# elcritch/figdraw

Measured on AMD Instinct MI355X. Metric: Mpixels/s composited @3840x2160, 300 SDF rects+shadows; % HBM roofline, higher is better.
Workload: dtype f32 (blur taps: u8 x f16 -> f32 MFMA); 1 GPU; S300@4K: renderlist_100 scene at 3840x2160, 300 shadowed SDF rects + full-frame and 360x240 2-pass Gaussian backdrop blur(18) (BASELINE.json configs[2]); draws=707, phases=3, blur_nodes=2, fragments=41088819, parallelism=single GPU, frames_in_flight_per_gpu=4, walk_pool_threads=7, walk_pool_threads_default=7

## Files before the change

figdraw_amd/csrc/fdh_context.cpp:

```cpp
#include "fdh_context.h"
#include "fdh_host.h"
#include "fdh_walkpool.h"

#include <chrono>

#include <algorithm>
#include <cmath>
#include <cstdio>
#include <cstring>

namespace fdh {

void hip_check(hipError_t e, const char* what) {
  if (e != hipSuccess) throw Error(FDH_ERR_HIP, std::string(what) + ": " + hipGetErrorString(e));
}

void poison_fresh(void* p, size_t bytes) {
#if defined(FDH_POISON)
  if (!p || !bytes) return;
  (void)hipMemset(p, FDH_POISON, bytes);
  (void)hipDeviceSynchronize();
#else
  (void)p; (void)bytes;
#endif
// ... 376 lines not shown
      B.sub_first[p] = at; B.sub_x0[p] = x0; B.sub_y0[p] = y0; B.sub_nx[p] = std::max(1, nx);
      at += nx * ny;
    }
    B.sub_first[np] = at;
    B.sub_n = np;
  }
  return B;
}

Context::Schedule Context::schedule(const LaunchJob& J, bool direct, bool partial) {
  const int nb = J.bins_x * J.bins_y;
  Schedule S;
  const int order_key = J.bins_x * 65536 + J.bins_y;
  if (order_valid_ && order_nb_ != order_key) order_valid_ = false;
  const bool sorting = J.clear && !J.phases.empty() && nb <= 8192 && J.phases[0].count > 0 && !direct && !partial;
  if (sorting) {
    S.order_now = order_valid_ ? d_order_[order_read_].ptr : nullptr;
    const int wr = order_valid_ ? 1 - order_read_ : order_read_;
    d_order_[wr].reserve(nb);
    S.order_next = d_order_[wr].ptr;
    order_read_ = wr;
    order_nb_ = order_key;
    order_valid_ = true;
  }
  static const int deep_env = [] { const char* e = std::getenv("FDH_DEEP_MIN"); return e ? std::atoi(e) : -1; }();
  S.deep_min = deep_env >= 0 ? deep_env : (vram_contexts_alive(device_) > 1 ? kDeepMinInFlight : kDeepMinDefault);
  if (sorting && S.deep_min > 0) {
    if (!deep_host_) {
      FDH_HIP(hipHostMalloc((void**)&deep_host_, 64, hipHostMallocDefault));
      for (int c = 0; c < 8; c++) deep_host_[c] = 0;
    }
    if (S.order_now) {
      uint32_t most = 0;
      for (int c = 0; c < 8; c++) most = std::max(most, (uint32_t)deep_host_[c]);
      S.deep_k8 = 8 * (int)std::min<uint32_t>(most, 1024u);
    }
  }
  return S;
}

uint32_t* Context::launch_blur(const LaunchJob& J, int p, uint32_t* cur, int row_lo, int row_hi, bool partial) {
  const Phase& ph = J.phases[p];
  if (ph.blur < 0) return cur;
  const BlurJob& j = J.blurs[ph.blur];
  const bool big = ph.blur == J.big_blur;
  const int vy0 = std::max(j.y0, row_lo), vy1 = std::min(j.y1, row_hi);
  if (vy1 <= vy0 || j.x1 <= j.x0) return cur;
  BlurParams bp;
  bp.W = J.W; bp.H = J.H; bp.pitch = J.W;
  bp.taps = j.taps;
  bp.node_pixels = (long long)(j.x1 - j.x0) * (j.y1 - j.y0);
  bp.fuse_draw = -1;
  bp.mx_w = (size_t)ph.blur < J.mx_w_h.size() ? J.mx_w_h[ph.blur] : nullptr;
  bp.x0 = j.x0; bp.x1 = j.x1; bp.y0 = vy0; bp.y1 = vy1;
  if ((size_t)ph.blur < J.blur_fused.size() && J.blur_fused[ph.blur]) {
    uint32_t* other = cur == fb_ ? alt_ : fb_;
    bp.src = cur; bp.dst = other;
    bp.fuse_draw = j.fuse_draw;
    span_begin(kSpanBlurFused);
    const bool done = launch_blur_fused(stream_, bp, J.mx_w_v[ph.blur], J.dv.recs, J.dv.exts);
    span_end();
    if (!done) throw Error(FDH_ERR_HIP, "fused blur: no kernel for this filter width (blur_fused_supported out of step with the launcher)");
    return other;
  }
  if (j.fuse_draw < 0 && J.latency_routes && blur_one_kernel_ok(j.x1 - j.x0, j.y1 - j.y0, j.taps.reach)) {
    bp.src = cur; bp.dst = backdrop_;
    span_begin(big ? kSpanBigBlurV : kSpanBlurV);
    launch_blur_small(stream_, bp);
    span_end();
    return cur;
  }
  bp.src = cur; bp.dst = blur_tmp_;
  bp.y0 = std::max(0, vy0 - j.taps.reach); bp.y1 = std::min(J.H, vy1 + j.taps.reach);
  const bool guard = partial && j.fuse_draw >= 0;
  if (guard) damage_.guard(stream_, J, ph.blur, false, cur, vy0, vy1);
  span_begin(big ? kSpanBigBlurH : kSpanBlurH);
  launch_blur_h(stream_, bp);
  span_end();
  bp.src = blur_tmp_; bp.dst = j.fuse_draw >= 0 ? cur : backdrop_;
  bp.mx_w = (size_t)ph.blur < J.mx_w_v.size() ? J.mx_w_v[ph.blur] : nullptr;
  bp.fuse_draw = j.fuse_draw;
  bp.y0 = vy0; bp.y1 = vy1;
  span_begin(big ? kSpanBigBlurV : kSpanBlurV);
  launch_blur_v(stream_, bp, J.dv.recs, J.dv.exts);
  span_end();
  if (guard) damage_.guard(stream_, J, ph.blur, true, cur, vy0, vy1);
  return cur;
}

CompositeParams Context::composite_params(const LaunchJob& J, int p, uint32_t* cur, int row_lo, int row_hi, bool direct, const Schedule& S) const {
  const Phase& ph = J.phases[p];
  const int nb = J.bins_x * J.bins_y;
  const bool full = p == 0 && J.clear;
  CompositeParams C;
  C.lists = J.lists + (size_t)p * nb * J.list_stride;
  C.counts = J.counts + (size_t)p * nb;
  C.backdrop = backdrop_;
  C.fb = cur;
  for (int l = 0; l < kMaxMips; l++) C.atlas.level[l] = atlas_levels_[l];
  C.atlas.size = atlas_size_; C.atlas.n_levels = n_levels_;
  C.W = J.W; C.H = J.H; C.pitch = J.W;
  C.bins_x = J.bins_x; C.stride = J.list_stride;
  C.bin_x0 = full ? 0 : ph.bin_x0; C.bin_y0 = full ? 0 : ph.bin_y0;
  C.bin_nx = full ? J.bins_x : ph.bin_x1 - ph.bin_x0; C.bin_ny = full ? J.bins_y : ph.bin_y1 - ph.bin_y0;
  C.row_lo = row_lo; C.row_hi = row_hi;
  C.load_fb = full ? 0 : 1;
  C.clear_rgba8 = J.clear_rgba8;
  C.direct = direct ? 1 : 0; C.direct_first = ph.first; C.direct_n = ph.count; C.binrec = J.dv.binrecs;
  C.order = full ? S.order_now : nullptr; C.order_next = full ? S.order_next : nullptr;
  C.deep_k8 = full ? S.deep_k8 : 0; C.deep_min = S.deep_min;
  static const int deep_strip_min = [] { const char* e = std::getenv("FDH_DEEP_STRIP_MIN"); return e ? std::atoi(e) : kDeepStripMinDefault; }();
  C.deep_strip_min = deep_strip_min;
  C.deep_out = (full && S.order_next && S.deep_min > 0) ? const_cast<uint32_t*>(deep_host_) : nullptr;
  C.has_slow = ph.has_slow; C.has_slow_atlas = ph.has_slow_atlas; C.has_rot = ph.has_rot; C.has_atlas = ph.has_atlas; C.has_masks = ph.has_masks;
  C.mask_spill = J.mask_spill; C.spill_stride = J.spill_stride;
  return C;
}

void Context::launch_frame(const LaunchJob& J, bool profile, uint32_t upload_seq) {
  profiling_ = profile;
  std::vector<int> lo, hi;
  phase_rows(J, lo, hi);
  const bool direct = direct_frame(J);
  const BinParams B = bin_params(J, upload_seq);
  span_begin(kSpanBin); if (!direct) launch_bin(stream_, B); span_end();
  const bool partial = damage_.launch(stream_, J, B, readback_, [this](bool begin) { if (begin) span_begin(kSpanBin); else span_end(); });
  const Schedule S = schedule(J, direct, partial);
  uint32_t* cur = fb_;
  for (int p = 0; p < (int)J.phases.size(); p++) {
    cur = launch_blur(J, p, cur, lo[p], hi[p], partial);
    CompositeParams C = composite_params(J, p, cur, lo[p], hi[p], direct, S);
    if (C.load_fb == 0) stats_.deep_bins = (float)composite_build(C).deep_k8;
    span_begin(p == 0 ? kSpanCompositeMain : kSpanCompositeLater);
    if (partial) damage_.composite(stream_, J, C);
    else launch_composite(stream_, J.dv.recs, J.dv.exts, C);
    span_end();
  }
  if (cur != fb_) std::swap(fb_, alt_);
  damage_.launched_whole(J);
  FDH_HIP(hipGetLastError());
}

void Context::replay(int times) {
  need_device("replay");
  drain();
  if (!have_frame_) throw Error(FDH_ERR_INVALID, "replay: no frame has been submitted");
  FDH_HIP(hipSetDevice(device_));
  if (times <= 0) return;
  FDH_HIP(hipEventRecord(ev_[0], stream_));
  for (int i = 0; i < times; i++) launch_frame(job_, false);
  FDH_HIP(hipEventRecord(ev_[1], stream_));
  FDH_HIP(hipEventSynchronize(ev_[1]));
  float ms = 0.0f;
  FDH_HIP(hipEventElapsedTime(&ms, ev_[0], ev_[1]));
  stats_.ms_total = ms / (float)times;
}

void Context::replay_async(int times) {
  need_device("replay_async");
  drain();
// ... 140 lines not shown
```

figdraw_amd/csrc/fdh_context.h:

```cpp
#pragma once
#include <hip/hip_runtime.h>

#include <algorithm>
#include <atomic>
#include <chrono>
#include <condition_variable>
#include <cstdint>
#include <cstdlib>
#include <cstring>
#include <exception>
#include <memory>
#include <mutex>
#include <stdexcept>
#include <string>
#include <thread>
#include <unordered_map>
#include <vector>

#include "../../include/figdraw_hip.h"
#include "../../include/figdraw_hip_pick.h"
#include "../../include/figdraw_hip_readback.h"
#include "../../include/figdraw_hip_stream.h"
#include "fdh_kernels.h"

// ... 279 lines not shown
  std::vector<DrawRec> recs;
  std::vector<BinRec> bins;
  std::vector<QuadExt> exts;
  std::vector<PickTag> tags;
  bool tagged = false;
  PhaseSum sum;
  int64_t fragments = 0;
  bool cacheable = false;
  bool dirty = true;
  uint64_t atlas_epoch = 0;
  int cull_y0 = 0, cull_y1 = 0;
};
struct RetainedLayer {
  int32_t zlevel = 0;
  std::vector<FdhFig> nodes;
  std::vector<int32_t> roots;
  std::vector<RetainedRoot> cache;
};
struct RetainedScene {
  bool valid = false;
  float fw = 0, fh = 0, rgba[4] = {1, 1, 1, 1};
  bool clear = true;
  float ui_scale = 1.0f, aa = 0.0f;
  bool subpixel = false, variants = false;
  uint32_t table_epoch = 0, table_epoch_seen = 0;
  std::vector<RetainedLayer> layers;
  std::vector<FdhGlyph> glyphs;
  std::vector<int64_t> variant_ids;
  std::vector<FdhDrawOp> ops;
  std::vector<float> controls;
  std::vector<FdhTextRect> text_rects;
  int64_t roots_walked = 0, roots_reused = 0;
};

struct FrameLayout {
  size_t recs = 0, exts = 0, binrecs = 0, boxes = 0, chunks = 0, phase_first = 0, tables = 0, total = 0;
  size_t n = 0, n_ext = 0, n_chunks = 1;
  std::vector<size_t> mx_h, mx_v;
  size_t misc() const { return chunks; }
  void lay_out(size_t n_recs, size_t n_exts, size_t n_phases, const std::vector<BlurJob>& blurs);
  bool operator==(const FrameLayout& o) const {
    return total == o.total && recs == o.recs && exts == o.exts && binrecs == o.binrecs && boxes == o.boxes && chunks == o.chunks &&
           phase_first == o.phase_first && n == o.n && n_ext == o.n_ext && mx_h == o.mx_h && mx_v == o.mx_v;
  }
};

struct LaunchJob {
  struct View { DrawRec* recs = nullptr; QuadExt* exts = nullptr; BinRec* binrecs = nullptr; int* phase_first = nullptr; uint32_t* binbox = nullptr; uint32_t* chunkbox = nullptr; };
  int W = 0, H = 0;
  int rec_y0 = 0, rec_y1 = 0;
  bool clear = true;
  bool latency_routes = true;
  uint32_t clear_rgba8 = 0xFFFFFFFFu;
  std::vector<Phase> phases;
  std::vector<BlurJob> blurs;
  std::vector<const uint4*> mx_w_h, mx_w_v;
  std::vector<char> blur_fused;
  int n_fused = 0;
  int n_recs = 0;
  FrameLayout layout;
  View dv;
  uint32_t* mask_spill = nullptr;
  size_t spill_stride = 0;
  uint2* lists = nullptr;
  uint32_t* counts = nullptr;
  int bins_x = 0, bins_y = 0, list_stride = 0, binbox_shift = 0;
  int big_blur = -1;
  std::vector<UploadRun> runs;
  UploadTable table;
  void* d_dst = nullptr;
  int staging_slot = -1;
  bool damage = false, damage_force = false;
  uint64_t damage_key = 0;
  int n_exts = 0;
  bool pick = false;
  std::vector<PickTag> pick_tags;
  int pick_depth = 0;
};

}
#include "fdh_damage_host.h"
namespace fdh {

class Context : public Recorder {
 public:
  Context(int atlas_size, float pixel_scale, int device, uint32_t flags);
  ~Context();

  void begin_frame(int w, int h, bool clear, const float rgba[4]);
  void end_frame();
  float pixel_scale() const { return pixel_scale_; }
  void set_subpixel_enabled(bool e) { subpixel_enabled_ = e; }
  void set_subpixel_variants(bool e) { subpixel_variants_ = e; }
  void set_text_lcd_filtering(bool e) { text_lcd_filtering_ = e; }
  bool text_lcd_filtering() const { return text_lcd_filtering_; }
  void comm_info(int* rank, int* world) const { *rank = comm_ ? comm_rank_ : 0; *world = comm_ ? comm_world_ : 1; }

  void put_image(int64_t key, int w, int h, const uint8_t* rgba, int out_rect[4]);
  void put_glyph_image(int64_t key, int w, int h, const uint8_t* rgba, uint32_t flags, int out_rect[4]);
  void put_glyph_outline(int64_t key, int w, int h, const float* segs, int n, uint32_t flags, int out_rect[4]);
  void update_image(int64_t key, int w, int h, const uint8_t* rgba);
  void put_mips(int64_t key, int n, const int* ws, const int* hs, const uint8_t* const* premul_rgba, int out_rect[4]);
  void put_flippy(int64_t key, const uint8_t* data, size_t n, int out_rect[4]);
  void remove_image(int64_t key) { entries_.erase(key); atlas_epoch_++; }
  bool has_image(int64_t key) const { return entries_.count(key) != 0; }
  void reset_atlas(int minimum_size);
// ... 37 lines not shown
  void set_damage_tracking(bool on);
  void damage_bins(uint8_t* mask, int cap, int* bins_x, int* bins_y, int* n_damaged, bool changed_only);
  void set_damage_readback(bool on);
  void read_damage(const FdhDamageTile** tiles, const uint8_t** pixels, int* n_tiles, int* frame_w, int* frame_h, int* full);
  void read_damage_into(uint8_t* image, int64_t pitch_bytes, int w, int h, int* n_tiles);
  void read_damage_coded(const FdhCodedTile** tiles, const uint8_t** payload, int* n_tiles, int64_t* payload_bytes, int* frame_w, int* frame_h, int* full);
  void set_damage_exact(bool on);
  void damage_exact_stats(int* n_pending, int* n_changed, int* fresh);
  void set_pick(bool on) { pick_on_ = on; }
  void set_pick_tag(int32_t z, int32_t id) { tag_ = PickTag{z, id}; }
  void pick_points(const float* xy, int n, int threshold, uint32_t flags, int max_hits, FdhPickHit* out, int* counts);
  void pick_region(int x, int y, int w, int h, int threshold, uint32_t flags, int32_t* out_draw);
  void pick_draw_tags(int32_t* zlevels, int32_t* ids, int cap, int* n);
  void set_cull(int mode) { cull_mode_ = mode < 0 ? 0 : (mode > 2 ? 2 : mode); }
  int64_t culled_draws() const { return culled_total_; }
  void set_walk_threads(int n) { walk_threads_ = n < 0 ? -1 : (n > 64 ? 64 : n); }
  int walk_threads() const;
  int64_t parallel_groups() const { return parallel_groups_; }
  void set_blur_route(int route) { blur_route_ = route < 0 ? -1 : (route ? 1 : 0); }
  void replay(int times);
  void replay_timed(int times, float* ms_out);
  void replay_async(int times);
  void profile(int times);
  void frame_stats(FdhFrameStats* out) { drain(); *out = stats_; out->ms_host_launch = launch_ms_.load(std::memory_order_relaxed); }
  void flush() { drain(); }

 private:
  friend class Recorder;
  friend struct ParallelWalk;
  void release_device_state();
  void rec_begin_frame(bool clear, const float rgba[4]);
  void rec_end_frame();
  void alloc_atlas(int size);
  void upload_atlas_rect(int level, int x, int y, int w, int h, const uint8_t* rgba);
  void put_levels(int x, int y, int w, int h, const uint8_t* rgba);
  void find_empty_rect(int w, int h, int* ox, int* oy);
  struct FoldGuard {
    BinRec* br = nullptr;
    BBox box{0, 0, 0, 0};
    FoldGuard() = default;
    FoldGuard(FoldGuard&& o) noexcept : br(o.br), box(o.box) { o.br = nullptr; }
    FoldGuard(const FoldGuard&) = delete;
    FoldGuard& operator=(const FoldGuard&) = delete;
    ~FoldGuard() { if (br) br->box = box; }
  };

  void prepare(LaunchJob& J);
  void describe_frame(LaunchJob& J);
  void size_bin_buffers(LaunchJob& J);
  void layout_frame_block(LaunchJob& J);
  void choose_fused_blurs(LaunchJob& J);
  void consolidate_pieces();
  FoldGuard fold_clear(LaunchJob& J);
  void damage_frame_key(LaunchJob& J) const;
  bool shadow_usable(const LaunchJob& J);
  bool tables_resident(const LaunchJob& J, bool shadow_ok);
  void build_misc(const LaunchJob& J, bool tables_resident);
  bool patch_runs(LaunchJob& J, bool shadow_ok);
  void gather_runs(LaunchJob& J, bool tables_resident);
  void account_frame(LaunchJob& J);
  void fence_staging();
  void issue(LaunchJob& J);
  void launch_frame(const LaunchJob& J, bool profile, uint32_t upload_seq = 0);
  struct Schedule { const int* order_now = nullptr; int* order_next = nullptr; int deep_min = 0, deep_k8 = 0; };
  void phase_rows(const LaunchJob& J, std::vector<int>& lo, std::vector<int>& hi) const;
  BinParams bin_params(const LaunchJob& J, uint32_t upload_seq) const;
  Schedule schedule(const LaunchJob& J, bool direct, bool partial);
  uint32_t* launch_blur(const LaunchJob& J, int p, uint32_t* cur, int row_lo, int row_hi, bool partial);
  CompositeParams composite_params(const LaunchJob& J, int p, uint32_t* cur, int row_lo, int row_hi, bool direct, const Schedule& S) const;
  template <typename Buf> void reserve_quiet(Buf& buf, size_t n);
  void drain();
  void worker_main();
  hipEvent_t next_event();
  void ensure_surfaces();
  void need_device(const char* what) const;
  void split_phase(int blur);
  void open_piece();
  void close_piece();
  void add_piece(const Piece& p, const PhaseSum& s, const BBox& outer_union, int64_t fragments, int64_t culled);
  void add_sum(const PhaseSum& s, int depth_base);
  void close_phase();
  uint32_t global_index(uint32_t lane0_index) const { return lane0_index + g0_delta_; }
  uint32_t global_count() const;
  Lane& lane(int i) { return i < 0 ? *merge_lane_[(size_t)staging_i_] : *lanes_[(size_t)staging_i_][(size_t)i]; }
  Lane& ensure_lane(int i);
  void splice_cached(const RetainedRoot& C);
  void pick_routes();
  void pool_slots(int slots);

  int device_ = 0;
  uint32_t flags_ = 0;
  int blur_route_ = -1;
  bool latency_routes_ = true;
  std::shared_ptr<void> comm_;
  int comm_rank_ = 0, comm_world_ = 1;
  hipStream_t own_stream_ = nullptr, stream_ = nullptr;
  volatile unsigned int* hdp_flush_reg_ = nullptr;
  hipEvent_t ev_[2] = {};
  std::vector<hipEvent_t> ev_pool_;
  size_t ev_used_ = 0;
  enum SpanKind { kSpanBin, kSpanCompositeMain, kSpanCompositeLater, kSpanBlurH, kSpanBlurV, kSpanBigBlurH, kSpanBigBlurV, kSpanBlurFused, kSpanKinds };
  struct Span { SpanKind kind; hipEvent_t a, b; };
  std::vector<Span> spans_;
  bool profiling_ = false;
  void span_begin(SpanKind kind); void span_end();

// ... 23 lines not shown
  std::exception_ptr worker_error_;
  alignas(128) LaunchJob job_;
  std::atomic<float> launch_ms_{0.0f};
  alignas(128) LaunchJob next_;
  const void* tables_dev_ = nullptr;
  FrameLayout tables_layout_;
  std::vector<float> tables_sig_, tables_sig_next_;

  alignas(128) bool rec_diff_upload_ = false;
  std::vector<Piece> pieces_;
  bool piece_open_ = false;
  uint32_t n_total_ = 0, n_ext_total_ = 0;
  uint32_t g0_delta_ = 0;
  std::vector<Phase> phases_;
  std::vector<BlurJob> blurs_;
  BBox phase_u_{0, 0, 0, 0};
  int stride_max_ = 1;
  int phase_extra_ = 0;
  int deepest_clip_ = 0;
  int64_t frag_mode_[4] = {0, 0, 0, 0}, frag_ellip_ = 0, frag_other_ = 0;
  bool have_frame_ = false;

  alignas(128) uint32_t* fb_ = nullptr;
  uint32_t *backdrop_ = nullptr, *blur_tmp_ = nullptr;
  uint32_t* alt_ = nullptr;
  uint32_t* dbg_snap_ = nullptr;
  void glyph_to_atlas(uint32_t* cur, uint32_t* nxt, int w, int h, int x, int y, uint32_t flags);
  void put_glyph_mtsdf(int64_t key, int w, int h, const float* segs, int n, float range, int out_rect[4]);
  DeviceBuf<float> glyph_lines_, glyph_acc_, glyph_edges_;
  DeviceBuf<uint32_t> glyph_a_, glyph_b_;
  RetainedScene retained_;
  uint64_t atlas_epoch_ = 1;
  void rebase_side(FdhFig* nodes, int n, const FdhScene* side);
  void compact_side();
  bool host_only_ = false;
  bool rec_on_ = false, rec_first_ = true, rec_mark_first_ = true;
  size_t rec_mark_ = 0;
  std::string rec_;
  int surf_w_ = 0, surf_h_ = 0;
  DeviceBuf<uint8_t> d_frame_;
  DeviceBuf<uint32_t> d_mask_spill_;
  DeviceBuf<uint2> d_lists_;
  DeviceBuf<uint32_t> d_counts_;
  DeviceBuf<int> d_order_[2];
  DamageTracker damage_;
  DamageReadback readback_;
  ReadFrame read_frame(const char* who);
  bool pick_on_ = false, pick_frame_ = false;
  void pick_check(const char* who, int threshold, uint32_t flags);
  DeviceBuf<uint8_t> d_pick_, d_pick_spill_;
  PinnedBuf<uint8_t> h_pick_;
  int order_read_ = 0, order_nb_ = 0;
  bool order_valid_ = false;
  struct MxTables { int reach; std::vector<float> dense; std::vector<uint8_t> h, v; };
  std::vector<MxTables> mx_cache_;
  static constexpr int kStaging = 4;
  std::vector<std::unique_ptr<Lane>> lanes_[kStaging];
  std::unique_ptr<Lane> merge_lane_[kStaging];
  std::vector<std::unique_ptr<Recorder>> pool_recs_;
  uint64_t frame_no_ = 0;
  HostVec<uint8_t> misc_[kStaging];
  std::vector<uint8_t> misc_host_;
  const uint8_t* misc_dev_[kStaging] = {};
  const uint8_t* misc_dev_host_[kStaging] = {};
  std::vector<uint8_t> shadow_;
  FrameLayout shadow_layout_;
  const void* shadow_dev_ = nullptr;
  int64_t uploaded_bytes_ = 0;
  hipEvent_t staging_ev_[kStaging] = {};
  char staging_busy_[kStaging] = {};
  uint32_t staging_seq_[kStaging] = {};
  volatile uint32_t* deep_host_ = nullptr;
  volatile uint32_t* seq_host_ = nullptr;
  uint32_t upload_seq_ = 0;
  void wait_staging(int slot);
  int staging_i_ = 0;

  int atlas_size_ = 0, initial_atlas_size_ = 0, atlas_margin_ = 4, n_levels_ = 0;
  uint32_t* atlas_levels_[kMaxMips] = {};
  std::vector<uint16_t> heights_;
  std::unordered_map<int64_t, AtlasEntry> entries_;

  FdhFrameStats stats_ = {};
 public:
  int64_t host_ns_[12] = {};
  struct HostTimer {
    int64_t& acc; std::chrono::steady_clock::time_point t0;
    explicit HostTimer(int64_t& a) : acc(a), t0(std::chrono::steady_clock::now()) {}
    ~HostTimer() { acc += std::chrono::duration_cast<std::chrono::nanoseconds>(std::chrono::steady_clock::now() - t0).count(); }
  };
 private:
  std::chrono::steady_clock::time_point t_begin_frame_, t_walk_begin_;
  float host_record_ms_ = 0.0f;
};

template <typename Buf> void Context::reserve_quiet(Buf& buf, size_t n) {
  if (n <= buf.cap) return;
  drain();
  FDH_HIP(hipStreamSynchronize(stream_));
  buf.reserve(n);
}

void record_host_form(DrawRec& r);
void stripe_rows(int height, int world, int rank, int* y0, int* y1);
void comm_unique_id(uint8_t out[FDH_COMM_ID_BYTES]);
void blur_weight_fragments(float blur_radius, bool vertical, float* dense, uint16_t* frag_bits, int* reach, int* k_steps);
void saturated_core_of(const float rect[4], const float rx[4], const float ry[4], int mode, float factor, float spread,
// ... 4 lines not shown
```

figdraw_amd/csrc/fdh_device.h:

```cpp
#pragma once
#include <hip/hip_runtime.h>
#include <hip/hip_ext.h>
#include <stdint.h>
#include <algorithm>
#include <type_traits>

#include "fdh_kernels.h"

#include <cstddef>
#include <cstdlib>

namespace fdh {

#ifndef FDH_STATS
#define FDH_STATS 0
#endif
#ifndef FDH_TIMING
#define FDH_TIMING 0
#endif
#ifndef FDH_SPLIT_UNIFORM
#define FDH_SPLIT_UNIFORM 0
#endif
#if FDH_TIMING
#define FDH_NOW() clock64()
// ... 375 lines not shown
    long long a0 = (long long)q.e[t][0].a * X + (long long)q.e[t][0].b * Y + q.e[t][0].c;
    long long a1 = (long long)q.e[t][1].a * X + (long long)q.e[t][1].b * Y + q.e[t][1].c;
    long long a2 = (long long)q.e[t][2].a * X + (long long)q.e[t][2].b * Y + q.e[t][2].c;
    bool in = a0 >= 0 && a1 >= 0 && a2 >= 0;
    uint32_t own = q.own >> (t * 3);
    if (a0 == 0 && !(own & 1u)) in = false;
    if (a1 == 0 && !(own & 2u)) in = false;
    if (a2 == 0 && !(own & 4u)) in = false;
    if (in) { hit = t; e0 = a0; e1 = a1; e2 = a2; }
  }
  f.covered = f.covered && hit >= 0;
  const int t = hit < 0 ? 0 : hit;
  const float is = q.inv_sum[t];
  const float l0 = (float)e0 * is, l1 = (float)e1 * is, l2 = (float)e2 * is;
  const float u0 = t == 0 ? uax : utx, v0 = t == 0 ? uay : uay;
  const float u1 = t == 0 ? uax : uax, v1 = t == 0 ? uty : uay;
  const float u2 = utx, v2 = uty;
  f.u = l0 * u0 + l1 * u1 + l2 * u2;
  f.v = l0 * v0 + l1 * v1 + l2 * v2;
  F4 c0 = unpack255(t == 0 ? r.col[3] : r.col[2]);
  F4 c1 = unpack255(t == 0 ? r.col[0] : r.col[3]);
  F4 c2 = unpack255(r.col[1]);
  const float k = 1.0f / 255.0f;
  f.col.x = (l0 * c0.x + l1 * c1.x + l2 * c2.x) * k;
  f.col.y = (l0 * c0.y + l1 * c1.y + l2 * c2.y) * k;
  f.col.z = (l0 * c0.z + l1 * c1.z + l2 * c2.z) * k;
  f.col.w = (l0 * c0.w + l1 * c1.w + l2 * c2.w) * k;
  f.fw_u = q.fw_u[t];
  f.fw_v = q.fw_v[t];
  f.lod = q.lod[t];
  return f;
}

typedef float f2 __attribute__((ext_vector_type(2)));
__device__ __forceinline__ void blend(F4& F, float r, float g, float b, float sa) {
  const float ia = 1.0f - sa, A = 255.0f * sa;
  F.x = __builtin_rintf(__builtin_fmaf(F.x, ia, r * A));
  F.y = __builtin_rintf(__builtin_fmaf(F.y, ia, g * A));
  F.z = __builtin_rintf(__builtin_fmaf(F.z, ia, b * A));
  F.w = __builtin_rintf(__builtin_fmaf(F.w, ia, A));
}
__device__ __forceinline__ void blend_pre(F4& F, f2 c_rg, f2 c_ba, float ia) {
  f2 xy = {F.x, F.y}, zw = {F.z, F.w};
  const f2 ia2 = {ia, ia};
  xy = __builtin_elementwise_fma(xy, ia2, c_rg);
  zw = __builtin_elementwise_fma(zw, ia2, c_ba);
  F.x = __builtin_rintf(xy.x); F.y = __builtin_rintf(xy.y); F.z = __builtin_rintf(zw.x); F.w = __builtin_rintf(zw.y);
}

__device__ __forceinline__ void blend_black(F4& F, float A, float ia) {
  F.x = __builtin_rintf(F.x * ia); F.y = __builtin_rintf(F.y * ia); F.z = __builtin_rintf(F.z * ia); F.w = __builtin_rintf(__builtin_fmaf(F.w, ia, A));
}

__device__ __forceinline__ float rect_mask_alpha(const DrawRec& r, float cx, float cy) {
  float lx = (r.ox * cx + r.oy * cy) + r.inv_w;
  float ly = (r.inv_h * cx + r.f0 * cy) + r.f1;
  float qx = lx - r.p0, qy = ly - r.p1;
  float dist = shape_dist((r.op_mode & F_ELLIP) != 0u, qx, -qy, r.p2, r.p3, r.r[0], r.r[1], r.r[2], r.r[3]);
  return 1.0f - clamp01(r.aa * dist + 0.5f);
}

__device__ __forceinline__ DrawRec load_rec(const DrawRec* __restrict__ p) {
  DrawRec r;
  const uint4* __restrict__ src = reinterpret_cast<const uint4*>(p);
  uint4* dst = reinterpret_cast<uint4*>(&r);
#pragma unroll
  for (int i = 0; i < 8; i++) dst[i] = src[i];
  return r;
}

typedef uint32_t u32x4 __attribute__((ext_vector_type(4)));
__device__ __forceinline__ DrawRec load_rec_whole(const DrawRec* __restrict__ p) {
  const u32x4* __restrict__ src = reinterpret_cast<const u32x4*>(p);
  u32x4 q[8];
#pragma unroll
  for (int i = 0; i < 8; i++) q[i] = src[i];
  asm volatile("" : "+s"(q[0]), "+s"(q[1]), "+s"(q[2]), "+s"(q[3]), "+s"(q[4]), "+s"(q[5]), "+s"(q[6]), "+s"(q[7]));
  DrawRec r;
  const auto f = [](uint32_t v) { return __uint_as_float(v); };
  r.op_mode = q[0].x; r.ext = q[0].y; r.ox = f(q[0].z); r.oy = f(q[0].w);
  r.inv_w = f(q[1].x); r.inv_h = f(q[1].y); r.p0 = f(q[1].z); r.p1 = f(q[1].w);
  r.p2 = f(q[2].x); r.p3 = f(q[2].y); r.f0 = f(q[2].z); r.f1 = f(q[2].w);
  r.r[0] = f(q[3].x); r.r[1] = f(q[3].y); r.r[2] = f(q[3].z); r.r[3] = f(q[3].w);
  r.col[0] = q[4].x; r.col[1] = q[4].y; r.col[2] = q[4].z; r.col[3] = q[4].w;
  r.mid = q[5].x; r.stop = q[5].y; r.aa = f(q[5].z); r.aux = f(q[5].w);
  r.aux2 = f(q[6].x);
  r.bx0 = (int16_t)(q[6].y & 0xffffu); r.by0 = (int16_t)(q[6].y >> 16); r.bx1 = (int16_t)(q[6].z & 0xffffu); r.by1 = (int16_t)(q[6].z >> 16);
  r.ix0 = (int16_t)(q[6].w & 0xffffu); r.iy0 = (int16_t)(q[6].w >> 16); r.ix1 = (int16_t)(q[7].x & 0xffffu); r.iy1 = (int16_t)(q[7].x >> 16);
  r.kx = f(q[7].y); r.ky = f(q[7].z); r._pad = q[7].w;
  return r;
}
static_assert(LE_PLAIN == 0x80000000u, "the compositor tests LE_PLAIN as the sign bit");
static_assert(offsetof(DrawRec, p2) == 32 && offsetof(DrawRec, col) == 64 && offsetof(DrawRec, aux2) == 96 && offsetof(DrawRec, bx0) == 100 && offsetof(DrawRec, ix0) == 108 && offsetof(DrawRec, aa) == 88 && offsetof(DrawRec, kx) == 116, "load_rec_whole follows DrawRec's layout");

__device__ __forceinline__ void local_x4(const DrawRec& r, float cx0, float (&lx)[4]) {
  lx[0] = __builtin_fmaf(cx0 - r.ox, r.inv_w, -0.5f) * (2.0f * r.p0);
  lx[1] = lx[0] + r.kx;
  lx[2] = __builtin_fmaf(2.0f, r.kx, lx[0]);
  lx[3] = __builtin_fmaf(3.0f, r.kx, lx[0]);
}
__device__ __forceinline__ float local_y_up(const DrawRec& r, float cy) {
  return __builtin_fmaf(r.oy - cy, r.inv_h, 0.5f) * (2.0f * r.p1);
}
__device__ __forceinline__ float cover_aa(float d, float aa) { return clamp01(__builtin_fmaf(-d, aa, 0.5f)); }

__device__ __forceinline__ void unpack2(uint32_t c, f2& rg, f2& ba) {
// ... 13 lines not shown
```

figdraw_amd/csrc/fdh_kernels.h:

```cpp
#pragma once
#include <hip/hip_runtime.h>

#include <cstdlib>

#include "fdh_types.h"

namespace fdh {

struct BinParams {
  const BinRec* binrec;
  const uint32_t* binbox;
  const uint32_t* chunkbox;
  int n_draws, binbox_shift;
  uint2* lists;
  uint32_t* counts;
  const int* phase_first;
  int n_phases, bins_x, bins_y, stride;
  const DrawRec* draws;
  const QuadExt* exts;
  int refine;
  uint32_t* seq_out = nullptr;
  uint32_t seq = 0;
  static constexpr int kBinSubs = 8;
  int sub_n = 0;
  int sub_first[kBinSubs + 1] = {};
  int sub_x0[kBinSubs] = {}, sub_y0[kBinSubs] = {}, sub_nx[kBinSubs] = {};
};

struct CompositeParams {
  const int* order;
  int* order_next;
  const uint32_t* counts;
  const uint2* lists;
  int bin_x0, bin_y0, bin_nx, bin_ny;
  int bins_x, stride;
  int row_lo, row_hi;
  int W, H, pitch;
  int load_fb;
  uint32_t clear_rgba8;
  int n_wg;
  uint32_t* fb;
  const uint32_t* backdrop;
  int has_masks;
  int has_slow;
  int has_slow_atlas = 0;
  int has_rot;
  int has_atlas;
  uint32_t* mask_spill;
  size_t spill_stride;
  AtlasView atlas;
  int direct = 0, direct_first = 0, direct_n = 0;
  const BinRec* binrec = nullptr;
  int deep_k8 = 0;
  int deep_strip_min = 0;
  int deep_min = 0;
  uint32_t* deep_out = nullptr;
};

struct BlurParams {
  const uint32_t* src;
  uint32_t* dst;
  int W, H, pitch;
  int x0, y0, x1, y1;
  int fuse_draw;
  const uint4* mx_w;
  BlurTaps taps;
  long long node_pixels = 0;
};

void set_launch_events(hipEvent_t start, hipEvent_t stop);
bool launch_events_used();
void launch_bin(hipStream_t s, const BinParams& P);
inline int forced_kernel_paths() { static const int v = [] { const char* e = std::getenv("FDH_FORCE_KERNEL_PATHS"); return e ? std::atoi(e) : 0; }(); return v; }
struct CompositeBuild { int paths = 4; size_t lds = 0; int deep_k8 = 0; bool deep = false; };
CompositeBuild composite_build(CompositeParams& P);
void launch_composite(hipStream_t s, const DrawRec* draws, const QuadExt* exts, CompositeParams P);
void launch_blur_h(hipStream_t s, const BlurParams& P);
void launch_blur_v(hipStream_t s, const BlurParams& P, const DrawRec* draws, const QuadExt* exts);
bool blur_one_kernel_ok(int w, int h, int reach);
void launch_blur_small(hipStream_t s, const BlurParams& P);
bool blur_fused_supported(int reach, int W, int pitch);
bool launch_blur_fused(hipStream_t s, const BlurParams& P, const uint4* w_v, const DrawRec* draws, const QuadExt* exts);
void launch_fill(hipStream_t s, uint32_t* p, uint32_t v, size_t n);
void launch_rasterize_lines(hipStream_t s, const float4* lines, int n, int w, int h, float* scratch, uint32_t* out);
void launch_lcd_filter(hipStream_t s, const uint32_t* src, uint32_t* dst, int w, int h);
void launch_minify2(hipStream_t s, const uint32_t* src, uint32_t* dst, int sw, int sh);
void launch_atlas_blit(hipStream_t s, uint32_t* level, int LS, int x, int y, const uint32_t* src, int w, int h);
void launch_msdf_generate(hipStream_t s, const float* edges, int n_edges, int w, int h, float orient, float range, uint32_t* out);
constexpr int kMaxUploadRuns = 96;
struct UploadRun { const void* src; uint32_t dst_off, bytes, ext_add, kind; };
struct UploadTable {
  uint32_t n_runs, copy_units, n_draws, binbox_shift;
  uint32_t bins_off, box_off, _pad0, _pad1;
  uint32_t unit_first[kMaxUploadRuns];
  UploadRun run[kMaxUploadRuns];
};
static_assert(sizeof(UploadTable) <= 4096, "the table must fit the kernel-argument segment");
void launch_upload_frame(hipStream_t s, void* dst, const UploadTable& T);

}
```

figdraw_amd/csrc/fdh_prepare.cpp:

```cpp
#include "fdh_context.h"
#include "fdh_damage.h"
#include "fdh_host.h"

#include <algorithm>
#include <chrono>
#include <cmath>
#include <cstring>

namespace fdh {

static uint16_t half_bits_rne(float f) {
  uint32_t u;
  std::memcpy(&u, &f, 4);
  const uint16_t sign = (uint16_t)((u >> 16) & 0x8000u);
  const float a = std::fabs(f);
  if (a == 0.0f) return sign;
  std::memcpy(&u, &a, 4);
  const int e = (int)(u >> 23) - 127;
  if (e < -14) return sign | (uint16_t)std::nearbyint(a * 16777216.0f);
  const uint32_t mant = u & 0x7fffffu, m = mant >> 13, rem = mant & 0x1fffu;
  uint32_t h = ((uint32_t)(e + 15) << 10) | m;
  if (rem > 0x1000u || (rem == 0x1000u && (m & 1u))) h++;
  return sign | (uint16_t)h;
}
static float half_value(uint16_t h) {
  const int e = (h >> 10) & 31, m = h & 1023;
  const float v = e == 0 ? std::ldexp((float)m, -24) : std::ldexp((float)(m + 1024), e - 25);
  return (h & 0x8000u) ? -v : v;
}
static void quantise_taps_f16(const BlurTaps& t, float* q) {
  const int r = t.reach;
  const double centre = (double)t.dense[kBlurPad + r] * 1024.0;
  q[r] = half_value(half_bits_rne((float)centre));
  double carry = 0.5 * (centre - (double)q[r]);
  for (int k = r - 1; k >= 0; k--) {
    if (t.dense[kBlurPad + k] == 0.0f) { q[k] = q[2 * r - k] = 0.0f; continue; }
    const double want = std::max((double)t.dense[kBlurPad + k] * 1024.0 + carry, 0.0);
    const float v = half_value(half_bits_rne((float)want));
    carry = want - (double)v;
    q[k] = q[2 * r - k] = v;
  }
}
static void build_mx_weights(const BlurTaps& t, bool vertical, uint8_t* out) {
  const int nk = mx_nk(t.reach, vertical), delta = mx_delta(t.reach, vertical);
  uint16_t* o = reinterpret_cast<uint16_t*>(out);
  float q[2 * kMaxBlurReach + 1];
  quantise_taps_f16(t, q);
  for (int m = 0; m < nk; m++)
    for (int lane = 0; lane < 64; lane++) {
      const int j = lane & 31, g = lane >> 5;
      for (int e = 0; e < 8; e++) {
        const int k = 16 * m + mx_krow(g, e, vertical) - delta - j;
#if FDH_MX_LO
        const float w = (k >= 0 && k <= 2 * t.reach) ? t.dense[kBlurPad + k] * 1024.0f : 0.0f;
        const uint16_t hi = half_bits_rne(w), lo = half_bits_rne(w - half_value(hi));
#else
        const float w = (k >= 0 && k <= 2 * t.reach) ? q[k] : 0.0f;
        const uint16_t hi = half_bits_rne(w), lo = 0;
#endif
        o[(((size_t)(2 * m) * 64 + lane) * 8) + e] = hi;
        o[(((size_t)(2 * m + 1) * 64 + lane) * 8) + e] = lo;
      }
    }
}

void blur_weight_fragments(float blur_radius, bool vertical, float* dense, uint16_t* frag_bits, int* reach, int* k_steps) {
  const BlurTaps t = make_taps(blur_radius);
  for (int k = 0; k <= 2 * t.reach; k++) dense[k] = t.dense[kBlurPad + k];
  *reach = t.reach;
  *k_steps = mx_nk(t.reach, vertical);
  if (*k_steps > kMxMaxNK) throw Error(FDH_ERR_INVALID, "blur_weight_fragments: filter too wide");
  build_mx_weights(t, vertical, reinterpret_cast<uint8_t*>(frag_bits));
}

void FrameLayout::lay_out(size_t n_recs, size_t n_exts, size_t n_phases, const std::vector<BlurJob>& blurs) {
  n = n_recs; n_ext = n_exts;
  n_chunks = std::max<size_t>((n + 255) / 256, 1);
  recs = 0;
  exts = align256(recs + n * sizeof(DrawRec));
  binrecs = align256(exts + n_ext * sizeof(QuadExt));
  boxes = align256(binrecs + n * sizeof(BinRec));
  chunks = align256(boxes + ((n + 3) & ~(size_t)3) * sizeof(uint32_t));
  phase_first = align256(chunks + n_chunks * sizeof(uint32_t));
  tables = align256(phase_first + (n_phases + 1) * sizeof(int));
  total = tables;
  mx_h.assign(blurs.size(), 0); mx_v.assign(blurs.size(), 0);
  for (size_t i = 0; i < blurs.size(); i++) {
    const int nkh = mx_nk(blurs[i].taps.reach, false), nkv = mx_nk(blurs[i].taps.reach, true);
    if (nkh > kMxMaxNK || nkv > kMxMaxNK) continue;
    mx_h[i] = total; total = align256(total + mx_table_bytes(nkh));
    mx_v[i] = total; total = align256(total + mx_table_bytes(nkv));
  }
}

void Context::prepare(LaunchJob& J) {
  const auto t_s0 = std::chrono::steady_clock::now();
  FDH_HIP(hipSetDevice(device_));
  describe_frame(J);
  size_bin_buffers(J);
  layout_frame_block(J);
  choose_fused_blurs(J);
  if (pieces_.size() * 3 + 2 > (size_t)kMaxUploadRuns) consolidate_pieces();
  const FoldGuard fold = fold_clear(J);
  damage_frame_key(J);
  const bool shadow_ok = shadow_usable(J), resident = tables_resident(J, shadow_ok);
  build_misc(J, resident);
  if (!patch_runs(J, shadow_ok)) gather_runs(J, resident);
  tables_dev_ = d_frame_.ptr; tables_layout_ = J.layout; tables_sig_.swap(tables_sig_next_);
  account_frame(J);
  fence_staging();
  stats_.ms_host_record = host_record_ms_;
  stats_.ms_host_upload = std::chrono::duration<float, std::milli>(std::chrono::steady_clock::now() - t_s0).count();
}

void Context::describe_frame(LaunchJob& J) {
  J.W = W_; J.H = H_; J.clear = clear_; J.clear_rgba8 = clear_rgba8_;
  J.rec_y0 = culling() ? cull_y0_ : 0; J.rec_y1 = culling() ? cull_y1_ : H_;
  J.latency_routes = latency_routes_;
  J.phases = phases_;
  J.blurs = blurs_;
  J.n_recs = (int)n_total_;
  J.n_exts = (int)n_ext_total_;
  J.bins_x = (W_ + kBin - 1) / kBin;
  J.bins_y = (H_ + kBin - 1) / kBin;
  J.binbox_shift = binbox_shift_;
  J.staging_slot = staging_i_;
}

void Context::size_bin_buffers(LaunchJob& J) {
  const int nb = J.bins_x * J.bins_y;
  J.list_stride = (stride_max_ + 7) & ~7;
  reserve_quiet(d_lists_, (size_t)J.phases.size() * nb * J.list_stride);
  reserve_quiet(d_counts_, (size_t)J.phases.size() * nb);
  J.lists = d_lists_.ptr; J.counts = d_counts_.ptr;
  J.mask_spill = nullptr;
  J.spill_stride = (size_t)nb * 16 * 64;
  if (deepest_clip_ > kMaskDepth) {
    const size_t levels = (size_t)(deepest_clip_ - kMaskDepth);
    if (levels * J.spill_stride * sizeof(uint32_t) > ((size_t)2 << 30))
      throw Error(FDH_ERR_UNSUPPORTED, "clip masks nested too deep for this frame size (the spill plane would exceed 2 GiB)");
    reserve_quiet(d_mask_spill_, levels * J.spill_stride);
    J.mask_spill = d_mask_spill_.ptr;
  }
}

void Context::layout_frame_block(LaunchJob& J) {
  FrameLayout& F = J.layout;
  F.lay_out(n_total_, n_ext_total_, J.phases.size(), J.blurs);
  if (F.total >= ((size_t)1 << 32)) throw Error(FDH_ERR_UNSUPPORTED, "frame block beyond 4 GiB");
  reserve_quiet(d_frame_, F.total);
  uint8_t* const d = d_frame_.ptr;
  J.d_dst = d;
  LaunchJob::View& dv = J.dv;
  dv.recs = reinterpret_cast<DrawRec*>(d + F.recs);
  dv.exts = reinterpret_cast<QuadExt*>(d + F.exts);
  dv.binrecs = reinterpret_cast<BinRec*>(d + F.binrecs);
// ... 13 lines not shown
  const bool fx_on = latency_routes_;
  J.blur_fused.assign(J.blurs.size(), 0);
  J.n_fused = 0;
  for (size_t i = 0; i < J.blurs.size(); i++) {
    const BlurJob& j = J.blurs[i];
    static const bool any_size = [] { const char* e = std::getenv("FDH_FORCE_BLUR_PATH"); return e && std::atoi(e) == 3; }();
    if (fx_on && clear_ && j.fuse_draw >= 0 && J.mx_w_h[i] && j.x0 == 0 && j.y0 == 0 && j.x1 == W_ && j.y1 == H_ && blur_fused_supported(j.taps.reach, W_, W_) &&
        (any_size || (long long)W_ * H_ >= 384 * 1024)) {
      J.blur_fused[i] = 1;
      J.n_fused++;
    }
  }
  if (J.n_fused > 0 && !alt_) {
    FDH_HIP(hipMalloc((void**)&alt_, (size_t)W_ * H_ * 4));
    poison_fresh(alt_, (size_t)W_ * H_ * 4);
    FDH_HIP(hipMemsetAsync(alt_, 0, (size_t)W_ * H_ * 4, stream_));
  }
}

Context::FoldGuard Context::fold_clear(LaunchJob& J) {
  FoldGuard g;
  static const bool fold_on = [] { const char* e = std::getenv("FDH_FOLD_CLEAR"); return !e || std::atoi(e) != 0; }();
  if (fold_on && clear_ && !pieces_.empty() && J.phases[0].count > 0) {
    const Piece& p0 = pieces_[0];
    Lane& L = lane(p0.lane);
    BinRec& br = L.bins[p0.first];
    const DrawRec& r = L.recs[p0.first];
    const uint32_t om = r.op_mode;
    if (((om >> 12) & 15u) == OP_DRAW && (br.flags & LE_PLAIN) && !(br.flags & BR_CORE_REMOVED) && (br.flags & BR_HAS_CORE) && br.ix0 <= 0 && br.iy0 <= 0 &&
        br.ix1 >= W_ && br.iy1 >= H_ && br.box.x0 <= 0 && br.box.y0 <= 0 && br.box.x1 >= W_ && br.box.y1 >= H_) {
      const float inv255 = 1.0f / 255.0f;
      const uint32_t c = r.col[0];
      float cf[3];
      std::memcpy(cf, &r.col[1], sizeof cf);
      const float sa = (float)(c >> 24) * inv255, A = 255.0f * sa, ia = 1.0f - sa;
      const float src[4] = {cf[0] * A, cf[1] * A, cf[2] * A, A};
      uint32_t out = 0;
      for (int k = 0; k < 4; k++) {
        const float F = (float)((J.clear_rgba8 >> (8 * k)) & 255u);
        const float v = std::nearbyintf(std::fmaf(F, ia, src[k]));
        out |= (uint32_t)std::min(std::max((int)v, 0), 255) << (8 * k);
      }
      J.clear_rgba8 = out;
      g.br = &br;
      g.box = br.box;
      br.box = BBox{0, 0, 0, 0};
      if (p0.lane > 0) L.publish_bytes(1, (size_t)p0.first * sizeof(BinRec), sizeof(BinRec));
    }
  }
  stats_.clear_folded = g.br ? 1.0f : 0.0f;
  return g;
}

void Context::damage_frame_key(LaunchJob& J) const {
  J.damage = damage_.on;
  J.damage_force = !clear_ || J.n_fused > 0 || J.blurs.size() > (size_t)kDamageMaxNodes;
  uint64_t k = 1469598103934665603ull;
  auto mix = [&k](uint64_t v) { for (int b = 0; b < 8; b++) { k ^= (v >> (8 * b)) & 255u; k *= 1099511628211ull; } };
  uint32_t aa_bits = 0, ps_bits = 0;
  std::memcpy(&aa_bits, &ctx_aa_, 4); std::memcpy(&ps_bits, &pixel_scale_, 4);
  mix((uint64_t)(uint32_t)W_ << 32 | (uint32_t)H_); mix((uint64_t)(uint32_t)J.bins_x << 32 | (uint32_t)J.bins_y);
  mix((uint64_t)J.clear_rgba8 << 1 | (clear_ ? 1u : 0u)); mix((uint64_t)aa_bits << 32 | ps_bits);
  mix(atlas_epoch_); mix((uint64_t)(uint32_t)atlas_size_);
  mix((uint64_t)(latency_routes_ ? 1u : 0u) << 8 | (uint64_t)(uint32_t)cull_mode_);
  J.damage_key = k;
}

bool Context::shadow_usable(const LaunchJob& J) {
  if (!rec_diff_upload_) shadow_dev_ = nullptr;
  return rec_diff_upload_ && shadow_dev_ == d_frame_.ptr && shadow_layout_ == J.layout && shadow_.size() == J.layout.total;
}

bool Context::tables_resident(const LaunchJob& J, bool shadow_ok) {
  std::vector<float>& sig = tables_sig_next_;
  sig.clear();
  for (size_t i = 0; i < J.blurs.size(); i++)
    if (J.layout.mx_h[i]) { const BlurTaps& t = J.blurs[i].taps; sig.push_back((float)t.reach); sig.insert(sig.end(), t.dense + kBlurPad, t.dense + kBlurPad + 2 * t.reach + 1); }
  return tables_dev_ == d_frame_.ptr && tables_layout_ == J.layout && tables_sig_ == sig && (!rec_diff_upload_ || shadow_ok);
}

void Context::build_misc(const LaunchJob& J, bool tables_resident) {
  const FrameLayout& F = J.layout;
  std::vector<uint8_t>& misc = misc_host_;
  const size_t o_misc = F.misc();
  misc.assign((tables_resident ? F.tables : F.total) - o_misc, 0);
  int* pf = reinterpret_cast<int*>(misc.data() + (F.phase_first - o_misc));
  for (size_t i = 0; i < J.phases.size(); i++) pf[i] = J.phases[i].first;
  pf[J.phases.size()] = (int)F.n;
  {
    uint32_t* cb = reinterpret_cast<uint32_t*>(misc.data());
    for (size_t c = 0; c < F.n_chunks; c++) cb[c] = 0x7f7f7f7fu;
    size_t g = 0;
    for (const Piece& p : pieces_) {
      const uint32_t* bx = lane(p.lane).boxes.p + p.first;
      for (uint32_t i = 0; i < p.n; i++, g++) {
        const uint32_t m = cb[g >> 8], v = bx[i];
        uint32_t o = 0;
        for (int sh = 0; sh < 32; sh += 8) o |= std::min((m >> sh) & 255u, (v >> sh) & 255u) << sh;
        cb[g >> 8] = o;
      }
    }
  }
  for (size_t i = 0; i < J.blurs.size() && !tables_resident; i++)
    if (F.mx_h[i]) {
      const BlurTaps& t = J.blurs[i].taps;
      const size_t bh = mx_table_bytes(mx_nk(t.reach, false)), bv = mx_table_bytes(mx_nk(t.reach, true));
      const MxTables* hit = nullptr;
      for (const MxTables& c : mx_cache_)
        if (c.reach == t.reach && std::memcmp(c.dense.data(), t.dense + kBlurPad, sizeof(float) * (2 * t.reach + 1)) == 0) { hit = &c; break; }
      if (!hit) {
        if (mx_cache_.size() >= 8) mx_cache_.erase(mx_cache_.begin());
        MxTables c;
        c.reach = t.reach;
        c.dense.assign(t.dense + kBlurPad, t.dense + kBlurPad + 2 * t.reach + 1);
        c.h.resize(bh); c.v.resize(bv);
        build_mx_weights(t, false, c.h.data());
        build_mx_weights(t, true, c.v.data());
        mx_cache_.push_back(std::move(c));
        hit = &mx_cache_.back();
      }
      std::memcpy(misc.data() + (F.mx_h[i] - o_misc), hit->h.data(), bh);
      std::memcpy(misc.data() + (F.mx_v[i] - o_misc), hit->v.data(), bv);
    }
  const int slot = J.staging_slot;
  HostVec<uint8_t>& up_misc = misc_[slot];
  up_misc.pinned = true;
  up_misc.vram = vram_staging(device_);
  up_misc.dev = device_;
  up_misc.n = 0;
  up_misc.reserve(misc.size());
  if (up_misc.p != misc_dev_host_[slot]) { misc_dev_[slot] = up_misc.device_view(); misc_dev_host_[slot] = up_misc.p; }
}

bool Context::patch_runs(LaunchJob& J, bool shadow_ok) {
  if (!shadow_ok || pieces_.size() > 1 || (!pieces_.empty() && pieces_[0].lane != 0)) return false;
  const Piece p0 = pieces_.empty() ? Piece{} : pieces_[0];
  if (p0.ext_first != 0) return false;
  const FrameLayout& F = J.layout;
  const std::vector<uint8_t>& misc = misc_host_;
  HostVec<uint8_t>& up_misc = misc_[J.staging_slot];
  const size_t o_misc = F.misc(), b_recs = F.n * sizeof(DrawRec), b_ext = F.n_ext * sizeof(QuadExt), b_bb = F.n * sizeof(BinRec);
  Lane& L = lane(0);
  L.publish(0, 0, 0, 0);
  std::vector<UploadRun>& runs = J.runs;
  runs.clear();
  std::vector<const uint8_t*> from;
  size_t dirty = 0;
  bool fits = true;
  auto diff = [&](const uint8_t* host, const uint8_t* dev_src, size_t off, size_t bytes, uint32_t kind) {
    for (size_t at = 0; at < bytes && fits; at += 256) {
      const size_t len = std::min<size_t>(256, bytes - at);
      if (std::memcmp(shadow_.data() + off + at, host + at, len) == 0) continue;
      dirty += len;
      if (!runs.empty() && runs.back().kind == kind && (size_t)runs.back().dst_off + runs.back().bytes == off + at) runs.back().bytes += (uint32_t)len;
      else if (runs.size() + 4 < (size_t)kMaxUploadRuns) { runs.push_back(UploadRun{dev_src + at, (uint32_t)(off + at), (uint32_t)len, 0u, kind}); from.push_back(host + at); }
      else fits = false;
    }
  };
  diff(reinterpret_cast<const uint8_t*>(L.recs.p + p0.first), L.d_recs + (size_t)p0.first * sizeof(DrawRec), F.recs, b_recs, 0u);
  diff(reinterpret_cast<const uint8_t*>(L.exts.p), L.d_exts, F.exts, b_ext, 0u);
  diff(reinterpret_cast<const uint8_t*>(L.bins.p + p0.first), L.d_bins + (size_t)p0.first * sizeof(BinRec), F.binrecs, b_bb, 1u);
  diff(misc.data(), misc_dev_[J.staging_slot], o_misc, F.tables - o_misc, 0u);
  if (!fits || dirty * 2 >= F.total) return false;
  for (size_t k = 0; k < runs.size(); k++) {
    std::memcpy(shadow_.data() + runs[k].dst_off, from[k], runs[k].bytes);
    const size_t off = runs[k].dst_off;
    if (off >= o_misc) std::memcpy(up_misc.p + (off - o_misc), misc.data() + (off - o_misc), runs[k].bytes);
    else if (off >= F.binrecs) L.publish_bytes(1, (size_t)p0.first * sizeof(BinRec) + (off - F.binrecs), runs[k].bytes);
    else if (off >= F.exts && b_ext) L.publish_bytes(2, off - F.exts, runs[k].bytes);
    else L.publish_bytes(0, (size_t)p0.first * sizeof(DrawRec) + (off - F.recs), runs[k].bytes);
  }
  uploaded_bytes_ = (int64_t)dirty;
  return true;
// ... 116 lines not shown
```

figdraw_amd/csrc/fdh_types.h:

```cpp
#pragma once
#include <stdint.h>

#ifndef FDH_MX_LO
#define FDH_MX_LO 0
#endif

namespace fdh {

constexpr int kTile = 8;
constexpr int kTileW = 4 * kTile;
constexpr int kTileH = kTile;
constexpr int kWavesPerWg = 4;
constexpr int kWgW = kTileW;
constexpr int kWgH = kTileH * kWavesPerWg;
constexpr int kBin = 64;
constexpr int kWgsPerBin = (kBin / kWgW) * (kBin / kWgH);
constexpr int kMaskDepth = 16;
constexpr int kDeepMinDefault = 24;
constexpr int kDeepMinInFlight = 40;
constexpr int kDeepStripMinDefault = 16;
constexpr int kMaxMips = 14;
constexpr int kMaxBlurTaps = 36;

enum : uint32_t { OP_DRAW = 0, OP_MASK_PUSH = 1, OP_MASK_POP = 2, OP_RMASK_BEGIN = 3, OP_RMASK_END = 4 };
// ... 22 lines not shown
  float aux2;
  int16_t bx0, by0, bx1, by1;
  int16_t ix0, iy0, ix1, iy1;
  float kx, ky;
  uint32_t _pad;
};
static_assert(sizeof(DrawRec) == 128, "DrawRec must be 128 bytes");

struct alignas(16) QuadExt {
  struct Edge { int32_t a, b; int64_t c; };
  Edge e[2][3];
  float inv_sum[2];
  uint32_t own;
  float fw_u[2], fw_v[2];
  float lod[2];
  float _pad[3];
  float core[4];
  float lm[2][6];
};
static_assert(sizeof(QuadExt) == 208 && offsetof(QuadExt, core) == 144 && offsetof(QuadExt, lm) == 160, "QuadExt: 208 bytes, core at 144, lm at 160");

struct alignas(8) BBox { int16_t x0, y0, x1, y1; };

struct alignas(8) BinRec { BBox box; int16_t ix0, iy0, ix1, iy1; uint32_t flags; uint32_t pad; };
static_assert(sizeof(BinRec) == 24, "BinRec must be 24 bytes");
constexpr uint32_t BR_HAS_CORE = 1u, BR_CORE_REMOVED = 2u;
constexpr uint32_t BR_GENERAL = 4u;
constexpr uint32_t BR_CURVE = 8u;
constexpr uint32_t BR_BOX_EXACT = 16u;
constexpr uint32_t LE_PLAIN = 1u << 31;
constexpr uint32_t LE_OPAQUE = 1u << 30;
constexpr int LE_PATH_SHIFT = 26;
constexpr uint32_t LE_SHARE = 1u << 25;
constexpr uint32_t LE_INDEX = LE_SHARE - 1u;

constexpr int kMaxBlurReach = 66;
constexpr int kBlurPad = 15;
struct BlurTaps {
  int n;
  int reach;
  int off[kMaxBlurTaps];
  float coef[kMaxBlurTaps];
  float dense[2 * kMaxBlurReach + 1 + 2 * kBlurPad + 16];
};

constexpr int kMxMaxNK = 11;
inline int mx_nk(int reach, bool vertical) { return (32 + 2 * reach + (vertical ? 0 : 3) + 15) / 16; }
inline int mx_delta(int reach, bool vertical) { return vertical ? 0 : ((-reach) % 4 + 4) % 4; }
#if defined(__HIPCC__)
__host__ __device__
#endif
inline int mx_krow(int g, int e, bool vertical) { return vertical ? (e & 3) + 8 * (e >> 2) + 4 * g : 8 * g + e; }
constexpr size_t mx_table_bytes(int nk) { return (size_t)nk * 2 * 64 * 16; }

struct AtlasView {
  const uint32_t* level[kMaxMips];
  int size;
  int n_levels;
};

}
```

figdraw_amd/csrc/k_blur_mx.hip:

```cpp
#include "fdh_device.h"

namespace fdh {
using h8 = __attribute__((ext_vector_type(8))) _Float16;
using f32x16 = __attribute__((ext_vector_type(16))) float;
union H8Bits { h8 v; uint32_t u[4]; };

template <int c> __device__ __forceinline__ h8 mx_frag(const uint32_t (&R)[8]) {
  constexpr uint32_t sel = 0x0c000c00u | (uint32_t)c | ((uint32_t)(4 + c) << 16);
  H8Bits o;
#pragma unroll
  for (int q = 0; q < 4; q++) o.u[q] = __builtin_amdgcn_perm(R[2 * q + 1], R[2 * q], sel);
  return o.v;
}
constexpr int kMxWaves = 2;
constexpr int mx_ring_slots(int nk, bool ) { return nk + 2; }
constexpr int mx_wg(int , bool ) { return 1; }
constexpr float kMxScale = 16384.0f;
constexpr int kMxSlot = 512;
__device__ __forceinline__ void lds_dma16(const void* src, uint32_t lds) {
  uint32_t m0_saved;
  asm volatile("s_mov_b32 %0, m0\n\ts_mov_b32 m0, %2\n\ts_nop 0\n\tglobal_load_lds_dwordx4 %1, off\n\ts_mov_b32 m0, %0"
               : "=&s"(m0_saved) : "v"(src), "s"(lds) : "memory");
}
__device__ __forceinline__ void lds_dma4(const void* src, uint32_t lds) {
  uint32_t m0_saved;
  asm volatile("s_mov_b32 %0, m0\n\ts_mov_b32 m0, %2\n\ts_nop 0\n\tglobal_load_lds_dword %1, off\n\ts_mov_b32 m0, %0"
               : "=&s"(m0_saved) : "v"(src), "s"(lds) : "memory");
}
template <int N> __device__ __forceinline__ void wait_vm() { asm volatile("s_waitcnt vmcnt(%0)" ::"n"(N) : "memory"); }

template <int NK, bool kV>
__global__ __launch_bounds__(64 * mx_wg(NK, kV), kMxWaves) void k_blur_mx(BlurParams P, const DrawRec* __restrict__ draws, const QuadExt* __restrict__ exts, int T) {
  constexpr int R = mx_ring_slots(NK, kV);
  extern __shared__ __attribute__((aligned(16))) uint32_t ring_wg[];
  constexpr int kWG = mx_wg(NK, kV);
  const int wave_in_wg = kWG > 1 ? __builtin_amdgcn_readfirstlane((int)(threadIdx.x >> 6)) : 0;
  uint32_t* const ring = ring_wg + wave_in_wg * (R * kMxSlot);
  const int a_lo = kV ? P.y0 : P.x0, a_hi = kV ? P.y1 : P.x1, a0 = a_lo & ~31;
  const int l0 = kV ? (P.x0 & ~31) : P.y0, l_hi = kV ? P.x1 : P.y1;
  const int n_along = (a_hi - a0 + 32 * T - 1) / (32 * T), n_lines = (l_hi - l0 + 31) >> 5;
  const int total = n_along * n_lines, per = (total + 7) >> 3, q = (int)(blockIdx.x >> 3) * kWG + wave_in_wg, item = (blockIdx.x & 7) * per + q;
  if (q >= per || item >= total) return;
  int sl, sa;
  if (kV) {
    constexpr int kBand = 16;
    const int per_band = kBand * n_along, band = item / per_band, rem = item - band * per_band;
    const int bw = min(kBand, n_lines - band * kBand);
    if (kWG > 1) {
      const int st = rem / n_along;
      sa = rem - st * n_along;
      sl = band * kBand + st;
    } else {
      sa = rem / bw;
      sl = band * kBand + rem - sa * bw;
    }
  } else {
    sl = item / n_along;
    sa = item - sl * n_along;
  }
  const int lane = threadIdx.x & 63, g = lane >> 5, j = lane & 31;
  const int reach = P.taps.reach;
  const int as = a0 + 32 * T * sa, lb = l0 + 32 * sl;
  const int n_blocks = min(T, (a_hi - as + 31) >> 5);
  const int w0 = as - reach, w0a = kV ? w0 : (w0 & ~3);
#if FDH_TIMING
  const unsigned long long T0 = FDH_NOW();
  unsigned long long T_wait = 0, T_st = 0, T_mma = 0, T_epi = 0, T_iss = 0;
#endif
  const uint32_t ring_lds = (uint32_t)reinterpret_cast<uintptr_t>(ring);

  const uint32_t* hsrc[2];
  if (!kV) {
    const int r = lane >> 2, c = lane & 3;
#pragma unroll
    for (int h = 0; h < 2; h++) {
      const int row = 16 * h + r, y = min(lb + row, P.y1 - 1);
      hsrc[h] = P.src + (size_t)y * P.pitch + 4 * (c ^ ((row >> 2) & 3));
    }
  }
  const int vxch = kV ? min(lb + 4 * (lane & 7), P.W - 4) : 0;
  int issue_slot = 0;
  auto issue = [&](int s) -> int {
    const uint32_t slot = ring_lds + (uint32_t)issue_slot * (kMxSlot * 4u);
    issue_slot = issue_slot + 1 == R ? 0 : issue_slot + 1;
    if (kV) {
      const int r = lane >> 3;
// ... 34 lines not shown
  h8 wlo[NK];
#endif
#pragma unroll
  for (int m = 0; m < NK; m++) {
    H8Bits a;
    const uint4 va = P.mx_w[(2 * m) * 64 + lane];
    a.u[0] = va.x; a.u[1] = va.y; a.u[2] = va.z; a.u[3] = va.w;
    whi[m] = a.v;
#if FDH_MX_LO
    H8Bits b;
    const uint4 vb = P.mx_w[(2 * m + 1) * 64 + lane];
    b.u[0] = vb.x; b.u[1] = vb.y; b.u[2] = vb.z; b.u[3] = vb.w;
    wlo[m] = b.v;
#endif
  }
  __builtin_amdgcn_s_waitcnt(0x0F70);
  last_batch = 0;
  int core_x0 = 0, core_y0 = 0, core_x1 = 0, core_y1 = 0;
  if (kV && P.fuse_draw >= 0) { const DrawRec* q = draws + P.fuse_draw; core_x0 = q->ix0; core_y0 = q->iy0; core_x1 = q->ix1; core_y1 = q->iy1; }
#if FDH_TIMING
  const unsigned long long T_pro = FDH_NOW() - T0 + (__builtin_amdgcn_readfirstlane(whi[0][0] != whi[0][1]) & 0u);
#endif
  uint32_t pend[16];
  uint32_t pmask = 0;
  int pbx = 0, pby = 0;
  auto store_pending = [&]() {
    const uint32_t lane_off = ((uint32_t)(4 * g) * (uint32_t)P.pitch + (uint32_t)j) * 4u;
    char* base = reinterpret_cast<char*>(P.dst + (size_t)pby * P.pitch + pbx);
    if (__all(pmask == 0xffffu)) {
#pragma unroll
      for (int rr = 0; rr < 16; rr++)
        *reinterpret_cast<uint32_t*>(base + (size_t)((rr & 3) + 8 * (rr >> 2)) * P.pitch * 4u + lane_off) = pend[rr];
    } else if (__any(pmask != 0u)) {
#pragma unroll
      for (int rr = 0; rr < 16; rr++)
        if ((pmask >> rr) & 1u) *reinterpret_cast<uint32_t*>(base + (size_t)((rr & 3) + 8 * (rr >> 2)) * P.pitch * 4u + lane_off) = pend[rr];
    }
    pmask = 0;
  };
  int slot0 = 0;
#pragma unroll 1
  for (int b = 0; b < n_blocks; b++) {
#if FDH_TIMING
    const unsigned long long Ta = FDH_NOW();
#endif
    wait_for_all_but(last_batch);
#if FDH_TIMING
    const unsigned long long Tb = FDH_NOW();
#endif
    store_pending();
#if FDH_TIMING
    const unsigned long long Tc = FDH_NOW();
#endif
    f32x16 acc[4];
#pragma unroll
    for (int c = 0; c < 4; c++)
#pragma unroll
      for (int e = 0; e < 16; e++) acc[c][e] = 0.0f;
#pragma unroll
    for (int m = 0; m < NK; m++) {
      const uint32_t* slot = ring + (slot0 + m >= R ? slot0 + m - R : slot0 + m) * kMxSlot;
      uint32_t t8[8];
      if (kV) {
#pragma unroll
        for (int t = 0; t < 8; t++) t8[t] = slot[((t & 3) + 8 * (t >> 2) + 4 * g) * 32 + j];
      } else {
        const uint4* row4 = reinterpret_cast<const uint4*>(slot + j * 16);
        const int sw = (j >> 2) & 3;
        const uint4 lo4 = row4[(2 * g) ^ sw], hi4 = row4[(2 * g + 1) ^ sw];
        t8[0] = lo4.x; t8[1] = lo4.y; t8[2] = lo4.z; t8[3] = lo4.w; t8[4] = hi4.x; t8[5] = hi4.y; t8[6] = hi4.z; t8[7] = hi4.w;
      }
      const h8 f0 = mx_frag<0>(t8), f1 = mx_frag<1>(t8), f2_ = mx_frag<2>(t8), f3 = mx_frag<3>(t8);
      if (kV) {
        acc[0] = __builtin_amdgcn_mfma_f32_32x32x16_f16(whi[m], f0, acc[0], 0, 0, 0);
        acc[1] = __builtin_amdgcn_mfma_f32_32x32x16_f16(whi[m], f1, acc[1], 0, 0, 0);
        acc[2] = __builtin_amdgcn_mfma_f32_32x32x16_f16(whi[m], f2_, acc[2], 0, 0, 0);
        acc[3] = __builtin_amdgcn_mfma_f32_32x32x16_f16(whi[m], f3, acc[3], 0, 0, 0);
#if FDH_MX_LO
        acc[0] = __builtin_amdgcn_mfma_f32_32x32x16_f16(wlo[m], f0, acc[0], 0, 0, 0);
        acc[1] = __builtin_amdgcn_mfma_f32_32x32x16_f16(wlo[m], f1, acc[1], 0, 0, 0);
        acc[2] = __builtin_amdgcn_mfma_f32_32x32x16_f16(wlo[m], f2_, acc[2], 0, 0, 0);
        acc[3] = __builtin_amdgcn_mfma_f32_32x32x16_f16(wlo[m], f3, acc[3], 0, 0, 0);
#endif
      } else {
        acc[0] = __builtin_amdgcn_mfma_f32_32x32x16_f16(f0, whi[m], acc[0], 0, 0, 0);
        acc[1] = __builtin_amdgcn_mfma_f32_32x32x16_f16(f1, whi[m], acc[1], 0, 0, 0);
        acc[2] = __builtin_amdgcn_mfma_f32_32x32x16_f16(f2_, whi[m], acc[2], 0, 0, 0);
        acc[3] = __builtin_amdgcn_mfma_f32_32x32x16_f16(f3, whi[m], acc[3], 0, 0, 0);
#if FDH_MX_LO
        acc[0] = __builtin_amdgcn_mfma_f32_32x32x16_f16(f0, wlo[m], acc[0], 0, 0, 0);
        acc[1] = __builtin_amdgcn_mfma_f32_32x32x16_f16(f1, wlo[m], acc[1], 0, 0, 0);
        acc[2] = __builtin_amdgcn_mfma_f32_32x32x16_f16(f2_, wlo[m], acc[2], 0, 0, 0);
        acc[3] = __builtin_amdgcn_mfma_f32_32x32x16_f16(f3, wlo[m], acc[3], 0, 0, 0);
#endif
      }
    }
#if FDH_TIMING
    const unsigned long long Td = FDH_NOW() + (__builtin_amdgcn_readfirstlane(__float_as_uint(acc[0][0] + acc[1][0] + acc[2][0] + acc[3][0])) & 0u);
#endif
    const int bx = kV ? lb : as + 32 * b, by = kV ? as + 32 * b : lb;
    const int x = bx + j;
    pbx = bx; pby = by;
    const bool x_ok = x >= P.x0 && x < P.x1;
#pragma unroll
    for (int rr = 0; rr < 16; rr++)
      pend[rr] = pack2(f2{acc[0][rr] * kMxScale, acc[1][rr] * kMxScale}, f2{acc[2][rr] * kMxScale, acc[3][rr] * kMxScale});
    if (bx >= P.x0 && bx + 32 <= P.x1 && by >= P.y0 && by + 32 <= P.y1) {
      pmask = 0xffffu;
    } else {
#pragma unroll
      for (int rr = 0; rr < 16; rr++) {
        const int y = by + (rr & 3) + 8 * (rr >> 2) + 4 * g;
        if (x_ok && y >= P.y0 && y < P.y1) pmask |= 1u << rr;
      }
    }
    if (kV && P.fuse_draw >= 0) {
      const bool core = bx >= core_x0 && bx + 32 <= core_x1 && by >= core_y0 && by + 32 <= core_y1;
      bool replace_all = false;
      if (core) {
        uint32_t conj = pend[0];
#pragma unroll
        for (int rr = 1; rr < 16; rr++) conj &= pend[rr];
        replace_all = __all((conj >> 24) == 255u);
      }
      if (!replace_all) {
      uint32_t blend_mask = 0;
      uint32_t* sc0 = ring + slot0 * kMxSlot;
      uint32_t* sc1 = ring + (slot0 + 1 >= R ? slot0 + 1 - R : slot0 + 1) * kMxSlot;
      if (core) {
#pragma unroll
        for (int rr = 0; rr < 16; rr++) if (((pmask >> rr) & 1u) && (pend[rr] >> 24) != 255u) blend_mask |= 1u << rr;
      } else {
        const uint32_t valid = pmask;
        pmask = 0;
#pragma unroll
        for (int rr = 0; rr < 16; rr++) (rr < 8 ? sc0 : sc1)[(rr & 7) * 64 + lane] = __float_as_uint(((valid >> rr) & 1u) ? 1.0f : -1.0f);
        __builtin_amdgcn_wave_barrier();
        const DrawRec r = load_rec(draws + P.fuse_draw);
        const int ry0 = min(max(P.y0 - by, 0), 32), ry1 = max(ry0, min(P.y1 - by, 32)), rx0 = min(max(P.x0 - bx, 0), 32), rx1 = max(rx0, min(P.x1 - bx, 32));
        const int ra = min(max(core_y0 - by, ry0), ry1), rb = max(ra, min(max(core_y1 - by, ry0), ry1));
        const int ca = min(max(core_x0 - bx, rx0), rx1), cb = max(ca, min(max(core_x1 - bx, rx0), rx1));
        const int nra = ra - ry0, nca = ca - rx0, nr = nra + ry1 - rb, nc = nca + rx1 - cb;
#pragma unroll 1
        for (int u0 = 0; u0 < nr + nc; u0 += 2) {
          const int u = u0 + g;
          int dx, dy;
          if (u < nr) { dy = u < nra ? ry0 + u : rb + (u - nra); dx = j; }
          else { const int v = u - nr; dx = v < nca ? rx0 + v : cb + (v - nca); dy = j; }
          if (u >= nr + nc) continue;
          const int ex = bx + dx, ey = by + dy;
          float alpha = -1.0f;
          if (ex >= P.x0 && ex < P.x1 && ey >= P.y0 && ey < P.y1) {
            const Frag f = make_frag(r, exts, ex, ey);
            if (f.covered) {
              const float lx = (f.u - 0.5f) * 2.0f * r.p0, ly = (f.v - 0.5f) * 2.0f * r.p1;
              const float dist = shape_dist((r.op_mode & F_ELLIP) != 0u, lx, -ly, r.p2, r.p3, r.r[0], r.r[1], r.r[2], r.r[3]);
              alpha = 1.0f - clamp01(r.aa * dist + 0.5f);
            }
          }
          const int er = (dy & 3) + 4 * (dy >> 3), el = dx + 32 * ((dy >> 2) & 1);
          (er < 8 ? sc0 : sc1)[(er & 7) * 64 + el] = __float_as_uint(alpha);
        }
        __builtin_amdgcn_wave_barrier();
#pragma unroll
        for (int rr = 0; rr < 16; rr++) {
          const float al = __uint_as_float((rr < 8 ? sc0 : sc1)[(rr & 7) * 64 + lane]);
          if (al >= 0.0f) {
            pmask |= 1u << rr;
            if (al != 1.0f || (pend[rr] >> 24) != 255u) blend_mask |= 1u << rr;
          }
        }
      }
      if (__any(blend_mask != 0u)) {
        uint32_t dstv[16];
#pragma unroll
        for (int rr = 0; rr < 16; rr++)
          dstv[rr] = ((blend_mask >> rr) & 1u) ? P.dst[(size_t)(by + (rr & 3) + 8 * (rr >> 2) + 4 * g) * P.pitch + x] : 0u;
        const float k = 1.0f / 255.0f;
#pragma unroll
        for (int rr = 0; rr < 16; rr++) {
          if (!((blend_mask >> rr) & 1u)) continue;
          const float alpha = core ? 1.0f : __uint_as_float((rr < 8 ? sc0 : sc1)[(rr & 7) * 64 + lane]);
          const F4 bl = unpack255(pend[rr]);
          F4 Fd = unpack255(dstv[rr]);
          const float sa = bl.w * k * alpha, A = 255.0f * sa;
          const float ia = 1.0f - sa;
          Fd.x = __builtin_rintf(__builtin_fmaf(Fd.x, ia, bl.x * k * A));
          Fd.y = __builtin_rintf(__builtin_fmaf(Fd.y, ia, bl.y * k * A));
          Fd.z = __builtin_rintf(__builtin_fmaf(Fd.z, ia, bl.z * k * A));
          Fd.w = __builtin_rintf(__builtin_fmaf(Fd.w, ia, A));
          pend[rr] = pack255(Fd);
        }
        __builtin_amdgcn_s_waitcnt(0x0F70);
      }
      __builtin_amdgcn_wave_barrier();
      }
    }
#if FDH_TIMING
    const unsigned long long Te = FDH_NOW() + (__builtin_amdgcn_readfirstlane(pend[0] + pend[15]) & 0u);
#endif
    __builtin_amdgcn_sched_barrier(0);
    last_batch = 0;
    if (b + 2 < n_blocks) { last_batch = issue(2 * b + NK + 2); last_batch += issue(2 * b + NK + 3); }
    slot0 = slot0 + 2 >= R ? slot0 + 2 - R : slot0 + 2;
#if FDH_TIMING
    const unsigned long long Tf = FDH_NOW();
    T_wait += Tb - Ta; T_st += Tc - Tb; T_mma += Td - Tc; T_epi += Te - Td; T_iss += Tf - Te;
#endif
  }
  store_pending();
#if FDH_TIMING
  if (lane == 0 && blockIdx.x < 32768) {
    unsigned long long* row = g_wave_times + 16 * ((size_t)blockIdx.x + (kV ? 32768 : 0));
    row[0] = FDH_NOW() - T0; row[1] = T_pro; row[2] = T_wait; row[3] = T_st; row[4] = T_mma; row[5] = T_epi; row[6] = kV ? 3 : 2; row[7] = T_iss; row[8] = n_blocks; row[9] = T0;
  }
#endif
}

constexpr int fx_vblocks(int nkv) { return ((nkv - 1) >> 1) + 1; }
constexpr int kFxWaves = 4;
constexpr int fx_wg_ksteps(int nkh) { return nkh + 2 * (kFxWaves - 1); }
constexpr int fx_slots(int nkh, int nkv) { return nkh + nkv + 2 * fx_wg_ksteps(nkh); }
constexpr float kMxMagic = 12582912.0f;
template <int NKH, int NKV>
__global__ __launch_bounds__(64 * kFxWaves, 2) void k_blur_fx(BlurParams P, const uint4* __restrict__ w_v, const DrawRec* __restrict__ draws, const QuadExt* __restrict__ exts, int T) {
  constexpr int HB = fx_vblocks(NKV);
  constexpr int NKW = fx_wg_ksteps(NKH);
  extern __shared__ __attribute__((aligned(16))) uint32_t ring[];
  const int wave = __builtin_amdgcn_readfirstlane((int)(threadIdx.x >> 6));
  const uint4* const hw = reinterpret_cast<const uint4*>(ring);
  const uint4* const vw = reinterpret_cast<const uint4*>(ring + NKH * kMxSlot);
  uint32_t* const src_base = ring + (NKH + NKV) * kMxSlot;
  const int n_strips = (P.x1 - (P.x0 & ~31) + 31) >> 5, n_sg = (n_strips + kFxWaves - 1) / kFxWaves;
  const int y_first = P.y0 & ~31;
  const int n_seg = (P.y1 - y_first + 32 * T - 1) / (32 * T);
  const int total = n_sg * n_seg, per = (total + 7) >> 3, q = (int)(blockIdx.x >> 3), item = (blockIdx.x & 7) * per + q;
  if (q >= per || item >= total) return;
  const int seg = item / n_sg, sg = item - seg * n_sg;
  const int strip = kFxWaves * sg + wave;
  const bool active = strip < n_strips;
  const int lane = threadIdx.x & 63, g = lane >> 5, j = lane & 31;
  const int reach = P.taps.reach;
  const int xb = (P.x0 & ~31) + 32 * strip;
  const int ys = y_first + 32 * T * seg;
  const int n_blocks = min(T, (P.y1 - ys + 31) >> 5);
  const int ws = ys - reach;
  const int w0a = ((P.x0 & ~31) + 32 * kFxWaves * sg - reach) & ~3;
  const uint32_t ring_lds = (uint32_t)reinterpret_cast<uintptr_t>(ring);
  const uint32_t src_lds = ring_lds + (uint32_t)((NKH + NKV) * kMxSlot * 4);

  auto issue_block = [&](int i) __attribute__((always_inline)) {
    const int r = lane >> 2, c = lane & 3;
    const uint32_t* dma_row[2];
#pragma unroll
    for (int h = 0; h < 2; h++) {
      const int row = 16 * h + r;
      int y = ws + 32 * i + row;
      y = y < 0 ? 0 : (y > P.H - 1 ? P.H - 1 : y);
      dma_row[h] = P.src + (size_t)y * P.pitch + 4 * (c ^ ((row >> 2) & 3));
    }
    const uint32_t copy = src_lds + (uint32_t)((i & 1) * NKW) * (kMxSlot * 4u);
#pragma unroll
    for (int s0 = 0; s0 < NKW; s0 += kFxWaves) {
      const int s = s0 + wave;
      if (s >= NKW) break;
      const uint32_t slot = copy + (uint32_t)s * (kMxSlot * 4u);
      const int xk = w0a + 16 * s;
      if (xk >= 0 && xk + 16 <= P.W) {
        lds_dma16(dma_row[0] + xk, slot);
        lds_dma16(dma_row[1] + xk, slot + 1024u);
      } else {
        const int rr = lane >> 4, pp = lane & 15;
#pragma unroll 1
        for (int e = 0; e < 8; e++) {
          const int row = 4 * e + rr;
          int y = ws + 32 * i + row;
          y = y < 0 ? 0 : (y > P.H - 1 ? P.H - 1 : y);
          int gx = xk + 4 * ((pp >> 2) ^ ((row >> 2) & 3)) + (pp & 3);
          gx = gx < 0 ? 0 : (gx > P.W - 1 ? P.W - 1 : gx);
          lds_dma4(P.src + (size_t)y * P.pitch + gx, slot + e * 256u);
        }
      }
    }
  };
  auto wait_for_all_but = [&](int n) __attribute__((always_inline)) {
    if (n >= 16) wait_vm<16>(); else if (n >= 3) wait_vm<3>(); else if (n == 2) wait_vm<2>(); else if (n == 1) wait_vm<1>(); else wait_vm<0>();
    __builtin_amdgcn_sched_barrier(0);
  };

#if FDH_TIMING
  const unsigned long long T0 = FDH_NOW();
  unsigned long long T_wait = 0, T_h = 0, T_v = 0, T_epi = 0, T_st = 0, T_cv = 0, T_cv_mark = 0, T_dma = 0;
#endif
  issue_block(0);
  int v_pieces = 0;
  {
    constexpr int NF = 2 * (NKH + NKV);
#pragma unroll
    for (int f0 = 0; f0 < NF; f0 += kFxWaves) {
      const int f = f0 + wave;
      if (f < NF) {
        lds_dma16((f < 2 * NKH ? P.mx_w + f * 64 : w_v + (f - 2 * NKH) * 64) + lane, ring_lds + (uint32_t)f * 1024u);
        if (f >= 2 * NKH) v_pieces++;
      }
    }
  }
#if FDH_TIMING
  const unsigned long long T_pro = FDH_NOW() - T0;
#endif
  int core_x0 = 0, core_y0 = 0, core_x1 = 0, core_y1 = 0;
  if (P.fuse_draw >= 0) { const DrawRec* qd = draws + P.fuse_draw; core_x0 = qd->ix0; core_y0 = qd->iy0; core_x1 = qd->ix1; core_y1 = qd->iy1; }

  uint32_t stash[2 * HB][4][4];
  auto operand = [](const uint32_t (&u)[4]) { H8Bits o; o.u[0] = u[0]; o.u[1] = u[1]; o.u[2] = u[2]; o.u[3] = u[3]; return o.v; };
  f32x16 acc[4];
  auto phase = [&](auto ph_tag, bool vertical) __attribute__((always_inline)) {
    constexpr int PH = decltype(ph_tag)::value;
    asm volatile("; k_blur_fx: phase %0" ::"n"(PH));
#pragma unroll
    for (int c = 0; c < 4; c++)
#pragma unroll
      for (int s2 = 0; s2 < 2; s2++)
#pragma unroll
        for (int qq = 0; qq < 4; qq++) {
          const float x0 = __builtin_fmaf(acc[c][8 * s2 + 2 * qq], kMxScale, kMxMagic), x1 = __builtin_fmaf(acc[c][8 * s2 + 2 * qq + 1], kMxScale, kMxMagic);
          const uint32_t pr = __builtin_amdgcn_perm(__float_as_uint(x1), __float_as_uint(x0), 0x0c040c00u);
          stash[2 * PH + s2][c][qq] = pr;
        }
#pragma unroll
    for (int c = 0; c < 4; c++)
#pragma unroll
      for (int s2 = 0; s2 < 2; s2++)
#pragma unroll
        for (int qq = 0; qq < 4; qq++) asm volatile("" : "+v"(stash[2 * PH + s2][c][qq]));
#if FDH_TIMING
    T_cv_mark = FDH_NOW() + (__builtin_amdgcn_readfirstlane(stash[2 * PH][0][0] ^ stash[2 * PH + 1][3][3]) & 0u);
#endif
    if (!vertical) return;
#pragma unroll
    for (int c = 0; c < 4; c++)
#pragma unroll
      for (int e = 0; e < 16; e++) acc[c][e] = 0.0f;
    constexpr int first = (PH + 1) % HB;
    uint4 va = vw[lane], vb = vw[64 + lane];
#pragma unroll
    for (int m = 0; m < NKV; m++) {
      const int slot = 2 * ((first + (m >> 1)) % HB) + (m & 1);
      H8Bits whi, wlo;
      whi.u[0] = va.x; whi.u[1] = va.y; whi.u[2] = va.z; whi.u[3] = va.w; wlo.u[0] = vb.x; wlo.u[1] = vb.y; wlo.u[2] = vb.z; wlo.u[3] = vb.w;
      if (m + 1 < NKV) { va = vw[(2 * m + 2) * 64 + lane]; vb = vw[(2 * m + 3) * 64 + lane]; }
      acc[0] = __builtin_amdgcn_mfma_f32_32x32x16_f16(whi.v, operand(stash[slot][0]), acc[0], 0, 0, 0);
      acc[1] = __builtin_amdgcn_mfma_f32_32x32x16_f16(whi.v, operand(stash[slot][1]), acc[1], 0, 0, 0);
      acc[2] = __builtin_amdgcn_mfma_f32_32x32x16_f16(whi.v, operand(stash[slot][2]), acc[2], 0, 0, 0);
      acc[3] = __builtin_amdgcn_mfma_f32_32x32x16_f16(whi.v, operand(stash[slot][3]), acc[3], 0, 0, 0);
#if FDH_MX_LO
      acc[0] = __builtin_amdgcn_mfma_f32_32x32x16_f16(wlo.v, operand(stash[slot][0]), acc[0], 0, 0, 0);
      acc[1] = __builtin_amdgcn_mfma_f32_32x32x16_f16(wlo.v, operand(stash[slot][1]), acc[1], 0, 0, 0);
      acc[2] = __builtin_amdgcn_mfma_f32_32x32x16_f16(wlo.v, operand(stash[slot][2]), acc[2], 0, 0, 0);
      acc[3] = __builtin_amdgcn_mfma_f32_32x32x16_f16(wlo.v, operand(stash[slot][3]), acc[3], 0, 0, 0);
#endif
      __builtin_amdgcn_sched_barrier(0);
    }
  };

  const int n_hblocks = n_blocks + HB - 1;
  int stores_behind = v_pieces;
  auto iteration = [&](auto ph_tag, int i) __attribute__((always_inline)) {
#if FDH_TIMING
    const unsigned long long Ta = FDH_NOW();
#endif
    wait_for_all_but(stores_behind);
    stores_behind = 0;
    __builtin_amdgcn_s_barrier();
    __builtin_amdgcn_sched_barrier(0);
    if (i + 1 < n_hblocks) issue_block(i + 1);
    __builtin_amdgcn_sched_barrier(0);
    if (!active) return;
    const uint32_t* const src_ring = src_base + ((i & 1) * NKW + 2 * wave) * kMxSlot;
#if FDH_TIMING
    const unsigned long long Tb = FDH_NOW();
#endif
#pragma unroll
    for (int c = 0; c < 4; c++)
#pragma unroll
      for (int e = 0; e < 16; e++) acc[c][e] = 0.0f;
    {
      const int sw = (j >> 2) & 3;
      auto texels = [&](int m, uint4& lo4, uint4& hi4) __attribute__((always_inline)) {
        const uint4* rowq = reinterpret_cast<const uint4*>(src_ring + m * kMxSlot + j * 16);
        lo4 = rowq[(2 * g) ^ sw]; hi4 = rowq[(2 * g + 1) ^ sw];
      };
      uint4 tl[3], th[3], wa[2], wb[2];
      h8 fr[2][4];
      texels(0, tl[0], th[0]);
      wa[0] = hw[lane]; wb[0] = hw[64 + lane];
      if (NKH > 1) { texels(1, tl[1], th[1]); wa[1] = hw[2 * 64 + lane]; wb[1] = hw[3 * 64 + lane]; }
      {
        const uint32_t t8[8] = {tl[0].x, tl[0].y, tl[0].z, tl[0].w, th[0].x, th[0].y, th[0].z, th[0].w};
        fr[0][0] = mx_frag<0>(t8); fr[0][1] = mx_frag<1>(t8); fr[0][2] = mx_frag<2>(t8); fr[0][3] = mx_frag<3>(t8);
      }
      __builtin_amdgcn_sched_barrier(0);
#pragma unroll
      for (int m = 0; m < NKH; m++) {
        const int cur = m & 1, nxt = cur ^ 1;
        H8Bits whi, wlo;
        whi.u[0] = wa[cur].x; whi.u[1] = wa[cur].y; whi.u[2] = wa[cur].z; whi.u[3] = wa[cur].w;
        wlo.u[0] = wb[cur].x; wlo.u[1] = wb[cur].y; wlo.u[2] = wb[cur].z; wlo.u[3] = wb[cur].w;
        if (m + 2 < NKH) texels(m + 2, tl[(m + 2) % 3], th[(m + 2) % 3]);
        acc[0] = __builtin_amdgcn_mfma_f32_32x32x16_f16(fr[cur][0], whi.v, acc[0], 0, 0, 0);
        acc[1] = __builtin_amdgcn_mfma_f32_32x32x16_f16(fr[cur][1], whi.v, acc[1], 0, 0, 0);
        acc[2] = __builtin_amdgcn_mfma_f32_32x32x16_f16(fr[cur][2], whi.v, acc[2], 0, 0, 0);
        acc[3] = __builtin_amdgcn_mfma_f32_32x32x16_f16(fr[cur][3], whi.v, acc[3], 0, 0, 0);
        if (m + 1 < NKH) {
          const uint4 &a4 = tl[(m + 1) % 3], &b4 = th[(m + 1) % 3];
          const uint32_t t8[8] = {a4.x, a4.y, a4.z, a4.w, b4.x, b4.y, b4.z, b4.w};
          fr[nxt][0] = mx_frag<0>(t8); fr[nxt][1] = mx_frag<1>(t8); fr[nxt][2] = mx_frag<2>(t8); fr[nxt][3] = mx_frag<3>(t8);
        }
#if FDH_MX_LO
        acc[0] = __builtin_amdgcn_mfma_f32_32x32x16_f16(fr[cur][0], wlo.v, acc[0], 0, 0, 0);
        acc[1] = __builtin_amdgcn_mfma_f32_32x32x16_f16(fr[cur][1], wlo.v, acc[1], 0, 0, 0);
        acc[2] = __builtin_amdgcn_mfma_f32_32x32x16_f16(fr[cur][2], wlo.v, acc[2], 0, 0, 0);
        acc[3] = __builtin_amdgcn_mfma_f32_32x32x16_f16(fr[cur][3], wlo.v, acc[3], 0, 0, 0);
#endif
        if (m + 2 < NKH) { wa[cur] = hw[(2 * m + 4) * 64 + lane]; wb[cur] = hw[(2 * m + 5) * 64 + lane]; }
        __builtin_amdgcn_sched_group_barrier(0x100, 2, 0);
        __builtin_amdgcn_sched_group_barrier(0x008, 4, 0);
        __builtin_amdgcn_sched_group_barrier(0x002, 16, 0);
#if FDH_MX_LO
        __builtin_amdgcn_sched_group_barrier(0x008, 4, 0);
        __builtin_amdgcn_sched_group_barrier(0x100, 2, 0);
#else
        __builtin_amdgcn_sched_group_barrier(0x100, 1, 0);
#endif
        __builtin_amdgcn_sched_barrier(0);
      }
    }
#if FDH_TIMING
    const unsigned long long Tc = FDH_NOW() + (__builtin_amdgcn_readfirstlane(__float_as_uint(acc[0][0] + acc[1][0] + acc[2][0] + acc[3][0])) & 0u);
    T_wait += Tb - Ta; T_h += Tc - Tb;
#endif
    const int b = i - (HB - 1);
    const int bx = xb, by = ys + 32 * b;
    const bool core = bx >= core_x0 && bx + 32 <= core_x1 && by >= core_y0 && by + 32 <= core_y1;
    __builtin_amdgcn_sched_barrier(0);
#if FDH_TIMING
    const unsigned long long Tc2 = FDH_NOW();
#endif
    phase(ph_tag, b >= 0);
#if FDH_TIMING
    const unsigned long long Td = FDH_NOW() + (__builtin_amdgcn_readfirstlane(__float_as_uint(acc[0][0] + acc[1][0] + acc[2][0] + acc[3][0])) & 0u);
    T_v += Td - Tc; T_cv += T_cv_mark - Tc2; T_dma += Tc2 - Tc;
#endif
    if (b < 0) return;
    const int x = bx + j;
    const bool x_ok = x >= P.x0 && x < P.x1;
    uint32_t pend[16];
    uint32_t pmask = 0;
#pragma unroll
    for (int rr = 0; rr < 16; rr++)
      pend[rr] = pack2(f2{acc[0][rr] * kMxScale, acc[1][rr] * kMxScale}, f2{acc[2][rr] * kMxScale, acc[3][rr] * kMxScale});
    if (bx >= P.x0 && bx + 32 <= P.x1 && by >= P.y0 && by + 32 <= P.y1) {
      pmask = 0xffffu;
    } else {
#pragma unroll
      for (int rr = 0; rr < 16; rr++) {
        const int y = by + (rr & 3) + 8 * (rr >> 2) + 4 * g;
        if (x_ok && y >= P.y0 && y < P.y1) pmask |= 1u << rr;
      }
    }
    if (P.fuse_draw >= 0) {
      bool replace_all = false;
      if (core) {
        uint32_t conj = pend[0];
#pragma unroll
        for (int rr = 1; rr < 16; rr++) conj &= pend[rr];
        replace_all = __all((conj >> 24) == 255u);
      }
      if (!replace_all) {
        const uint32_t valid = pmask;
        float al16[16];
#pragma unroll
        for (int rr = 0; rr < 16; rr++) al16[rr] = 1.0f;
        if (!core) {
          const DrawRec r = load_rec(draws + P.fuse_draw);
          const int ry0 = min(max(P.y0 - by, 0), 32), ry1 = max(ry0, min(P.y1 - by, 32)), rx0 = min(max(P.x0 - bx, 0), 32), rx1 = max(rx0, min(P.x1 - bx, 32));
          const int ra = min(max(core_y0 - by, ry0), ry1), rb = max(ra, min(max(core_y1 - by, ry0), ry1));
          const int ca = min(max(core_x0 - bx, rx0), rx1), cb = max(ca, min(max(core_x1 - bx, rx0), rx1));
          const int nra = ra - ry0, nca = ca - rx0, nr = nra + ry1 - rb, nc = nca + rx1 - cb;
#pragma unroll 1
          for (int u0 = 0; u0 < nr + nc; u0 += 2) {
            const int u = min(u0 + g, nr + nc - 1);
            int dx, dy;
            if (u < nr) { dy = u < nra ? ry0 + u : rb + (u - nra); dx = j; }
            else { const int v = u - nr; dx = v < nca ? rx0 + v : cb + (v - nca); dy = j; }
            const int ex = bx + dx, ey = by + dy;
            float alpha = 0.0f;
            if (ex >= P.x0 && ex < P.x1 && ey >= P.y0 && ey < P.y1) {
              const Frag f = make_frag(r, exts, ex, ey);
              if (f.covered) {
                const float lx = (f.u - 0.5f) * 2.0f * r.p0, ly = (f.v - 0.5f) * 2.0f * r.p1;
                const float dist = shape_dist((r.op_mode & F_ELLIP) != 0u, lx, -ly, r.p2, r.p3, r.r[0], r.r[1], r.r[2], r.r[3]);
                alpha = 1.0f - clamp01(r.aa * dist + 0.5f);
              }
            }
            const int abits = (int)__float_as_uint(alpha);
#pragma unroll
            for (int rr = 0; rr < 16; rr++) {
              const int y = (rr & 3) + 8 * (rr >> 2) + 4 * g;
              int su = -2, sl = 0;
              if (y >= ry0 && y < ry1 && j >= rx0 && j < rx1) {
                if (y < ra || y >= rb) { su = y < ra ? y - ry0 : nra + (y - rb); sl = j; }
                else if (j < ca || j >= cb) { su = nr + (j < ca ? j - rx0 : nca + (j - cb)); sl = y; }
              }
              const int v = __builtin_amdgcn_ds_bpermute(4 * (sl + 32 * (su & 1)), abits);
              if ((su & ~1) == u0) al16[rr] = __uint_as_float((uint32_t)v);
            }
          }
        }
        uint32_t blend_mask = 0;
#pragma unroll
        for (int rr = 0; rr < 16; rr++) {
          if (!((valid >> rr) & 1u)) continue;
          if (al16[rr] != 1.0f || (pend[rr] >> 24) != 255u) blend_mask |= 1u << rr;
        }
        if (__any(blend_mask != 0u)) {
          uint32_t dstv[16];
#pragma unroll
          for (int rr = 0; rr < 16; rr++)
            dstv[rr] = ((blend_mask >> rr) & 1u) ? P.src[(size_t)(by + (rr & 3) + 8 * (rr >> 2) + 4 * g) * P.pitch + x] : 0u;
          const float k = 1.0f / 255.0f;
#pragma unroll
          for (int rr = 0; rr < 16; rr++) {
            if (!((blend_mask >> rr) & 1u)) continue;
            const float alpha = al16[rr];
            const F4 bl = unpack255(pend[rr]);
            F4 Fd = unpack255(dstv[rr]);
            const float sa = bl.w * k * alpha, A = 255.0f * sa, ia = 1.0f - sa;
            Fd.x = __builtin_rintf(__builtin_fmaf(Fd.x, ia, bl.x * k * A));
            Fd.y = __builtin_rintf(__builtin_fmaf(Fd.y, ia, bl.y * k * A));
            Fd.z = __builtin_rintf(__builtin_fmaf(Fd.z, ia, bl.z * k * A));
            Fd.w = __builtin_rintf(__builtin_fmaf(Fd.w, ia, A));
            pend[rr] = pack255(Fd);
          }
          __builtin_amdgcn_s_waitcnt(0x0F70);
        }
      }
    }
#if FDH_TIMING
    const unsigned long long Te = FDH_NOW() + (__builtin_amdgcn_readfirstlane(pend[0] + pend[15]) & 0u);
    T_epi += Te - Td;
#endif
    __builtin_amdgcn_sched_barrier(0);
    {
      const uint32_t lane_off = ((uint32_t)(4 * g) * (uint32_t)P.pitch + (uint32_t)j) * 4u;
      char* base = reinterpret_cast<char*>(P.dst + (size_t)by * P.pitch + bx);
      if (__all(pmask == 0xffffu)) {
#pragma unroll
        for (int rr = 0; rr < 16; rr++)
          *reinterpret_cast<uint32_t*>(base + (size_t)((rr & 3) + 8 * (rr >> 2)) * P.pitch * 4u + lane_off) = pend[rr];
        stores_behind = 16;
      } else if (__any(pmask != 0u)) {
#pragma unroll
        for (int rr = 0; rr < 16; rr++)
          if ((pmask >> rr) & 1u) *reinterpret_cast<uint32_t*>(base + (size_t)((rr & 3) + 8 * (rr >> 2)) * P.pitch * 4u + lane_off) = pend[rr];
      }
    }
    __builtin_amdgcn_sched_barrier(0);
#if FDH_TIMING
    T_st += FDH_NOW() - Te;
#endif
  };
#pragma unroll 1
  for (int i = 0; i < n_hblocks; i += HB) {
    iteration(std::integral_constant<int, 0>{}, i);
    if (HB >= 2) { if (i + 1 >= n_hblocks) break; iteration(std::integral_constant<int, HB >= 2 ? 1 : 0>{}, i + 1); }
    if (HB >= 3) { if (i + 2 >= n_hblocks) break; iteration(std::integral_constant<int, HB >= 3 ? 2 : 0>{}, i + 2); }
  }
#if FDH_TIMING
  if (lane == 0) {
    const size_t w_id = (size_t)blockIdx.x * kFxWaves + wave;
    if (w_id < 32768) {
      unsigned long long* row = g_wave_times + 16 * w_id;
      row[0] = FDH_NOW() - T0; row[1] = T_pro; row[2] = T_wait; row[3] = T_h; row[4] = T_v; row[5] = T_epi; row[6] = 7; row[7] = T_st; row[8] = n_hblocks; row[9] = T0; row[10] = n_blocks; row[11] = T_cv; row[12] = T_dma;
    }
  }
#endif
}

static int mx_pick_t(long long per_cu, long long outputs_along, long long lines) {
  const long long slots = 256 * std::min<long long>(per_cu, 4 * kMxWaves);
  const long long along_blocks = (outputs_along + 31) / 32, line_groups = (lines + 31) / 32;
  for (int t = 1; t < 64; t++) if (line_groups * ((along_blocks + t - 1) / t) <= slots) return t;
  return 64;
}
template <int NK, bool kV> static void launch_blur_mx(hipStream_t s, const BlurParams& P, const DrawRec* draws, const QuadExt* exts) {
  constexpr size_t lds = (size_t)mx_ring_slots(NK, kV) * kMxSlot * sizeof(uint32_t);
  constexpr int kWG = mx_wg(NK, kV);
  static const int per_cu = [] {
    int n = 0;
    if (hipOccupancyMaxActiveBlocksPerMultiprocessor(&n, k_blur_mx<NK, kV>, 64 * kWG, lds * kWG) != hipSuccess || n <= 0) n = std::min<int>(4 * kMxWaves, 160 / (mx_ring_slots(NK, kV) * 2)) / kWG;
    return n * kWG;
  }();
  const int t = kV ? mx_pick_t(per_cu, P.y1 - P.y0, P.x1 - P.x0) : mx_pick_t(per_cu, P.x1 - P.x0, P.y1 - P.y0);
  const int a_lo = kV ? P.y0 : P.x0, a_hi = kV ? P.y1 : P.x1, l_lo = kV ? (P.x0 & ~31) : P.y0, l_hi = kV ? P.x1 : P.y1;
  const int total = ((a_hi - (a_lo & ~31) + 32 * t - 1) / (32 * t)) * ((l_hi - l_lo + 31) / 32);
  FDH_LAUNCH((k_blur_mx<NK, kV>), dim3(8 * ((total + 8 * kWG - 1) / (8 * kWG))), dim3(64 * kWG), lds * kWG, s, P, draws, exts, t);
}
template <bool kV> static bool launch_blur_mx_nk(hipStream_t s, const BlurParams& P, const DrawRec* draws, const QuadExt* exts) {
  if (!P.mx_w || (P.pitch & 3) || (reinterpret_cast<uintptr_t>(P.src) & 15) || P.W < 4) return false;
  const int nk = mx_nk(P.taps.reach, kV);
  switch (nk) {
    case 3: launch_blur_mx<3, kV>(s, P, draws, exts); return true;
    case 4: launch_blur_mx<4, kV>(s, P, draws, exts); return true;
    case 5: launch_blur_mx<5, kV>(s, P, draws, exts); return true;
    case 6: launch_blur_mx<6, kV>(s, P, draws, exts); return true;
    case 7: launch_blur_mx<7, kV>(s, P, draws, exts); return true;
    case 8: launch_blur_mx<8, kV>(s, P, draws, exts); return true;
    case 9: launch_blur_mx<9, kV>(s, P, draws, exts); return true;
    case 10: launch_blur_mx<10, kV>(s, P, draws, exts); return true;
    case 11: launch_blur_mx<11, kV>(s, P, draws, exts); return true;
    default: return false;
  }
}
template <int NKH, int NKV> static void launch_blur_fx(hipStream_t s, const BlurParams& P, const uint4* w_v, const DrawRec* draws, const QuadExt* exts) {
  constexpr size_t lds = (size_t)fx_slots(NKH, NKV) * kMxSlot * sizeof(uint32_t);
  static const int wg_per_cu = [] {
    int n = 0;
    if (hipOccupancyMaxActiveBlocksPerMultiprocessor(&n, k_blur_fx<NKH, NKV>, 64 * kFxWaves, lds) != hipSuccess || n <= 0) n = std::min<int>(8 / kFxWaves, (int)(160 * 1024 / lds));
    return n;
  }();
  const int n_strips = (P.x1 - (P.x0 & ~31) + 31) >> 5, n_sg = (n_strips + kFxWaves - 1) / kFxWaves, blocks = (P.y1 - (P.y0 & ~31) + 31) >> 5;
  const long long slots = 256LL * std::min(wg_per_cu, 8 / kFxWaves);
  int t = 2;
  while (t < 64 && (long long)n_sg * ((blocks + t - 1) / t) > slots) t++;
  const int total = n_sg * ((blocks + t - 1) / t), per = (total + 7) / 8;
  FDH_LAUNCH((k_blur_fx<NKH, NKV>), dim3(8 * per), dim3(64 * kFxWaves), lds, s, P, w_v, draws, exts, t);
}
bool blur_fused_supported(int reach, int W, int pitch) {
  const int nkh = mx_nk(reach, false), nkv = mx_nk(reach, true);
  return (pitch & 3) == 0 && W >= 4 && nkh >= 3 && nkh <= 6 && (nkh == nkv || nkh == nkv + 1);
}
bool launch_blur_fused(hipStream_t s, const BlurParams& P, const uint4* w_v, const DrawRec* draws, const QuadExt* exts) {
  if (P.x1 <= P.x0 || P.y1 <= P.y0) return true;
  if (!P.mx_w || !w_v || !blur_fused_supported(P.taps.reach, P.W, P.pitch) || (reinterpret_cast<uintptr_t>(P.src) & 15)) return false;
  const int nkh = mx_nk(P.taps.reach, false), nkv = mx_nk(P.taps.reach, true);
#define FDH_FX(a, b) if (nkh == a && nkv == b) { launch_blur_fx<a, b>(s, P, w_v, draws, exts); return true; }
  FDH_FX(3, 3) FDH_FX(4, 3) FDH_FX(4, 4) FDH_FX(5, 4) FDH_FX(5, 5) FDH_FX(6, 5) FDH_FX(6, 6)
#undef FDH_FX
  return false;
}
bool launch_blur_mx_pass(bool vertical, hipStream_t s, const BlurParams& P, const DrawRec* draws, const QuadExt* exts) {
  return vertical ? launch_blur_mx_nk<true>(s, P, draws, exts) : launch_blur_mx_nk<false>(s, P, draws, exts);
}
}
```

figdraw_amd/csrc/k_composite.hip:

```cpp
#include "fdh_device.h"
#include "fdh_shade.h"
#include "fdh_damage.h"

#ifndef FDH_TU
#define FDH_TU 0
#endif

namespace fdh {

__device__ __forceinline__ void order_bins_wave(const uint32_t* __restrict__ counts, int* __restrict__ order, int nx, int nb, uint32_t* offs, int lane, int cls,
                                                int deep_min = 0, uint32_t* __restrict__ deep_out = nullptr) {
#pragma unroll
  for (int k = 0; k < 4; k++) offs[lane + 64 * k] = 0;
  __builtin_amdgcn_wave_barrier();
  constexpr int kU = 8;
  const int nc = (nb - cls + 7) >> 3;
  for (int i0 = lane; i0 < nc; i0 += 64 * kU) {
    uint32_t c[kU];
#pragma unroll
    for (int k = 0; k < kU; k++) c[k] = i0 + 64 * k < nc ? counts[cls + 8 * (i0 + 64 * k)] : 0xffffffffu;
#pragma unroll
    for (int k = 0; k < kU; k++) if (c[k] != 0xffffffffu) atomicAdd(&offs[255u - min(c[k], 255u)], 1u);
  }
  __builtin_amdgcn_wave_barrier();
// ... 106 lines not shown
constexpr int kFastWaves = 5;
constexpr int kAtlasWaves = 5;
constexpr int kSlowWaves = 4;
constexpr int kSlowAtlasWaves = 3;
constexpr int kRotWaves = 4;
constexpr int kUniformWaves = 6;
constexpr int kWinCols = 64, kWinRows = 12, kWinStride = 68;
constexpr int kDeepSlots = 6;
constexpr int kDeepSlotFloats = 16 * 64;
constexpr int kDeepHdr = 8;
[[maybe_unused]] constexpr int kDeepLdsDwords = kDeepSlots * (kDeepSlotFloats + kDeepHdr) + kDeepSlots + 2;
constexpr uint32_t DT_NOP = 0, DT_PACKED = 1, DT_PACKED_BLACK = 2, DT_GENERIC = 3, DT_SELF17 = 4, DT_UNIFORM_PRE = 5;
struct DeepRing {
  float* data;
  uint32_t* hdr;
  uint32_t* ready;
  uint32_t* consumed;
  __device__ __forceinline__ explicit DeepRing(uint32_t* lds)
      : data(reinterpret_cast<float*>(lds)), hdr(lds + kDeepSlots * kDeepSlotFloats), ready(lds + kDeepSlots * (kDeepSlotFloats + kDeepHdr)),
        consumed(lds + kDeepSlots * (kDeepSlotFloats + kDeepHdr) + kDeepSlots) {}
};
__device__ __forceinline__ void deep_wait_ge(const uint32_t* p, const uint32_t want) {
  for (int spins = 0; spins < (1 << 20); spins++) {
    const uint32_t v = __builtin_amdgcn_readfirstlane(__hip_atomic_load(p, __ATOMIC_ACQUIRE, __HIP_MEMORY_SCOPE_WORKGROUP));
    if ((int32_t)(v - want) >= 0) return;
    __builtin_amdgcn_s_sleep(1);
  }
}

__device__ __forceinline__ uint32_t strip_shade_count(const CompositeParams& P, const int bin, const int sbit, const int lane) {
  const uint32_t cnt = P.counts[bin];
  const uint2* __restrict__ list = P.lists + (size_t)bin * P.stride;
  uint32_t n = 0;
  for (uint32_t base = 0; base < cnt; base += 64) {
    const uint32_t i = base + lane;
    const uint2 e = list[min(i, cnt - 1u)];
    const uint32_t ey = i < cnt ? e.y : 0u;
    const uint32_t st = (ey >> sbit) & 0x10001u;
    unsigned long long m = __ballot(st != 0u);
    const unsigned long long m_opaque = __ballot(st == 0x10001u && (e.x & LE_OPAQUE) != 0u);
    if (m_opaque != 0) m &= ~((1ull << (63 - __builtin_clzll(m_opaque))) - 1ull);
    m &= ~__ballot(st == 0x10001u && (int32_t)e.x < 0);
    n += (uint32_t)__builtin_popcountll(m);
  }
  return n;
}

template <int kPaths, bool kFull, int kRole, bool kDirect = false>
__device__ __forceinline__ void composite_strip(const CompositeParams& P, const DrawRec* __restrict__ draws, const QuadExt* __restrict__ exts,
                                                uint32_t* composite_lds, const int bin, const int sidx, const int sbit, const int tx0, const int ty0,
                                                const int lane, const int shader_id);

template <int kPaths, bool kFull, bool kDirect = false>
__global__ __launch_bounds__(64, (kPaths & 16) ? kSlowAtlasWaves : (kPaths & 1) ? kSlowWaves : kPaths == 4 ? kUniformWaves : (kPaths & 2) ? kAtlasWaves : (kPaths & 8) ? kRotWaves : kFastWaves) void k_composite_tiles(
    const int* __restrict__ a_order, int* __restrict__ a_order_next, const uint32_t* __restrict__ a_counts, const uint2* __restrict__ a_lists,
    int a_bin_x0, int a_bin_y0, int a_bin_nx, int a_bin_ny, int a_bins_x, int a_stride, int a_row_lo, int a_row_hi,
    const DrawRec* __restrict__ draws, const QuadExt* __restrict__ exts, const CompositeParams P_in) {
  CompositeParams P = P_in;
  [[maybe_unused]] const AtlasView& atlas_view = P_in.atlas;
  P.order = kFull ? a_order : nullptr; P.order_next = kFull ? a_order_next : nullptr; P.counts = a_counts; P.lists = a_lists;
  if (kFull) P.load_fb = 0;
  P.bin_x0 = a_bin_x0; P.bin_y0 = a_bin_y0; P.bin_nx = a_bin_nx; P.bin_ny = a_bin_ny;
  P.bins_x = a_bins_x; P.stride = a_stride; P.row_lo = a_row_lo; P.row_hi = a_row_hi;
  extern __shared__ uint32_t composite_lds[];
  uint32_t (*mask_stack)[kMaskDepth][64] = reinterpret_cast<uint32_t (*)[kMaskDepth][64]>(composite_lds);
  constexpr int kStripsPerBin = kWgsPerBin * kWavesPerWg;
  const int blk = P.order_next ? (int)blockIdx.x - 8 : (int)blockIdx.x;
  const int q = blk >> 3, xcd = blk & 7;
  if (blk < 0) {
    order_bins_wave(P.counts, P.order_next, P.bin_nx, P.bin_nx * P.bin_ny, &mask_stack[0][0][0], threadIdx.x, (int)blockIdx.x, kPaths == 4 ? P.deep_min : 0, kPaths == 4 ? P.deep_out : nullptr);
    return;
  }
  int bin_local = xcd + 8 * (q / kStripsPerBin);
  const int sidx = q % kStripsPerBin;
  if (bin_local >= P.bin_nx * P.bin_ny) return;
  const int j = sidx >> 2, wave = sidx & 3, lane = threadIdx.x & 63;
  const int sbit = j * 4 + wave;
  int bly, blx;
  if (P.order) {
    const int rc = P.order[bin_local];
    bly = rc >> 16; blx = rc & 0xffff;
  } else {
    bly = bin_local / P.bin_nx; blx = bin_local - bly * P.bin_nx;
  }
  const int bin_x = P.bin_x0 + blx, bin_y = P.bin_y0 + bly;
  const int bin = bin_y * P.bins_x + bin_x;
  const int tx0 = bin_x * kBin + (j & 1) * kWgW;
  const int ty0 = bin_y * kBin + (j >> 1) * kWgH + wave * kTileH;
  if (tx0 >= P.W) return;
  asm volatile("");
  if (ty0 >= P.H) return;
  asm volatile("");
  if (ty0 + kTileH <= P.row_lo) return;
  asm volatile("");
  if (ty0 >= P.row_hi) return;
#if FDH_TU == 1
  composite_strip<kPaths, kFull, 0, kDirect>(P, draws, exts, composite_lds, bin, sidx, sbit, tx0, ty0, lane, 0);
#else
  constexpr int kRole = 0;
  constexpr int shader_id = 0;
  {
#include "k_composite_strip.inc"
  }
#endif
}

template <int kUnit>
__global__ __launch_bounds__(256, kUniformWaves) void k_composite_deep(const DrawRec* __restrict__ draws, const QuadExt* __restrict__ exts, CompositeParams P) {
  extern __shared__ uint32_t composite_lds[];
  constexpr int kStripsPerBin = kWgsPerBin * kWavesPerWg;
  const int lane = threadIdx.x & 63, wg_wave = __builtin_amdgcn_readfirstlane((int)threadIdx.x >> 6);
  int blk = (int)blockIdx.x - 8;
  if (blk < 0) {
    if (wg_wave == 0) order_bins_wave(P.counts, P.order_next, P.bin_nx, P.bin_nx * P.bin_ny, composite_lds, lane, (int)blockIdx.x, P.deep_min, P.deep_out);
    return;
  }
  const int n_deep = P.deep_k8 * kStripsPerBin;
  const bool deep = blk < n_deep;
  int bin_local, sidx;
  if (deep) {
    const int q = blk >> 3;
    bin_local = (blk & 7) + 8 * (q / kStripsPerBin);
    sidx = q % kStripsPerBin;
// ... 41 lines not shown
  const int i = (int)blockIdx.x;
  if (i >= (int)dmg_count[0] * kStripsPerBin) return;
  CompositeParams P = P_in;
  P.order = nullptr; P.order_next = nullptr; P.deep_k8 = 0; P.deep_out = nullptr; P.direct = 0;
  if (kFull) P.load_fb = 0;
  extern __shared__ uint32_t composite_lds[];
  const int lane = threadIdx.x & 63;
  const int bin = dmg_list[i / kStripsPerBin];
  const int sidx = i % kStripsPerBin;
  const int bin_y = bin / P.bins_x, bin_x = bin - bin_y * P.bins_x;
  if (bin_x < P.bin_x0 || bin_x >= P.bin_x0 + P.bin_nx || bin_y < P.bin_y0 || bin_y >= P.bin_y0 + P.bin_ny) return;
  const int j = sidx >> 2, wave = sidx & 3;
  const int sbit = j * 4 + wave;
  const int tx0 = bin_x * kBin + (j & 1) * kWgW;
  const int ty0 = bin_y * kBin + (j >> 1) * kWgH + wave * kTileH;
  if (tx0 >= P.W) return;
  asm volatile("");
  if (ty0 >= P.H) return;
  asm volatile("");
  if (ty0 + kTileH <= P.row_lo) return;
  asm volatile("");
  if (ty0 >= P.row_hi) return;
  composite_strip<kPaths, kFull, 0>(P, draws, exts, composite_lds, bin, sidx, sbit, tx0, ty0, lane, 0);
}
template <int kPaths, bool kFull, bool kDirect>
static void launch_tiles(hipStream_t s, const CompositeBuild& b, int grid, const DrawRec* draws, const QuadExt* exts, const CompositeParams& P) {
  FDH_LAUNCH((k_composite_tiles<kPaths, kFull, kDirect>), dim3(grid), dim3(64), b.lds, s, P.order, P.order_next, P.counts, P.lists, P.bin_x0, P.bin_y0,
             P.bin_nx, P.bin_ny, P.bins_x, P.stride, P.row_lo, P.row_hi, draws, exts, P);
}
template <int kPaths>
static void launch_damage(hipStream_t s, const CompositeBuild& b, int grid, const DrawRec* draws, const QuadExt* exts, const CompositeParams& P,
                          const int* list, const uint32_t* count) {
  if (P.load_fb == 0) FDH_LAUNCH((k_composite_damage<kPaths, true>), dim3(grid), dim3(64), b.lds, s, list, count, draws, exts, P);
  else FDH_LAUNCH((k_composite_damage<kPaths, false>), dim3(grid), dim3(64), b.lds, s, list, count, draws, exts, P);
}
template <int kPaths>
static void launch_tiles_build(hipStream_t s, const CompositeBuild& b, int grid, const DrawRec* draws, const QuadExt* exts, const CompositeParams& P) {
  constexpr bool kHasDirect = kPaths == 0 || kPaths == 2 || kPaths == 4;
  const bool direct = kHasDirect && P.direct;
  if (P.load_fb == 0) direct ? launch_tiles<kPaths, true, kHasDirect>(s, b, grid, draws, exts, P) : launch_tiles<kPaths, true, false>(s, b, grid, draws, exts, P);
  else direct ? launch_tiles<kPaths, false, kHasDirect>(s, b, grid, draws, exts, P) : launch_tiles<kPaths, false, false>(s, b, grid, draws, exts, P);
}

void launch_composite_uniform(hipStream_t s, const CompositeBuild& b, int grid, const DrawRec* draws, const QuadExt* exts, const CompositeParams& P);
void launch_composite_damage_uniform(hipStream_t s, const CompositeBuild& b, int grid, const DrawRec* draws, const QuadExt* exts, const CompositeParams& P,
                                     const int* list, const uint32_t* count);
#if FDH_TU == 1 || !FDH_SPLIT_UNIFORM
void launch_composite_uniform(hipStream_t s, const CompositeBuild& b, int grid, const DrawRec* draws, const QuadExt* exts, const CompositeParams& P) {
  if (b.deep) {
    const int bins8 = (P.bin_nx * P.bin_ny + 7) / 8;
    FDH_LAUNCH((k_composite_deep<FDH_TU>), dim3(8 + P.deep_k8 * 16 + 8 * bins8 * kWgsPerBin), dim3(256), b.lds, s, draws, exts, P);
  } else if (b.paths == 2) launch_tiles_build<2>(s, b, grid, draws, exts, P);
  else if (b.paths == 0) launch_tiles_build<0>(s, b, grid, draws, exts, P);
  else launch_tiles_build<4>(s, b, grid, draws, exts, P);
}
void launch_composite_damage_uniform(hipStream_t s, const CompositeBuild& b, int grid, const DrawRec* draws, const QuadExt* exts, const CompositeParams& P,
                                     const int* list, const uint32_t* count) {
  if (b.paths == 2) launch_damage<2>(s, b, grid, draws, exts, P, list, count);
  else if (b.paths == 0) launch_damage<0>(s, b, grid, draws, exts, P, list, count);
  else launch_damage<4>(s, b, grid, draws, exts, P, list, count);
}
#endif

#if FDH_TU == 0
CompositeBuild composite_build(CompositeParams& P) {
  switch (forced_kernel_paths()) {
    case 3: P.has_slow = 1; P.has_slow_atlas = 0; break;
    case 19: P.has_slow = 1; P.has_slow_atlas = 1; break;
    case 8: P.has_rot = 1; break;
    case 2: P.has_atlas = 1; break;
    case 1: P.has_masks = 1; break;
  }
  CompositeBuild b;
  if (P.has_slow || (P.has_rot && P.has_atlas)) b.paths = P.has_slow_atlas ? 19 : 3;
  else if (P.has_rot) b.paths = 8;
  else b.paths = P.has_atlas ? 2 : P.has_masks ? 0 : 4;
  const int bins8 = (P.bin_nx * P.bin_ny + 7) / 8;
  if (b.paths == 4 && P.load_fb == 0 && P.order && P.order_next) b.deep_k8 = std::min(P.deep_k8 & ~7, 8 * bins8);
  b.deep = b.deep_k8 > 0;
  b.lds = b.deep ? sizeof(uint32_t) * kDeepLdsDwords
                 : (P.has_masks ? sizeof(uint32_t) * kMaskDepth * 64 : sizeof(uint32_t) * 256) +
                       (P.has_atlas || P.has_slow ? sizeof(uint32_t) * kWinRows * kWinStride : 0);
  return b;
}
void launch_composite_damage(hipStream_t s, const DrawRec* draws, const QuadExt* exts, CompositeParams P, const int* list, const uint32_t* count,
                             int grid) {
  if (grid <= 0 || P.bin_nx <= 0 || P.bin_ny <= 0) return;
  const CompositeBuild b = composite_build(P);
  P.n_wg = grid;
  if (b.paths == 19) launch_damage<19>(s, b, grid, draws, exts, P, list, count);
  else if (b.paths == 3) launch_damage<3>(s, b, grid, draws, exts, P, list, count);
  else if (b.paths == 8) launch_damage<8>(s, b, grid, draws, exts, P, list, count);
  else launch_composite_damage_uniform(s, b, grid, draws, exts, P, list, count);
}
void launch_composite(hipStream_t s, const DrawRec* draws, const QuadExt* exts, CompositeParams P) {
  const int n = P.bin_nx * P.bin_ny * kWgsPerBin;
  if (n <= 0) return;
  const CompositeBuild b = composite_build(P);
  P.n_wg = n;
  P.deep_k8 = b.deep_k8;
  const int bins8 = (P.bin_nx * P.bin_ny + 7) / 8;
  const int grid = 8 * bins8 * kWgsPerBin * kWavesPerWg + (P.order_next ? 8 : 0);
  if (b.paths == 19) launch_tiles_build<19>(s, b, grid, draws, exts, P);
  else if (b.paths == 3) launch_tiles_build<3>(s, b, grid, draws, exts, P);
  else if (b.paths == 8) launch_tiles_build<8>(s, b, grid, draws, exts, P);
  else launch_composite_uniform(s, b, grid, draws, exts, P);
}
#endif
}
```

figdraw_amd/csrc/k_composite_strip.inc:

```
  static_assert(kRole == 0 || (kPaths == 4 && kFull), "deep strips: the no-clip build's full-frame launch only");
  constexpr int kStripsPerBin = kWgsPerBin * kWavesPerWg;
  constexpr int mslot = 0;
  constexpr bool kBlender = kRole == 1, kShader = kRole == 2;
  uint32_t (*mask_stack)[kMaskDepth][64] = reinterpret_cast<uint32_t (*)[kMaskDepth][64]>(composite_lds);
  const DeepRing ring(composite_lds);
  uint32_t rank = 0, unit = 0;
  const int tx1 = tx0 + kTileW, ty1 = ty0 + kTileH;
  const int px0 = tx0 + (lane & 7) * 4, py = ty0 + (lane >> 3);
  const size_t spill_at = ((size_t)bin * kStripsPerBin + (size_t)sidx) * 64 + (size_t)lane;
  auto stack_put = [&](const int depth, const uint32_t v) __attribute__((always_inline)) {
    if (depth < kMaskDepth) mask_stack[mslot][depth][lane] = v;
    else __hip_atomic_store(P.mask_spill + (size_t)(depth - kMaskDepth) * P.spill_stride + spill_at, v, __ATOMIC_RELAXED, __HIP_MEMORY_SCOPE_AGENT);
  };
  auto stack_get = [&](const int depth) __attribute__((always_inline)) -> uint32_t {
    if (depth < kMaskDepth) return mask_stack[mslot][depth][lane];
    return __hip_atomic_load(P.mask_spill + (size_t)(depth - kMaskDepth) * P.spill_stride + spill_at, __ATOMIC_RELAXED, __HIP_MEMORY_SCOPE_AGENT);
  };
  constexpr bool kMasks = (kPaths & 4) == 0;
#if FDH_TIMING
  const unsigned long long T0 = FDH_NOW(), W0 = wall_clock64();
  unsigned long long T_cull = 0, T_rec = 0, T_shade = 0, T_cnt = 0, n_draws_t = 0, T_cull_core = 0, n_core_t = 0, n_all_t = 0;
  unsigned long long T_mode[4] = {0, 0, 0, 0}, N_mode[4] = {0, 0, 0, 0};
#endif
  constexpr bool direct = kDirect;
  const uint32_t cnt = direct ? (uint32_t)P.direct_n : P.counts[bin];
#if FDH_TIMING
  T_cnt = FDH_NOW() - T0 + (cnt & 0u);
#endif
  if (!kFull && cnt == 0 && P.load_fb) return;

  const bool row_ok = py < P.H;
  const bool vec_ok = row_ok && px0 + 3 < P.W && (P.pitch & 3) == 0;
  const size_t pix = (size_t)py * P.pitch + px0;
  F4 F0, F1, F2, F3;
  F0 = F1 = F2 = F3 = unpack255(P.clear_rgba8);
  if (!kFull && P.load_fb) {
    if (vec_ok) {
      const uint4 q = *reinterpret_cast<const uint4*>(P.fb + pix);
      F0 = unpack255(q.x); F1 = unpack255(q.y); F2 = unpack255(q.z); F3 = unpack255(q.w);
    } else if (row_ok) {
      if (px0 + 0 < P.W) F0 = unpack255(P.fb[pix + 0]);
      if (px0 + 1 < P.W) F1 = unpack255(P.fb[pix + 1]);
      if (px0 + 2 < P.W) F2 = unpack255(P.fb[pix + 2]);
      if (px0 + 3 < P.W) F3 = unpack255(P.fb[pix + 3]);
    }
  }
  float mk0 = 1.0f, mk1 = 1.0f, mk2 = 1.0f, mk3 = 1.0f;
  float rm0 = 1.0f, rm1 = 1.0f, rm2 = 1.0f, rm3 = 1.0f;
  int mask_depth = 0;
  bool rmask_on = false;
  bool touched = false;
  const uint2* __restrict__ list = P.lists + (size_t)bin * P.stride;
  const float cy = (float)py + 0.5f;
  const float cx0 = (float)px0 + 0.5f;
  const float inv255 = 1.0f / 255.0f;

  auto deep_slot = [&](const uint32_t rk) __attribute__((always_inline)) -> uint32_t {
    if (rk >= (uint32_t)kDeepSlots) deep_wait_ge(ring.consumed, rk - (uint32_t)kDeepSlots + 1u);
    return rk % (uint32_t)kDeepSlots;
  };
  auto deep_publish = [&](const uint32_t slot, const uint32_t rk, const uint32_t tag, const uint32_t h1, const uint32_t h2, const uint32_t h3, const uint32_t h4, const uint32_t h5) __attribute__((always_inline)) {
    uint32_t* h = ring.hdr + slot * kDeepHdr;
    h[0] = tag; h[1] = h1; h[2] = h2; h[3] = h3; h[4] = h4; h[5] = h5;
    __hip_atomic_store(ring.ready + slot, rk + 1u, __ATOMIC_RELEASE, __HIP_MEMORY_SCOPE_WORKGROUP);
  };
  auto deep_nop = [&](const uint32_t rk) __attribute__((always_inline)) { deep_publish(deep_slot(rk), rk, DT_NOP, 0u, 0u, 0u, 0u, 0u); };
  auto deep_consume = [&](const uint32_t rk) __attribute__((always_inline)) {
    const uint32_t slot = rk % (uint32_t)kDeepSlots;
    const uint32_t* h = ring.hdr + slot * kDeepHdr;
    const float* v = ring.data + slot * kDeepSlotFloats + lane;
    uint32_t tag, h1, h2, h3, h4, h5;
    float v0, v1, v2, v3;
#if FDH_TIMING
    const unsigned long long Tw0 = FDH_NOW();
#endif
    for (int spins = 0; spins < (1 << 20); spins++) {
      const uint32_t seq = __hip_atomic_load(ring.ready + slot, __ATOMIC_ACQUIRE, __HIP_MEMORY_SCOPE_WORKGROUP);
      tag = h[0]; h1 = h[1]; h2 = h[2]; h3 = h[3]; h4 = h[4]; h5 = h[5];
      v0 = v[0]; v1 = v[64]; v2 = v[128]; v3 = v[192];
      asm volatile("" : "+v"(tag), "+v"(h1), "+v"(h2), "+v"(h3), "+v"(h4), "+v"(h5), "+v"(v0), "+v"(v1), "+v"(v2), "+v"(v3));
      if ((int32_t)((uint32_t)__builtin_amdgcn_readfirstlane(seq) - (rk + 1u)) >= 0) break;
#if FDH_TIMING
      N_mode[3]++;
#endif
      __builtin_amdgcn_s_sleep(1);
    }
#if FDH_TIMING
    T_mode[3] += FDH_NOW() - Tw0 + (tag & 0u);
#endif
    tag = __builtin_amdgcn_readfirstlane(tag);
    if (tag == DT_PACKED || tag == DT_PACKED_BLACK) {
      const f2 saa = {v0, v1}, sab = {v2, v3};
      const f2 Aa = saa * 255.0f, Ab = sab * 255.0f, iaa = 1.0f - saa, iab = 1.0f - sab;
      if (tag == DT_PACKED_BLACK) {
        blend_black(F0, Aa.x, iaa.x); blend_black(F1, Aa.y, iaa.y); blend_black(F2, Ab.x, iab.x); blend_black(F3, Ab.y, iab.y);
      } else {
        const f2 crg = {__uint_as_float(__builtin_amdgcn_readfirstlane(h1)), __uint_as_float(__builtin_amdgcn_readfirstlane(h2))};
// ... 34 lines not shown
      e = list[min(i, cnt - 1u)];
    }
    const uint32_t idx = e.x;
    const uint32_t ey = i < cnt ? e.y : 0u;
    const uint32_t st = (ey >> sbit) & 0x10001u;
    unsigned long long m = __ballot(st != 0u);
    const unsigned long long m_core = __ballot(st == 0x10001u);
    const unsigned long long m_inq = __ballot(st == 0x10000u);
    if (!kMasks || !P.has_masks) {
      const unsigned long long m_opaque = __ballot(st == 0x10001u && (idx & LE_OPAQUE) != 0u);
      if (m_opaque != 0) m &= ~((1ull << (63 - __builtin_clzll(m_opaque))) - 1ull);
    }
#if FDH_TIMING
    T_cull += FDH_NOW() - Tc0 + (m & 0ull);
#endif
    if (m == 0) continue;
    const unsigned long long m_plainc = m_core & __ballot((int32_t)idx < 0);
    u32x4 plain_col = {0u, 0u, 0u, 0u};
    if (kBlender) plain_col = *reinterpret_cast<const u32x4*>(draws[idx & LE_INDEX].col);
    const uint32_t code_l = idx & (15u << LE_PATH_SHIFT);
    const unsigned long long m_simple = m & ~m_core & __ballot((kPaths & 3) == 0 ? code_l != 0u : (code_l - 1u) < (4u << LE_PATH_SHIFT));
    auto dist4 = [&](const DrawRec& r, const f2 pxa, const f2 pxb, const float py_, const float bx, const float by, f2& da, f2& db) __attribute__((always_inline)) {
      const bool top = py_ > 0.0f;
      const float rR = top ? r.r[0] : r.r[1], rL = top ? r.r[2] : r.r[3];
      const float ay = __builtin_fabsf(py_) - by;
      const f2 rra = {pxa.x > 0.0f ? rR : rL, pxa.y > 0.0f ? rR : rL}, rrb = {pxb.x > 0.0f ? rR : rL, pxb.y > 0.0f ? rR : rL};
      const f2 axa = {__builtin_fabsf(pxa.x), __builtin_fabsf(pxa.y)}, axb = {__builtin_fabsf(pxb.x), __builtin_fabsf(pxb.y)};
      const f2 qxa = axa - bx + rra, qxb = axb - bx + rrb;
      const f2 qya = ay + rra, qyb = ay + rrb;
      f2 ma = {__builtin_fmaxf(qxa.x, qya.x), __builtin_fmaxf(qxa.y, qya.y)}, mb = {__builtin_fmaxf(qxb.x, qyb.x), __builtin_fmaxf(qxb.y, qyb.y)};
      const f2 lowa = {__builtin_fminf(qxa.x, qya.x), __builtin_fminf(qxa.y, qya.y)}, lowb = {__builtin_fminf(qxb.x, qyb.x), __builtin_fminf(qxb.y, qyb.y)};
      if (__any(lowa.x > 0.0f || lowa.y > 0.0f || lowb.x > 0.0f || lowb.y > 0.0f)) {
        const f2 sa2 = qxa * qxa + qya * qya, sb2 = qxb * qxb + qyb * qyb;
        ma.x = lowa.x > 0.0f ? fsqrt(sa2.x) : ma.x; ma.y = lowa.y > 0.0f ? fsqrt(sa2.y) : ma.y;
        mb.x = lowb.x > 0.0f ? fsqrt(sb2.x) : mb.x; mb.y = lowb.y > 0.0f ? fsqrt(sb2.y) : mb.y;
      }
      da = ma - rra; db = mb - rrb;
    };
    auto dist4e = [&](const DrawRec& r, const f2 pxa, const f2 pxb, const float py_, const float bx, const float by, f2& oa, f2& ob) __attribute__((always_inline)) {
      const float px4[4] = {pxa.x, pxa.y, pxb.x, pxb.y};
      float d4[4];
      shape_distN<4>(true, px4, py_, bx, by, r.r[0], r.r[1], r.r[2], r.r[3], d4);
      oa = {d4[0], d4[1]}; ob = {d4[2], d4[3]};
    };
    auto edge_geom = [&](const DrawRec& r, const bool inset, const bool ellip, f2& lxa, f2& lxb, float& pyy, f2& da, f2& db) __attribute__((always_inline)) {
      const float shx = inset ? r.p0 : r.p2, shy = inset ? r.p1 : r.p3;
      pyy = local_y_up(r, cy);
      float lx4[4];
      local_x4(r, cx0, lx4);
      lxa = {lx4[0], lx4[1]}; lxb = {lx4[2], lx4[3]};
      if ((kPaths & 3) == 0 && ellip) dist4e(r, lxa, lxb, pyy, shx, shy, da, db); else dist4(r, lxa, lxb, pyy, shx, shy, da, db);
    };
    auto edge_blend = [&](const DrawRec& r, const uint32_t mode, const bool ellip, const bool inq, const float m_p2, const float m_p3, const float m_f0, const float m_f1,
                          const u32x4 m_col, const f2 lxa, const f2 lxb, const float pyy, const f2 da, const f2 db, F4& A0, F4& A1, F4& A2, F4& A3, const uint32_t rk) __attribute__((always_inline)) {
      f2 ala, alb;
      if (mode == 3u) {
        ala = {cover_aa(da.x, r.aa), cover_aa(da.y, r.aa)}; alb = {cover_aa(db.x, r.aa), cover_aa(db.y, r.aa)};
      } else if (mode == 12u) {
        const float h = m_f0 * 0.5f;
        const f2 ea = da + h, eb = db + h;
        const f2 ga = {__builtin_fabsf(ea.x), __builtin_fabsf(ea.y)}, gb = {__builtin_fabsf(eb.x), __builtin_fabsf(eb.y)};
        ala = {cover_aa(ga.x - h, r.aa), cover_aa(ga.y - h, r.aa)}; alb = {cover_aa(gb.x - h, r.aa), cover_aa(gb.y - h, r.aa)};
        if (__all(ala.x == 0.0f && ala.y == 0.0f && alb.x == 0.0f && alb.y == 0.0f)) {
          if (kShader) deep_nop(rk);
          return;
        }
      } else if (mode == 9u) {
        f2 sha, shb;
        if ((kPaths & 3) == 0 && ellip) dist4e(r, lxa - m_p2, lxb - m_p2, pyy + m_p3, r.p0, r.p1, sha, shb); else dist4(r, lxa - m_p2, lxb - m_p2, pyy + m_p3, r.p0, r.p1, sha, shb);
        const float spread = m_f1;
        const f2 sda = sha + spread, sdb = shb + spread;
        const float rs = frcp(__builtin_fmaxf(0.5f * m_f0, 0.5f));
        const f2 za = f2{__builtin_fminf(sda.x, 0.0f), __builtin_fminf(sda.y, 0.0f)} * rs, zb = f2{__builtin_fminf(sdb.x, 0.0f), __builtin_fminf(sdb.y, 0.0f)} * rs;
        const f2 ea = -0.72134752044f * za * za, eb = -0.72134752044f * zb * zb;
        ala = {cover_aa(da.x, r.aa) * fexp2(ea.x), cover_aa(da.y, r.aa) * fexp2(ea.y)};
        alb = {cover_aa(db.x, r.aa) * fexp2(eb.x), cover_aa(db.y, r.aa) * fexp2(eb.y)};
      } else {
        const float spread = m_f1;
        const f2 sda = da - spread, sdb = db - spread;
        if (__all(sda.x <= 0.0f && sda.y <= 0.0f && sdb.x <= 0.0f && sdb.y <= 0.0f)) {
          ala = 1.0f; alb = 1.0f;
        } else {
          const float rs = frcp(__builtin_fmaxf(0.5f * m_f0, 0.5f));
          const f2 za = f2{__builtin_fmaxf(sda.x, 0.0f), __builtin_fmaxf(sda.y, 0.0f)} * rs, zb = f2{__builtin_fmaxf(sdb.x, 0.0f), __builtin_fmaxf(sdb.y, 0.0f)} * rs;
          const f2 ea = -0.72134752044f * za * za, eb = -0.72134752044f * zb * zb;
          ala = {fexp2(ea.x), fexp2(ea.y)};
          alb = {fexp2(eb.x), fexp2(eb.y)};
        }
      }
      const float cw = (float)(m_col.x >> 24) * inv255;
      f2 saa = ala * cw, sab = alb * cw;
      FDH_COUNT(inq ? 64 : 65);
      if ((m_col.y | m_col.z | m_col.w) == 0u) FDH_COUNT(71);
      if (!inq) {
        const uint32_t xrel = (uint32_t)(px0 - (int)r.bx0);
        const uint32_t wcov = (py >= r.by0 && py < r.by1) ? (uint32_t)((int)r.bx1 - (int)r.bx0) : 0u;
        saa.x = xrel < wcov ? saa.x : 0.0f; saa.y = xrel + 1u < wcov ? saa.y : 0.0f;
        sab.x = xrel + 2u < wcov ? sab.x : 0.0f; sab.y = xrel + 3u < wcov ? sab.y : 0.0f;
      }
      if (kShader) {
        const uint32_t slot = deep_slot(rk);
        float* v = ring.data + slot * kDeepSlotFloats + lane;
        v[0] = saa.x; v[64] = saa.y; v[128] = sab.x; v[192] = sab.y;
        deep_publish(slot, rk, (m_col.y | m_col.z | m_col.w) == 0u ? DT_PACKED_BLACK : DT_PACKED, m_col.y, m_col.z, m_col.w, 0u, 0u);
        return;
      }
      const f2 Aa = saa * 255.0f, Ab = sab * 255.0f, iaa = 1.0f - saa, iab = 1.0f - sab;
// ... 16 lines not shown
        mask_depth--;
        if (mask_depth > 0) {
          const uint32_t w = stack_get(mask_depth - 1);
          mk0 = (float)(w & 255u) * inv255; mk1 = (float)((w >> 8) & 255u) * inv255;
          mk2 = (float)((w >> 16) & 255u) * inv255; mk3 = (float)(w >> 24) * inv255;
        } else {
          mk0 = mk1 = mk2 = mk3 = 1.0f;
        }
        return;
      }
      if (kMasks && op == OP_RMASK_END) { rm0 = rm1 = rm2 = rm3 = 1.0f; rmask_on = false; return; }
      if (kMasks && op == OP_RMASK_BEGIN && r.inv_h == 0.0f) {
        float qx[4], dm[4];
#pragma unroll
        for (int k = 0; k < 4; k++) qx[k] = ((r.ox * (cx0 + (float)k) + r.oy * cy) + r.inv_w) - r.p0;
        const float qy = ((r.inv_h * cx0 + r.f0 * cy) + r.f1) - r.p1;
        shape_distN<4>((om & F_ELLIP) != 0u, qx, -qy, r.p2, r.p3, r.r[0], r.r[1], r.r[2], r.r[3], dm);
        rm0 = 1.0f - clamp01(r.aa * dm[0] + 0.5f); rm1 = 1.0f - clamp01(r.aa * dm[1] + 0.5f);
        rm2 = 1.0f - clamp01(r.aa * dm[2] + 0.5f); rm3 = 1.0f - clamp01(r.aa * dm[3] + 0.5f);
        rmask_on = true;
        return;
      }
      const bool atlas_mode = (mode == 0u) || (mode >= 13u && mode <= 16u);
      const bool fast = (kPaths & 11) == 0 || (!(om & F_GENERAL) && !atlas_mode && mode < 18u && (op == OP_DRAW || (kMasks && op == OP_MASK_PUSH)));
      constexpr bool kSlow = (kPaths & 1) != 0, kAtlas = (kPaths & 2) != 0, kRot = (kPaths & 9) != 0;
      if (kAtlas && atlas_mode && !(om & F_GENERAL) && op == OP_DRAW && !(mode == 0u && r.aux2 > 0.0f && atlas_view.n_levels >= 2)) {
        const uint32_t fill_mode = (om >> 9) & 7u;
        const int S = atlas_view.size, msk = S - 1;
        const float fS = (float)S;
        const uint32_t* __restrict__ tex = atlas_view.level[0];
        if (mode == 0u && (om & F_TEXEL_1TO1) != 0u) {
          const uint32_t xrel = (uint32_t)(px0 - (int)r.bx0);
          const bool rowc = py >= r.by0 && py < r.by1;
          const uint32_t wcov = rowc ? (uint32_t)((int)r.bx1 - (int)r.bx0) : 0u;
          const bool any_px = rowc & (px0 + 3 >= (int)r.bx0) & (px0 < (int)r.bx1);
          const int tx = px0 + (int)r.ext, ty = py + (int)r._pad;
          const uint32_t off_in = ((((uint32_t)ty) << (uint32_t)__builtin_ctz((uint32_t)S)) + (uint32_t)tx) << 2;
          const uint32_t off = any_px ? off_in : 0u;
          struct __attribute__((packed, aligned(4))) Run4 { uint32_t v[4]; };
          const Run4 run = *reinterpret_cast<const Run4*>(reinterpret_cast<const char*>(tex) + off);
          const F4 c0u = unpack255(r.col[0]);
          const bool solid = (om & F_SOLID) != 0u, masked = mask_depth > 0 || rmask_on;
          const bool lane_col = solid || (r.col[0] == r.col[1] && r.col[2] == r.col[3]);
          const float t = (cy - r.oy) * r.inv_h;
          F4 colL = {c0u.x * inv255, c0u.y * inv255, c0u.z * inv255, c0u.w * inv255};
          if (!solid && lane_col) {
            const F4 br = unpack255(r.col[1]), tr = unpack255(r.col[2]), tl = unpack255(r.col[3]);
            const float s0 = (cx0 - r.ox) * r.inv_w;
            colL.x = tri_lerp(tl.x, c0u.x, br.x, tr.x, s0, t) * inv255;
            colL.y = tri_lerp(tl.y, c0u.y, br.y, tr.y, s0, t) * inv255;
            colL.z = tri_lerp(tl.z, c0u.z, br.z, tr.z, s0, t) * inv255;
            colL.w = tri_lerp(tl.w, c0u.w, br.w, tr.w, s0, t) * inv255;
          }
          auto texel_px = [&](const int k, F4& F, const float mk, const float rm) __attribute__((always_inline)) {
            const F4 a = unpack255(run.v[k]);
            F4 col = colL;
            if (!lane_col) {
              const F4 br = unpack255(r.col[1]), tr = unpack255(r.col[2]), tl = unpack255(r.col[3]);
              const float sk = (cx0 + (float)k - r.ox) * r.inv_w;
              col.x = tri_lerp(tl.x, c0u.x, br.x, tr.x, sk, t) * inv255;
              col.y = tri_lerp(tl.y, c0u.y, br.y, tr.y, sk, t) * inv255;
              col.z = tri_lerp(tl.z, c0u.z, br.z, tr.z, sk, t) * inv255;
              col.w = tri_lerp(tl.w, c0u.w, br.w, tr.w, sk, t) * inv255;
            }
            float sa = a.w * inv255 * col.w;
            if (masked) sa = sa * mk * rm;
            blend(F, a.x * inv255 * col.x, a.y * inv255 * col.y, a.z * inv255 * col.z, (xrel + (uint32_t)k) < wcov ? sa : 0.0f);
          };
          texel_px(0, F0, mk0, rm0); texel_px(1, F1, mk1, rm1); texel_px(2, F2, mk2, rm2); texel_px(3, F3, mk3, rm3);
          return;
        }
        const float uax = r.r[0], uay = r.r[1], utx = r.r[2], uty = r.r[3];
        const float t = (cy - r.oy) * r.inv_h;
        const float v = uay + (uty - uay) * t;
        const float ty_ = v * fS - 0.5f, fy = __builtin_floorf(ty_), ayf = ty_ - fy;
        const int y0 = (int)fy & msk, y1 = (y0 + 1) & msk;
        const uint32_t xrel = (uint32_t)(px0 - (int)r.bx0);
        const uint32_t wcov = (py >= r.by0 && py < r.by1) ? (uint32_t)((int)r.bx1 - (int)r.bx0) : 0u;
        float ushift = 0.0f;
        if (mode == 0u && (om & F_SUBPIXEL)) ushift = r.aux * frcp(__builtin_fmaxf(fS, 1.0f));
        float sK[4], uK[4], axK[4];
        uint32_t q00[4], q01[4], q10[4], q11[4];
        int fxi[4];
#pragma unroll
        for (int k = 0; k < 4; k++) {
          sK[k] = (cx0 + (float)k - r.ox) * r.inv_w;
          uK[k] = uax + (utx - uax) * sK[k];
          const float tx_ = (uK[k] - ushift) * fS - 0.5f, fx = __builtin_floorf(tx_);
          axK[k] = tx_ - fx;
          fxi[k] = (int)fx;
        }
        const int fyi = (int)fy;
        const int wxa = __builtin_amdgcn_readlane(fxi[0], 0), wxb = __builtin_amdgcn_readlane(fxi[3], 7);
        const int wya = __builtin_amdgcn_readlane(fyi, 0), wyb = __builtin_amdgcn_readlane(fyi, 56);
        const int wx0 = min(wxa, wxb), wx1 = max(wxa, wxb) + 1, wy0 = min(wya, wyb), wy1 = max(wya, wyb) + 1;
        const bool windowed = wx1 - wx0 < kWinCols && wy1 - wy0 < kWinRows && wx0 >= 0 && wy0 >= 0 && wx1 + 3 < S && wy1 < S;
        if (windowed) {
          uint32_t* const win = composite_lds + (P.has_masks ? kMaskDepth * 64 : 256);
          {
            const int lr = lane >> 4, lc = (lane & 15) * 4;
            const int cc = min(lc, (wx1 - wx0) & ~3);
            struct __attribute__((packed, aligned(4))) Run4 { uint32_t v[4]; };
#pragma unroll
            for (int pass = 0; pass < kWinRows / 4; pass++) {
              const int row = min(pass * 4 + lr, wy1 - wy0);
              const Run4 run = *reinterpret_cast<const Run4*>(tex + (((uint32_t)(wy0 + row)) << (uint32_t)__builtin_ctz((uint32_t)S)) + (uint32_t)(wx0 + cc));
              uint4 q4 = {run.v[0], run.v[1], run.v[2], run.v[3]};
              *reinterpret_cast<uint4*>(win + (pass * 4 + lr) * kWinStride + lc) = q4;
            }
          }
          __builtin_amdgcn_wave_barrier();
          const int ly = min(max(fyi - wy0, 0), kWinRows - 2);
#pragma unroll
          for (int k = 0; k < 4; k++) {
            const int lx = min(max(fxi[k] - wx0, 0), kWinCols - 2);
            const uint32_t* w0 = win + ly * kWinStride + lx;
            q00[k] = w0[0]; q01[k] = w0[1]; q10[k] = w0[kWinStride]; q11[k] = w0[kWinStride + 1];
          }
          __builtin_amdgcn_wave_barrier();
        } else {
          const char* __restrict__ texb = reinterpret_cast<const char*>(tex);
          const uint32_t row0 = ((uint32_t)y0 * (uint32_t)S) << 2, row1 = ((uint32_t)y1 * (uint32_t)S) << 2;
          auto texel = [&](uint32_t off) __attribute__((always_inline)) { return *reinterpret_cast<const uint32_t*>(texb + off); };
#pragma unroll
          for (int k = 0; k < 4; k++) {
            const uint32_t x0 = (uint32_t)(fxi[k] & msk), x1 = (x0 + 1u) & (uint32_t)msk;
            q00[k] = texel(row0 + (x0 << 2)); q01[k] = texel(row0 + (x1 << 2));
            q10[k] = texel(row1 + (x0 << 2)); q11[k] = texel(row1 + (x1 << 2));
          }
        }
        const bool solid = (om & F_SOLID) != 0u;
        const bool masked = mask_depth > 0 || rmask_on;
        const bool msdf = mode != 0u;
        const bool is_mtsdf = (mode == 14u || mode == 16u), is_stroke = (mode == 15u || mode == 16u);
        float spr = 1.0f;
        if (msdf) {
          const float unit = r.f0 * frcp(r.p0);
          const float fw_u = __builtin_fabsf((utx - uax) * r.inv_w), fw_v = __builtin_fabsf((uty - uay) * r.inv_h);
          spr = __builtin_fmaxf(0.5f * (unit * frcp(fw_u) + unit * frcp(fw_v)), 1.0f);
        }
        const F4 c0u = unpack255(r.col[0]);
        const bool lane_col = solid || (r.col[0] == r.col[1] && r.col[2] == r.col[3]);
        F4 colL = {c0u.x * inv255, c0u.y * inv255, c0u.z * inv255, c0u.w * inv255};
        if (!solid && lane_col) {
          const F4 br = unpack255(r.col[1]), tr = unpack255(r.col[2]), tl = unpack255(r.col[3]);
          colL.x = tri_lerp(tl.x, c0u.x, br.x, tr.x, sK[0], t) * inv255;
          colL.y = tri_lerp(tl.y, c0u.y, br.y, tr.y, sK[0], t) * inv255;
          colL.z = tri_lerp(tl.z, c0u.z, br.z, tr.z, sK[0], t) * inv255;
          colL.w = tri_lerp(tl.w, c0u.w, br.w, tr.w, sK[0], t) * inv255;
        }
        const bool msdf3 = msdf && !is_mtsdf;
        auto pixel = [&](const int k, F4& F, const float mk, const float rm) __attribute__((always_inline)) {
          const F4 a = unpack255(q00[k]), b = unpack255(q01[k]), c = unpack255(q10[k]), d = unpack255(q11[k]);
          const float ax = axK[k];
          F4 col = colL;
          if (!lane_col) {
            const F4 br = unpack255(r.col[1]), tr = unpack255(r.col[2]), tl = unpack255(r.col[3]);
            col.x = tri_lerp(tl.x, c0u.x, br.x, tr.x, sK[k], t) * inv255;
            col.y = tri_lerp(tl.y, c0u.y, br.y, tr.y, sK[k], t) * inv255;
            col.z = tri_lerp(tl.z, c0u.z, br.z, tr.z, sK[k], t) * inv255;
            col.w = tri_lerp(tl.w, c0u.w, br.w, tr.w, sK[k], t) * inv255;
          }
          float sr, sg, sb, sa;
          if (msdf3) {
            const float bx_ = mixf(a.x, b.x, ax) * (1.0f - ayf) + mixf(c.x, d.x, ax) * ayf;
            const float by_ = mixf(a.y, b.y, ax) * (1.0f - ayf) + mixf(c.y, d.y, ax) * ayf;
            const float bz_ = mixf(a.z, b.z, ax) * (1.0f - ayf) + mixf(c.z, d.z, ax) * ayf;
            const F4 fc = eval_fill_rec(r, col, fill_mode, uK[k], v);
            const float sd = median3(bx_, by_, bz_) * inv255;
            const float spd = spr * (sd - r.f1);
            const float alpha = is_stroke ? clamp01(__builtin_fmaxf(r.p1, 0.0f) * 0.5f - __builtin_fabsf(spd) + 0.5f) : clamp01(spd + 0.5f);
            sr = fc.x; sg = fc.y; sb = fc.z; sa = fc.w * alpha;
          } else {
            F4 tx;
            tx.x = (mixf(a.x, b.x, ax) * (1.0f - ayf) + mixf(c.x, d.x, ax) * ayf) * inv255;
            tx.y = (mixf(a.y, b.y, ax) * (1.0f - ayf) + mixf(c.y, d.y, ax) * ayf) * inv255;
            tx.z = (mixf(a.z, b.z, ax) * (1.0f - ayf) + mixf(c.z, d.z, ax) * ayf) * inv255;
            tx.w = (mixf(a.w, b.w, ax) * (1.0f - ayf) + mixf(c.w, d.w, ax) * ayf) * inv255;
            if (!msdf) {
              sr = tx.x * col.x; sg = tx.y * col.y; sb = tx.z * col.z; sa = tx.w * col.w;
            } else {
              const F4 fc = eval_fill_rec(r, col, fill_mode, uK[k], v);
              const float sd = is_mtsdf ? tx.w : median3(tx.x, tx.y, tx.z);
              const float spd = spr * (sd - r.f1);
              const float alpha = is_stroke ? clamp01(__builtin_fmaxf(r.p1, 0.0f) * 0.5f - __builtin_fabsf(spd) + 0.5f) : clamp01(spd + 0.5f);
              sr = fc.x; sg = fc.y; sb = fc.z; sa = fc.w * alpha;
            }
          }
          if (masked) sa = sa * mk * rm;
          blend(F, sr, sg, sb, (xrel + (uint32_t)k) < wcov ? sa : 0.0f);
        };
        pixel(0, F0, mk0, rm0); pixel(1, F1, mk1, rm1); pixel(2, F2, mk2, rm2); pixel(3, F3, mk3, rm3);
        return;
      }
      auto tri_bary = [&](const QuadExt& q, float (&L0)[4], float (&L1)[4], float (&L2)[4], bool (&T1)[4], bool (&cov)[4], const bool exact) __attribute__((always_inline)) {
        const int X0 = 2 * tx0 + 1, Y0 = 2 * ty0 + 1;
        const int dxl = 8 * (lane & 7), dyl = 2 * (lane >> 3);
        int eb[2][3], a2[2][3], nb[2][3];
#pragma unroll
        for (int t = 0; t < 2; t++)
#pragma unroll
          for (int k = 0; k < 3; k++) {
            const int a = q.e[t][k].a, b = q.e[t][k].b;
            nb[t][k] = (int)(((q.own >> (t * 3 + k)) & 1u) ^ 1u);
            const int base = a * X0 + b * Y0 + (int)(uint32_t)(uint64_t)q.e[t][k].c - nb[t][k];
// ... 367 lines not shown
              colv[k].z = tri_lerp(tl.z, c0.z, br.z, tr.z, u[k], t) * inv255; colv[k].w = tri_lerp(tl.w, c0.w, br.w, tr.w, u[k], t) * inv255;
            }
          }
        }
        float fx, fy, sx, sy, ex, ey;
        safe_normalize(Cx - Ax, Cy - Ay, 1.0f, 0.0f, fx, fy);
        {
          const float bf = (Bx - Ax) * fx + (By - Ay) * fy, bg = (By - Ay) * fx - (Bx - Ax) * fy;
          const float lac = (Cx - Ax) * fx + (Cy - Ay) * fy;
          const float x_lo = __builtin_fminf(0.0f, bf), x_hi = __builtin_fmaxf(lac, bf), y_lo = __builtin_fminf(0.0f, 0.5f * bg), y_hi = __builtin_fmaxf(0.0f, 0.5f * bg);
          const float ocx = 0.5f * (x_lo + x_hi), ohx = 0.5f * (x_hi - x_lo), ocy = 0.5f * (y_lo + y_hi), ohy = 0.5f * (y_hi - y_lo);
          const float reach = 1.41422f * (hw + 0.5f * frcp(r.aa)) + 0.01f;
          bool near = false;
#pragma unroll
          for (int k = 0; k < 4; k++) {
            const float rx = lx[k] - Ax, ry = lyv[k] - Ay;
            const float X = rx * fx + ry * fy, Y = ry * fx - rx * fy;
            const float db = __builtin_fmaxf(__builtin_fabsf(X - ocx) - ohx, __builtin_fabsf(Y - ocy) - ohy);
            near = near || (cov[k] && db < reach);
          }
          if (!__any(near)) { FDH_COUNT(62); return; }
        }
        FDH_COUNT(61);
        float dist[4];
        if (general) sd_bezierN<4, true>(lx, lyv, Ax, Ay, Bx, By, Cx, Cy, dist);
        else sd_bezierN<4, false>(lx, lyv, Ax, Ay, Bx, By, Cx, Cy, dist);
        float alpha[4];
        if (mode == 18u) {
#pragma unroll
          for (int k = 0; k < 4; k++) alpha[k] = 1.0f - clamp01(r.aa * (dist[k] - hw) + 0.5f);
        } else {
          safe_normalize(Bx - Ax, By - Ay, fx, fy, sx, sy);
          safe_normalize(Cx - Bx, Cy - By, fx, fy, ex, ey);
          const float trim = mode == 20u ? hw : 0.0f;
#pragma unroll
          for (int k = 0; k < 4; k++) {
            const float start_proj = (lx[k] - Ax) * sx + (lyv[k] - Ay) * sy, end_proj = (lx[k] - Cx) * ex + (lyv[k] - Cy) * ey;
            float tube = dist[k];
            if (mode == 20u) {
              const float ta = __builtin_fminf(tube, __builtin_fabsf((lx[k] - Ax) * sy - (lyv[k] - Ay) * sx));
              tube = start_proj < 0.0f ? ta : tube;
              const float tb = __builtin_fminf(tube, __builtin_fabsf((lx[k] - Cx) * ey - (lyv[k] - Cy) * ex));
              tube = end_proj > 0.0f ? tb : tube;
            }
            const float cap = __builtin_fmaxf(-start_proj - trim, end_proj - trim);
            alpha[k] = 1.0f - clamp01(r.aa * __builtin_fmaxf(tube - hw, cap) + 0.5f);
          }
        }
        const uint32_t fill_mode = (om >> 9) & 7u;
#pragma unroll
        for (int k = 0; k < 4; k++) {
          const F4 fc = eval_fill_rec(r, colv[k], fill_mode, u[k], vv[k]);
          const float mkk = k == 0 ? mk0 : k == 1 ? mk1 : k == 2 ? mk2 : mk3, rmk = k == 0 ? rm0 : k == 1 ? rm1 : k == 2 ? rm2 : rm3;
          F4& F = k == 0 ? F0 : k == 1 ? F1 : k == 2 ? F2 : F3;
          blend(F, fc.x, fc.y, fc.z, cov[k] ? fc.w * alpha[k] * mkk * rmk : 0.0f);
        }
        return;
      }
      if (!kSlow && !fast) return;
      if (kSlow && !fast) {
        FDH_COUNT(1);
        uint32_t packed = 0;
#pragma unroll 1
        for (int k = 0; k < 4; k++) {
          const int px = px0 + k;
          if (op == OP_RMASK_BEGIN) {
            rmask_on = true;
            rm0 = rect_mask_alpha(draws[d], (float)px + 0.5f, cy);
          } else {
            const bool in_frame = row_ok && px < P.W;
            const Src s = shade_one(draws + d, exts, &atlas_view, P.backdrop, pix + k, in_frame, px, py, F0);
            if (op == OP_MASK_PUSH) {
              float a = s.covered ? s.a * mk0 : 0.0f;
              const float q = __builtin_rintf(a * a * 255.0f);
              packed |= (uint32_t)q << (8 * k);
              mk0 = q * inv255;
            } else {
              float a = s.a * mk0 * rm0;
              a = s.covered ? a : 0.0f;
              blend(F0, s.r, s.g, s.b, a);
            }
          }
          { const F4 t = F0; F0 = F1; F1 = F2; F2 = F3; F3 = t; }
          { const float t = mk0; mk0 = mk1; mk1 = mk2; mk2 = mk3; mk3 = t; }
          { const float t = rm0; rm0 = rm1; rm1 = rm2; rm2 = rm3; rm3 = t; }
        }
        if (op == OP_MASK_PUSH) { stack_put(mask_depth, packed); mask_depth++; }
        return;
      }

      const bool ellip = (om & F_ELLIP) != 0u;
      const uint32_t fill_mode = (om >> 9) & 7u;
      if (core) {
        if (mode == 9u || mode == 11u || mode == 12u) { FDH_COUNT(32); if (kShader) deep_nop(rk); return; }
        if (op == OP_DRAW && (om & F_SOLID) && fill_mode == 0u && mode != 17u) {
          FDH_COUNT(33);
          const F4 c0 = unpack255(r.col[0]);
          const float sa = c0.w * inv255;
          if (mask_depth == 0 && !rmask_on) {
            const float A = 255.0f * sa, ia = 1.0f - sa;
            const f2 c_rg = {c0.x * inv255 * A, c0.y * inv255 * A}, c_ba = {c0.z * inv255 * A, A};
            if (kShader) {
              deep_publish(deep_slot(rk), rk, DT_UNIFORM_PRE, __float_as_uint(c_rg.x), __float_as_uint(c_rg.y), __float_as_uint(c_ba.x), __float_as_uint(c_ba.y), __float_as_uint(ia));
              return;
            }
            blend_pre(F0, c_rg, c_ba, ia); blend_pre(F1, c_rg, c_ba, ia); blend_pre(F2, c_rg, c_ba, ia); blend_pre(F3, c_rg, c_ba, ia);
          } else {
            const float cr = c0.x * inv255, cg = c0.y * inv255, cb = c0.z * inv255;
            blend(F0, cr, cg, cb, sa * mk0 * rm0); blend(F1, cr, cg, cb, sa * mk1 * rm1);
            blend(F2, cr, cg, cb, sa * mk2 * rm2); blend(F3, cr, cg, cb, sa * mk3 * rm3);
          }
          return;
        }
        FDH_COUNT(34);
      }
      FDH_COUNT(8 + (mode & 31u));
      if (ellip) FDH_COUNT(2);
      if (!(om & F_SOLID)) FDH_COUNT(3);
      if (fill_mode != 0u) FDH_COUNT(4);
      const float t = (cy - r.oy) * r.inv_h;
      const bool rowc = py >= r.by0 && py < r.by1;
      const bool all_cov = core || inq;
      float u[4];
      bool cov[4];
#pragma unroll
      for (int k = 0; k < 4; k++) {
        u[k] = (cx0 + (float)k - r.ox) * r.inv_w;
        cov[k] = rowc && px0 + k >= r.bx0 && px0 + k < r.bx1;
      }
      F4 col[4];
      {
        const F4 c0 = unpack255(r.col[0]);
        if (om & F_SOLID) {
#pragma unroll
          for (int k = 0; k < 4; k++) col[k] = {c0.x * inv255, c0.y * inv255, c0.z * inv255, c0.w * inv255};
        } else {
// ... 353 lines not shown
```

Baseline: 184,000 Mpixels/s.

## Skip alpha channel math when framebuffer is opaque in composite and blur

When the clear color is fully opaque, the frame is marked opaque and the composite and blur kernels get a specialized variant that tracks only RGB. The alpha is fixed at 255, so the blur runs three MFMA chains instead of four and the composite blend drops alpha arithmetic and registers. Fused blur-draw tiles in the core region can also be replaced outright. A host check that the quantised blur weights sum to the scale exact enough to keep alpha at 255 is added. This adds more template instantiations, and a frame now errors out if the weights fail that check.

```diff
diff --git a/figdraw_amd/csrc/fdh_context.cpp b/figdraw_amd/csrc/fdh_context.cpp
--- a/figdraw_amd/csrc/fdh_context.cpp
+++ b/figdraw_amd/csrc/fdh_context.cpp
@@ -452,6 +452,7 @@
   bp.node_pixels = (long long)(j.x1 - j.x0) * (j.y1 - j.y0);
   bp.fuse_draw = -1;
   bp.mx_w = (size_t)ph.blur < J.mx_w_h.size() ? J.mx_w_h[ph.blur] : nullptr;
+  bp.opaque = J.opaque ? 1 : 0;
   bp.x0 = j.x0; bp.x1 = j.x1; bp.y0 = vy0; bp.y1 = vy1;
   if ((size_t)ph.blur < J.blur_fused.size() && J.blur_fused[ph.blur]) {
     uint32_t* other = cur == fb_ ? alt_ : fb_;
@@ -506,6 +507,7 @@
   C.row_lo = row_lo; C.row_hi = row_hi;
   C.load_fb = full ? 0 : 1;
   C.clear_rgba8 = J.clear_rgba8;
+  C.opaque = J.opaque ? 1 : 0;
   C.direct = direct ? 1 : 0; C.direct_first = ph.first; C.direct_n = ph.count; C.binrec = J.dv.binrecs;
   C.order = full ? S.order_now : nullptr; C.order_next = full ? S.order_next : nullptr;
   C.deep_k8 = full ? S.deep_k8 : 0; C.deep_min = S.deep_min;
diff --git a/figdraw_amd/csrc/fdh_context.h b/figdraw_amd/csrc/fdh_context.h
--- a/figdraw_amd/csrc/fdh_context.h
+++ b/figdraw_amd/csrc/fdh_context.h
@@ -355,6 +355,7 @@
   bool clear = true;
   bool latency_routes = true;
   uint32_t clear_rgba8 = 0xFFFFFFFFu;
+  bool opaque = false;
   std::vector<Phase> phases;
   std::vector<BlurJob> blurs;
   std::vector<const uint4*> mx_w_h, mx_w_v;
@@ -498,6 +499,7 @@
   void choose_fused_blurs(LaunchJob& J);
   void consolidate_pieces();
   FoldGuard fold_clear(LaunchJob& J);
+  void decide_opaque(LaunchJob& J) const;
   void damage_frame_key(LaunchJob& J) const;
   bool shadow_usable(const LaunchJob& J);
   bool tables_resident(const LaunchJob& J, bool shadow_ok);
@@ -627,7 +629,7 @@
   PinnedBuf<uint8_t> h_pick_;
   int order_read_ = 0, order_nb_ = 0;
   bool order_valid_ = false;
-  struct MxTables { int reach; std::vector<float> dense; std::vector<uint8_t> h, v; };
+  struct MxTables { int reach; std::vector<float> dense; std::vector<uint8_t> h, v; bool keeps_opaque = false; };
   std::vector<MxTables> mx_cache_;
   static constexpr int kStaging = 4;
   std::vector<std::unique_ptr<Lane>> lanes_[kStaging];
diff --git a/figdraw_amd/csrc/fdh_device.h b/figdraw_amd/csrc/fdh_device.h
--- a/figdraw_amd/csrc/fdh_device.h
+++ b/figdraw_amd/csrc/fdh_device.h
@@ -451,6 +451,40 @@
   F.x = __builtin_rintf(F.x * ia); F.y = __builtin_rintf(F.y * ia); F.z = __builtin_rintf(F.z * ia); F.w = __builtin_rintf(__builtin_fmaf(F.w, ia, A));
 }
 
+struct F4o {
+  float x, y, z;
+  static constexpr float w = 255.0f;
+  __host__ __device__ operator F4() const { return F4{x, y, z, 255.0f}; }
+};
+template <class T> __device__ __forceinline__ T unpack_texel(uint32_t c);
+template <> __device__ __forceinline__ F4 unpack_texel<F4>(uint32_t c) { return unpack255(c); }
+template <> __device__ __forceinline__ F4o unpack_texel<F4o>(uint32_t c) {
+  F4o r;
+  r.x = (float)(c & 255u);
+  r.y = (float)((c >> 8) & 255u);
+  r.z = (float)((c >> 16) & 255u);
+  return r;
+}
+__device__ __forceinline__ uint32_t pack255(F4o f) {
+  uint32_t o = __builtin_amdgcn_cvt_pk_u8_f32(f.x, 0, 0xFF000000u);
+  o = __builtin_amdgcn_cvt_pk_u8_f32(f.y, 1, o);
+  return __builtin_amdgcn_cvt_pk_u8_f32(f.z, 2, o);
+}
+__device__ __forceinline__ void blend(F4o& F, float r, float g, float b, float sa) {
+  const float ia = 1.0f - sa, A = 255.0f * sa;
+  F.x = __builtin_rintf(__builtin_fmaf(F.x, ia, r * A));
+  F.y = __builtin_rintf(__builtin_fmaf(F.y, ia, g * A));
+  F.z = __builtin_rintf(__builtin_fmaf(F.z, ia, b * A));
+}
+__device__ __forceinline__ void blend_pre(F4o& F, f2 c_rg, f2 c_ba, float ia) {
+  F.x = __builtin_rintf(__builtin_fmaf(F.x, ia, c_rg.x));
+  F.y = __builtin_rintf(__builtin_fmaf(F.y, ia, c_rg.y));
+  F.z = __builtin_rintf(__builtin_fmaf(F.z, ia, c_ba.x));
+}
+__device__ __forceinline__ void blend_black(F4o& F, float , float ia) {
+  F.x = __builtin_rintf(F.x * ia); F.y = __builtin_rintf(F.y * ia); F.z = __builtin_rintf(F.z * ia);
+}
+
 __device__ __forceinline__ float rect_mask_alpha(const DrawRec& r, float cx, float cy) {
   float lx = (r.ox * cx + r.oy * cy) + r.inv_w;
   float ly = (r.inv_h * cx + r.f0 * cy) + r.f1;
diff --git a/figdraw_amd/csrc/fdh_kernels.h b/figdraw_amd/csrc/fdh_kernels.h
--- a/figdraw_amd/csrc/fdh_kernels.h
+++ b/figdraw_amd/csrc/fdh_kernels.h
@@ -1,6 +1,7 @@
 #pragma once
 #include <hip/hip_runtime.h>
 
+#include <cstddef>
 #include <cstdlib>
 
 #include "fdh_types.h"
@@ -54,8 +55,10 @@
   int deep_k8 = 0;
   int deep_strip_min = 0;
   int deep_min = 0;
+  int opaque = 0;
   uint32_t* deep_out = nullptr;
 };
+static_assert(offsetof(CompositeParams, deep_out) == offsetof(CompositeParams, opaque) + 4 && offsetof(CompositeParams, deep_out) + 8 == sizeof(CompositeParams), "`opaque` sits in what was padding");
 
 struct BlurParams {
   const uint32_t* src;
@@ -66,6 +69,7 @@
   const uint4* mx_w;
   BlurTaps taps;
   long long node_pixels = 0;
+  int opaque = 0;
 };
 
 void set_launch_events(hipEvent_t start, hipEvent_t stop);
diff --git a/figdraw_amd/csrc/fdh_prepare.cpp b/figdraw_amd/csrc/fdh_prepare.cpp
--- a/figdraw_amd/csrc/fdh_prepare.cpp
+++ b/figdraw_amd/csrc/fdh_prepare.cpp
@@ -41,11 +41,12 @@
     q[k] = q[2 * r - k] = v;
   }
 }
-static void build_mx_weights(const BlurTaps& t, bool vertical, uint8_t* out) {
+static float build_mx_weights(const BlurTaps& t, bool vertical, uint8_t* out) {
   const int nk = mx_nk(t.reach, vertical), delta = mx_delta(t.reach, vertical);
   uint16_t* o = reinterpret_cast<uint16_t*>(out);
   float q[2 * kMaxBlurReach + 1];
   quantise_taps_f16(t, q);
+  double sum[32] = {};
   for (int m = 0; m < nk; m++)
     for (int lane = 0; lane < 64; lane++) {
       const int j = lane & 31, g = lane >> 5;
@@ -60,8 +61,12 @@
 #endif
         o[(((size_t)(2 * m) * 64 + lane) * 8) + e] = hi;
         o[(((size_t)(2 * m + 1) * 64 + lane) * 8) + e] = lo;
+        sum[j] += (double)half_value(hi) + (double)half_value(lo);
       }
     }
+  double dev = 0.0;
+  for (int j = 0; j < 32; j++) dev = std::max(dev, std::fabs(sum[j] - 1024.0));
+  return (float)dev;
 }
 
 void blur_weight_fragments(float blur_radius, bool vertical, float* dense, uint16_t* frag_bits, int* reach, int* k_steps) {
@@ -102,6 +107,7 @@
   choose_fused_blurs(J);
   if (pieces_.size() * 3 + 2 > (size_t)kMaxUploadRuns) consolidate_pieces();
   const FoldGuard fold = fold_clear(J);
+  decide_opaque(J);
   damage_frame_key(J);
   const bool shadow_ok = shadow_usable(J), resident = tables_resident(J, shadow_ok);
   build_misc(J, resident);
@@ -221,6 +227,11 @@
   return g;
 }
 
+void Context::decide_opaque(LaunchJob& J) const {
+  static const bool opaque_on = [] { const char* e = std::getenv("FDH_OPAQUE"); return !e || std::atoi(e) != 0; }();
+  J.opaque = opaque_on && clear_ && (J.clear_rgba8 >> 24) == 255u;
+}
+
 void Context::damage_frame_key(LaunchJob& J) const {
   J.damage = damage_.on;
   J.damage_force = !clear_ || J.n_fused > 0 || J.blurs.size() > (size_t)kDamageMaxNodes;
@@ -283,11 +294,13 @@
         c.reach = t.reach;
         c.dense.assign(t.dense + kBlurPad, t.dense + kBlurPad + 2 * t.reach + 1);
         c.h.resize(bh); c.v.resize(bv);
-        build_mx_weights(t, false, c.h.data());
-        build_mx_weights(t, true, c.v.data());
+        const float dev_h = build_mx_weights(t, false, c.h.data());
+        const float dev_v = build_mx_weights(t, true, c.v.data());
+        c.keeps_opaque = std::max(dev_h, dev_v) <= kMxOpaqueSumBound;
         mx_cache_.push_back(std::move(c));
         hit = &mx_cache_.back();
       }
+      if (!hit->keeps_opaque) throw Error(FDH_ERR_INVALID, "blur weights: the fragments' sum misses the scale (an opaque surface would not stay opaque)");
       std::memcpy(misc.data() + (F.mx_h[i] - o_misc), hit->h.data(), bh);
       std::memcpy(misc.data() + (F.mx_v[i] - o_misc), hit->v.data(), bv);
     }
diff --git a/figdraw_amd/csrc/fdh_types.h b/figdraw_amd/csrc/fdh_types.h
--- a/figdraw_amd/csrc/fdh_types.h
+++ b/figdraw_amd/csrc/fdh_types.h
@@ -98,6 +98,7 @@
 #endif
 inline int mx_krow(int g, int e, bool vertical) { return vertical ? (e & 3) + 8 * (e >> 2) + 4 * g : 8 * g + e; }
 constexpr size_t mx_table_bytes(int nk) { return (size_t)nk * 2 * 64 * 16; }
+constexpr float kMxOpaqueSumBound = 1.0f;
 
 struct AtlasView {
   const uint32_t* level[kMaxMips];
diff --git a/figdraw_amd/csrc/k_blur_mx.hip b/figdraw_amd/csrc/k_blur_mx.hip
--- a/figdraw_amd/csrc/k_blur_mx.hip
+++ b/figdraw_amd/csrc/k_blur_mx.hip
@@ -27,11 +27,22 @@
   asm volatile("s_mov_b32 %0, m0\n\ts_mov_b32 m0, %2\n\ts_nop 0\n\tglobal_load_lds_dword %1, off\n\ts_mov_b32 m0, %0"
                : "=&s"(m0_saved) : "v"(src), "s"(lds) : "memory");
 }
+constexpr int mx_channels(bool opaque) { return opaque ? 3 : 4; }
+template <bool kOpaque, int NC> __device__ __forceinline__ uint32_t mx_texel(const f32x16 (&acc)[NC], int rr) {
+  if constexpr (kOpaque) {
+    uint32_t o = __builtin_amdgcn_cvt_pk_u8_f32(acc[0][rr] * kMxScale, 0, 0xFF000000u);
+    o = __builtin_amdgcn_cvt_pk_u8_f32(acc[1][rr] * kMxScale, 1, o);
+    return __builtin_amdgcn_cvt_pk_u8_f32(acc[2][rr] * kMxScale, 2, o);
+  } else {
+    return pack2(f2{acc[0][rr] * kMxScale, acc[1][rr] * kMxScale}, f2{acc[2][rr] * kMxScale, acc[3][rr] * kMxScale});
+  }
+}
 template <int N> __device__ __forceinline__ void wait_vm() { asm volatile("s_waitcnt vmcnt(%0)" ::"n"(N) : "memory"); }
 
-template <int NK, bool kV>
+template <int NK, bool kV, bool kOpaque>
 __global__ __launch_bounds__(64 * mx_wg(NK, kV), kMxWaves) void k_blur_mx(BlurParams P, const DrawRec* __restrict__ draws, const QuadExt* __restrict__ exts, int T) {
   constexpr int R = mx_ring_slots(NK, kV);
+  constexpr int NC = mx_channels(kOpaque);
   extern __shared__ __attribute__((aligned(16))) uint32_t ring_wg[];
   constexpr int kWG = mx_wg(NK, kV);
   const int wave_in_wg = kWG > 1 ? __builtin_amdgcn_readfirstlane((int)(threadIdx.x >> 6)) : 0;
@@ -172,9 +183,9 @@
 #if FDH_TIMING
     const unsigned long long Tc = FDH_NOW();
 #endif
-    f32x16 acc[4];
-#pragma unroll
-    for (int c = 0; c < 4; c++)
+    f32x16 acc[NC];
+#pragma unroll
+    for (int c = 0; c < NC; c++)
 #pragma unroll
       for (int e = 0; e < 16; e++) acc[c][e] = 0.0f;
 #pragma unroll
@@ -190,33 +201,35 @@
         const uint4 lo4 = row4[(2 * g) ^ sw], hi4 = row4[(2 * g + 1) ^ sw];
         t8[0] = lo4.x; t8[1] = lo4.y; t8[2] = lo4.z; t8[3] = lo4.w; t8[4] = hi4.x; t8[5] = hi4.y; t8[6] = hi4.z; t8[7] = hi4.w;
       }
-      const h8 f0 = mx_frag<0>(t8), f1 = mx_frag<1>(t8), f2_ = mx_frag<2>(t8), f3 = mx_frag<3>(t8);
+      const h8 f0 = mx_frag<0>(t8), f1 = mx_frag<1>(t8), f2_ = mx_frag<2>(t8);
+      [[maybe_unused]] h8 f3 = f2_;
+      if constexpr (!kOpaque) f3 = mx_frag<3>(t8);
       if (kV) {
         acc[0] = __builtin_amdgcn_mfma_f32_32x32x16_f16(whi[m], f0, acc[0], 0, 0, 0);
         acc[1] = __builtin_amdgcn_mfma_f32_32x32x16_f16(whi[m], f1, acc[1], 0, 0, 0);
         acc[2] = __builtin_amdgcn_mfma_f32_32x32x16_f16(whi[m], f2_, acc[2], 0, 0, 0);
-        acc[3] = __builtin_amdgcn_mfma_f32_32x32x16_f16(whi[m], f3, acc[3], 0, 0, 0);
+        if constexpr (!kOpaque) acc[3] = __builtin_amdgcn_mfma_f32_32x32x16_f16(whi[m], f3, acc[3], 0, 0, 0);
 #if FDH_MX_LO
         acc[0] = __builtin_amdgcn_mfma_f32_32x32x16_f16(wlo[m], f0, acc[0], 0, 0, 0);
         acc[1] = __builtin_amdgcn_mfma_f32_32x32x16_f16(wlo[m], f1, acc[1], 0, 0, 0);
         acc[2] = __builtin_amdgcn_mfma_f32_32x32x16_f16(wlo[m], f2_, acc[2], 0, 0, 0);
-        acc[3] = __builtin_amdgcn_mfma_f32_32x32x16_f16(wlo[m], f3, acc[3], 0, 0, 0);
+        if constexpr (!kOpaque) acc[3] = __builtin_amdgcn_mfma_f32_32x32x16_f16(wlo[m], f3, acc[3], 0, 0, 0);
 #endif
       } else {
         acc[0] = __builtin_amdgcn_mfma_f32_32x32x16_f16(f0, whi[m], acc[0], 0, 0, 0);
         acc[1] = __builtin_amdgcn_mfma_f32_32x32x16_f16(f1, whi[m], acc[1], 0, 0, 0);
         acc[2] = __builtin_amdgcn_mfma_f32_32x32x16_f16(f2_, whi[m], acc[2], 0, 0, 0);
-        acc[3] = __builtin_amdgcn_mfma_f32_32x32x16_f16(f3, whi[m], acc[3], 0, 0, 0);
+        if constexpr (!kOpaque) acc[3] = __builtin_amdgcn_mfma_f32_32x32x16_f16(f3, whi[m], acc[3], 0, 0, 0);
 #if FDH_MX_LO
         acc[0] = __builtin_amdgcn_mfma_f32_32x32x16_f16(f0, wlo[m], acc[0], 0, 0, 0);
         acc[1] = __builtin_amdgcn_mfma_f32_32x32x16_f16(f1, wlo[m], acc[1], 0, 0, 0);
         acc[2] = __builtin_amdgcn_mfma_f32_32x32x16_f16(f2_, wlo[m], acc[2], 0, 0, 0);
-        acc[3] = __builtin_amdgcn_mfma_f32_32x32x16_f16(f3, wlo[m], acc[3], 0, 0, 0);
-#endif
-      }
-    }
-#if FDH_TIMING
-    const unsigned long long Td = FDH_NOW() + (__builtin_amdgcn_readfirstlane(__float_as_uint(acc[0][0] + acc[1][0] + acc[2][0] + acc[3][0])) & 0u);
+        if constexpr (!kOpaque) acc[3] = __builtin_amdgcn_mfma_f32_32x32x16_f16(f3, wlo[m], acc[3], 0, 0, 0);
+#endif
+      }
+    }
+#if FDH_TIMING
+    const unsigned long long Td = FDH_NOW() + (__builtin_amdgcn_readfirstlane(__float_as_uint(acc[0][0] + acc[1][0] + acc[2][0] + acc[NC - 1][0])) & 0u);
 #endif
     const int bx = kV ? lb : as + 32 * b, by = kV ? as + 32 * b : lb;
     const int x = bx + j;
@@ -224,7 +237,7 @@
     const bool x_ok = x >= P.x0 && x < P.x1;
 #pragma unroll
     for (int rr = 0; rr < 16; rr++)
-      pend[rr] = pack2(f2{acc[0][rr] * kMxScale, acc[1][rr] * kMxScale}, f2{acc[2][rr] * kMxScale, acc[3][rr] * kMxScale});
+      pend[rr] = mx_texel<kOpaque>(acc, rr);
     if (bx >= P.x0 && bx + 32 <= P.x1 && by >= P.y0 && by + 32 <= P.y1) {
       pmask = 0xffffu;
     } else {
@@ -236,8 +249,8 @@
     }
     if (kV && P.fuse_draw >= 0) {
       const bool core = bx >= core_x0 && bx + 32 <= core_x1 && by >= core_y0 && by + 32 <= core_y1;
-      bool replace_all = false;
-      if (core) {
+      bool replace_all = kOpaque && core;
+      if (!kOpaque && core) {
         uint32_t conj = pend[0];
 #pragma unroll
         for (int rr = 1; rr < 16; rr++) conj &= pend[rr];
@@ -303,7 +316,7 @@
           const float alpha = core ? 1.0f : __uint_as_float((rr < 8 ? sc0 : sc1)[(rr & 7) * 64 + lane]);
           const F4 bl = unpack255(pend[rr]);
           F4 Fd = unpack255(dstv[rr]);
-          const float sa = bl.w * k * alpha, A = 255.0f * sa;
+          const float sa = (kOpaque ? 255.0f : bl.w) * k * alpha, A = 255.0f * sa;
           const float ia = 1.0f - sa;
           Fd.x = __builtin_rintf(__builtin_fmaf(Fd.x, ia, bl.x * k * A));
           Fd.y = __builtin_rintf(__builtin_fmaf(Fd.y, ia, bl.y * k * A));
@@ -342,10 +355,11 @@
 constexpr int fx_wg_ksteps(int nkh) { return nkh + 2 * (kFxWaves - 1); }
 constexpr int fx_slots(int nkh, int nkv) { return nkh + nkv + 2 * fx_wg_ksteps(nkh); }
 constexpr float kMxMagic = 12582912.0f;
-template <int NKH, int NKV>
+template <int NKH, int NKV, bool kOpaque>
 __global__ __launch_bounds__(64 * kFxWaves, 2) void k_blur_fx(BlurParams P, const uint4* __restrict__ w_v, const DrawRec* __restrict__ draws, const QuadExt* __restrict__ exts, int T) {
   constexpr int HB = fx_vblocks(NKV);
   constexpr int NKW = fx_wg_ksteps(NKH);
+  constexpr int NC = mx_channels(kOpaque);
   extern __shared__ __attribute__((aligned(16))) uint32_t ring[];
   const int wave = __builtin_amdgcn_readfirstlane((int)(threadIdx.x >> 6));
   const uint4* const hw = reinterpret_cast<const uint4*>(ring);
@@ -431,14 +445,14 @@
   int core_x0 = 0, core_y0 = 0, core_x1 = 0, core_y1 = 0;
   if (P.fuse_draw >= 0) { const DrawRec* qd = draws + P.fuse_draw; core_x0 = qd->ix0; core_y0 = qd->iy0; core_x1 = qd->ix1; core_y1 = qd->iy1; }
 
-  uint32_t stash[2 * HB][4][4];
+  uint32_t stash[2 * HB][NC][4];
   auto operand = [](const uint32_t (&u)[4]) { H8Bits o; o.u[0] = u[0]; o.u[1] = u[1]; o.u[2] = u[2]; o.u[3] = u[3]; return o.v; };
-  f32x16 acc[4];
+  f32x16 acc[NC];
   auto phase = [&](auto ph_tag, bool vertical) __attribute__((always_inline)) {
     constexpr int PH = decltype(ph_tag)::value;
     asm volatile("; k_blur_fx: phase %0" ::"n"(PH));
 #pragma unroll
-    for (int c = 0; c < 4; c++)
+    for (int c = 0; c < NC; c++)
 #pragma unroll
       for (int s2 = 0; s2 < 2; s2++)
 #pragma unroll
@@ -448,17 +462,17 @@
           stash[2 * PH + s2][c][qq] = pr;
         }
 #pragma unroll
-    for (int c = 0; c < 4; c++)
+    for (int c = 0; c < NC; c++)
 #pragma unroll
       for (int s2 = 0; s2 < 2; s2++)
 #pragma unroll
         for (int qq = 0; qq < 4; qq++) asm volatile("" : "+v"(stash[2 * PH + s2][c][qq]));
 #if FDH_TIMING
-    T_cv_mark = FDH_NOW() + (__builtin_amdgcn_readfirstlane(stash[2 * PH][0][0] ^ stash[2 * PH + 1][3][3]) & 0u);
+    T_cv_mark = FDH_NOW() + (__builtin_amdgcn_readfirstlane(stash[2 * PH][0][0] ^ stash[2 * PH + 1][NC - 1][3]) & 0u);
 #endif
     if (!vertical) return;
 #pragma unroll
-    for (int c = 0; c < 4; c++)
+    for (int c = 0; c < NC; c++)
 #pragma unroll
       for (int e = 0; e < 16; e++) acc[c][e] = 0.0f;
     constexpr int first = (PH + 1) % HB;
@@ -472,12 +486,12 @@
       acc[0] = __builtin_amdgcn_mfma_f32_32x32x16_f16(whi.v, operand(stash[slot][0]), acc[0], 0, 0, 0);
       acc[1] = __builtin_amdgcn_mfma_f32_32x32x16_f16(whi.v, operand(stash[slot][1]), acc[1], 0, 0, 0);
       acc[2] = __builtin_amdgcn_mfma_f32_32x32x16_f16(whi.v, operand(stash[slot][2]), acc[2], 0, 0, 0);
-      acc[3] = __builtin_amdgcn_mfma_f32_32x32x16_f16(whi.v, operand(stash[slot][3]), acc[3], 0, 0, 0);
+      if constexpr (!kOpaque) acc[NC - 1] = __builtin_amdgcn_mfma_f32_32x32x16_f16(whi.v, operand(stash[slot][NC - 1]), acc[NC - 1], 0, 0, 0);
 #if FDH_MX_LO
       acc[0] = __builtin_amdgcn_mfma_f32_32x32x16_f16(wlo.v, operand(stash[slot][0]), acc[0], 0, 0, 0);
       acc[1] = __builtin_amdgcn_mfma_f32_32x32x16_f16(wlo.v, operand(stash[slot][1]), acc[1], 0, 0, 0);
       acc[2] = __builtin_amdgcn_mfma_f32_32x32x16_f16(wlo.v, operand(stash[slot][2]), acc[2], 0, 0, 0);
-      acc[3] = __builtin_amdgcn_mfma_f32_32x32x16_f16(wlo.v, operand(stash[slot][3]), acc[3], 0, 0, 0);
+      if constexpr (!kOpaque) acc[NC - 1] = __builtin_amdgcn_mfma_f32_32x32x16_f16(wlo.v, operand(stash[slot][NC - 1]), acc[NC - 1], 0, 0, 0);
 #endif
       __builtin_amdgcn_sched_barrier(0);
     }
@@ -501,7 +515,7 @@
     const unsigned long long Tb = FDH_NOW();
 #endif
 #pragma unroll
-    for (int c = 0; c < 4; c++)
+    for (int c = 0; c < NC; c++)
 #pragma unroll
       for (int e = 0; e < 16; e++) acc[c][e] = 0.0f;
     {
@@ -511,13 +525,14 @@
         lo4 = rowq[(2 * g) ^ sw]; hi4 = rowq[(2 * g + 1) ^ sw];
       };
       uint4 tl[3], th[3], wa[2], wb[2];
-      h8 fr[2][4];
+      h8 fr[2][NC];
       texels(0, tl[0], th[0]);
       wa[0] = hw[lane]; wb[0] = hw[64 + lane];
       if (NKH > 1) { texels(1, tl[1], th[1]); wa[1] = hw[2 * 64 + lane]; wb[1] = hw[3 * 64 + lane]; }
       {
         const uint32_t t8[8] = {tl[0].x, tl[0].y, tl[0].z, tl[0].w, th[0].x, th[0].y, th[0].z, th[0].w};
-        fr[0][0] = mx_frag<0>(t8); fr[0][1] = mx_frag<1>(t8); fr[0][2] = mx_frag<2>(t8); fr[0][3] = mx_frag<3>(t8);
+        fr[0][0] = mx_frag<0>(t8); fr[0][1] = mx_frag<1>(t8); fr[0][2] = mx_frag<2>(t8);
+        if constexpr (!kOpaque) fr[0][NC - 1] = mx_frag<3>(t8);
       }
       __builtin_amdgcn_sched_barrier(0);
 #pragma unroll
@@ -530,24 +545,25 @@
         acc[0] = __builtin_amdgcn_mfma_f32_32x32x16_f16(fr[cur][0], whi.v, acc[0], 0, 0, 0);
         acc[1] = __builtin_amdgcn_mfma_f32_32x32x16_f16(fr[cur][1], whi.v, acc[1], 0, 0, 0);
         acc[2] = __builtin_amdgcn_mfma_f32_32x32x16_f16(fr[cur][2], whi.v, acc[2], 0, 0, 0);
-        acc[3] = __builtin_amdgcn_mfma_f32_32x32x16_f16(fr[cur][3], whi.v, acc[3], 0, 0, 0);
+        if constexpr (!kOpaque) acc[NC - 1] = __builtin_amdgcn_mfma_f32_32x32x16_f16(fr[cur][NC - 1], whi.v, acc[NC - 1], 0, 0, 0);
         if (m + 1 < NKH) {
           const uint4 &a4 = tl[(m + 1) % 3], &b4 = th[(m + 1) % 3];
           const uint32_t t8[8] = {a4.x, a4.y, a4.z, a4.w, b4.x, b4.y, b4.z, b4.w};
-          fr[nxt][0] = mx_frag<0>(t8); fr[nxt][1] = mx_frag<1>(t8); fr[nxt][2] = mx_frag<2>(t8); fr[nxt][3] = mx_frag<3>(t8);
+          fr[nxt][0] = mx_frag<0>(t8); fr[nxt][1] = mx_frag<1>(t8); fr[nxt][2] = mx_frag<2>(t8);
+          if constexpr (!kOpaque) fr[nxt][NC - 1] = mx_frag<3>(t8);
         }
 #if FDH_MX_LO
         acc[0] = __builtin_amdgcn_mfma_f32_32x32x16_f16(fr[cur][0], wlo.v, acc[0], 0, 0, 0);
         acc[1] = __builtin_amdgcn_mfma_f32_32x32x16_f16(fr[cur][1], wlo.v, acc[1], 0, 0, 0);
         acc[2] = __builtin_amdgcn_mfma_f32_32x32x16_f16(fr[cur][2], wlo.v, acc[2], 0, 0, 0);
-        acc[3] = __builtin_amdgcn_mfma_f32_32x32x16_f16(fr[cur][3], wlo.v, acc[3], 0, 0, 0);
+        if constexpr (!kOpaque) acc[NC - 1] = __builtin_amdgcn_mfma_f32_32x32x16_f16(fr[cur][NC - 1], wlo.v, acc[NC - 1], 0, 0, 0);
 #endif
         if (m + 2 < NKH) { wa[cur] = hw[(2 * m + 4) * 64 + lane]; wb[cur] = hw[(2 * m + 5) * 64 + lane]; }
         __builtin_amdgcn_sched_group_barrier(0x100, 2, 0);
-        __builtin_amdgcn_sched_group_barrier(0x008, 4, 0);
-        __builtin_amdgcn_sched_group_barrier(0x002, 16, 0);
+        __builtin_amdgcn_sched_group_barrier(0x008, NC, 0);
+        __builtin_amdgcn_sched_group_barrier(0x002, 4 * NC, 0);
 #if FDH_MX_LO
-        __builtin_amdgcn_sched_group_barrier(0x008, 4, 0);
+        __builtin_amdgcn_sched_group_barrier(0x008, NC, 0);
         __builtin_amdgcn_sched_group_barrier(0x100, 2, 0);
 #else
         __builtin_amdgcn_sched_group_barrier(0x100, 1, 0);
@@ -556,7 +572,7 @@
       }
     }
 #if FDH_TIMING
-    const unsigned long long Tc = FDH_NOW() + (__builtin_amdgcn_readfirstlane(__float_as_uint(acc[0][0] + acc[1][0] + acc[2][0] + acc[3][0])) & 0u);
+    const unsigned long long Tc = FDH_NOW() + (__builtin_amdgcn_readfirstlane(__float_as_uint(acc[0][0] + acc[1][0] + acc[2][0] + acc[NC - 1][0])) & 0u);
     T_wait += Tb - Ta; T_h += Tc - Tb;
 #endif
     const int b = i - (HB - 1);
@@ -568,7 +584,7 @@
 #endif
     phase(ph_tag, b >= 0);
 #if FDH_TIMING
-    const unsigned long long Td = FDH_NOW() + (__builtin_amdgcn_readfirstlane(__float_as_uint(acc[0][0] + acc[1][0] + acc[2][0] + acc[3][0])) & 0u);
+    const unsigned long long Td = FDH_NOW() + (__builtin_amdgcn_readfirstlane(__float_as_uint(acc[0][0] + acc[1][0] + acc[2][0] + acc[NC - 1][0])) & 0u);
     T_v += Td - Tc; T_cv += T_cv_mark - Tc2; T_dma += Tc2 - Tc;
 #endif
     if (b < 0) return;
@@ -578,7 +594,7 @@
     uint32_t pmask = 0;
 #pragma unroll
     for (int rr = 0; rr < 16; rr++)
-      pend[rr] = pack2(f2{acc[0][rr] * kMxScale, acc[1][rr] * kMxScale}, f2{acc[2][rr] * kMxScale, acc[3][rr] * kMxScale});
+      pend[rr] = mx_texel<kOpaque>(acc, rr);
     if (bx >= P.x0 && bx + 32 <= P.x1 && by >= P.y0 && by + 32 <= P.y1) {
       pmask = 0xffffu;
     } else {
@@ -589,8 +605,8 @@
       }
     }
     if (P.fuse_draw >= 0) {
-      bool replace_all = false;
-      if (core) {
+      bool replace_all = kOpaque && core;
+      if (!kOpaque && core) {
         uint32_t conj = pend[0];
 #pragma unroll
         for (int rr = 1; rr < 16; rr++) conj &= pend[rr];
@@ -655,7 +671,7 @@
             const float alpha = al16[rr];
             const F4 bl = unpack255(pend[rr]);
             F4 Fd = unpack255(dstv[rr]);
-            const float sa = bl.w * k * alpha, A = 255.0f * sa, ia = 1.0f - sa;
+            const float sa = (kOpaque ? 255.0f : bl.w) * k * alpha, A = 255.0f * sa, ia = 1.0f - sa;
             Fd.x = __builtin_rintf(__builtin_fmaf(Fd.x, ia, bl.x * k * A));
             Fd.y = __builtin_rintf(__builtin_fmaf(Fd.y, ia, bl.y * k * A));
             Fd.z = __builtin_rintf(__builtin_fmaf(Fd.z, ia, bl.z * k * A));
@@ -713,40 +729,42 @@
   for (int t = 1; t < 64; t++) if (line_groups * ((along_blocks + t - 1) / t) <= slots) return t;
   return 64;
 }
-template <int NK, bool kV> static void launch_blur_mx(hipStream_t s, const BlurParams& P, const DrawRec* draws, const QuadExt* exts) {
+template <int NK, bool kV, bool kOpaque> static void launch_blur_mx(hipStream_t s, const BlurParams& P, const DrawRec* draws, const QuadExt* exts) {
   constexpr size_t lds = (size_t)mx_ring_slots(NK, kV) * kMxSlot * sizeof(uint32_t);
   constexpr int kWG = mx_wg(NK, kV);
   static const int per_cu = [] {
     int n = 0;
-    if (hipOccupancyMaxActiveBlocksPerMultiprocessor(&n, k_blur_mx<NK, kV>, 64 * kWG, lds * kWG) != hipSuccess || n <= 0) n = std::min<int>(4 * kMxWaves, 160 / (mx_ring_slots(NK, kV) * 2)) / kWG;
+    if (hipOccupancyMaxActiveBlocksPerMultiprocessor(&n, k_blur_mx<NK, kV, kOpaque>, 64 * kWG, lds * kWG) != hipSuccess || n <= 0) n = std::min<int>(4 * kMxWaves, 160 / (mx_ring_slots(NK, kV) * 2)) / kWG;
     return n * kWG;
   }();
   const int t = kV ? mx_pick_t(per_cu, P.y1 - P.y0, P.x1 - P.x0) : mx_pick_t(per_cu, P.x1 - P.x0, P.y1 - P.y0);
   const int a_lo = kV ? P.y0 : P.x0, a_hi = kV ? P.y1 : P.x1, l_lo = kV ? (P.x0 & ~31) : P.y0, l_hi = kV ? P.x1 : P.y1;
   const int total = ((a_hi - (a_lo & ~31) + 32 * t - 1) / (32 * t)) * ((l_hi - l_lo + 31) / 32);
-  FDH_LAUNCH((k_blur_mx<NK, kV>), dim3(8 * ((total + 8 * kWG - 1) / (8 * kWG))), dim3(64 * kWG), lds * kWG, s, P, draws, exts, t);
+  FDH_LAUNCH((k_blur_mx<NK, kV, kOpaque>), dim3(8 * ((total + 8 * kWG - 1) / (8 * kWG))), dim3(64 * kWG), lds * kWG, s, P, draws, exts, t);
 }
 template <bool kV> static bool launch_blur_mx_nk(hipStream_t s, const BlurParams& P, const DrawRec* draws, const QuadExt* exts) {
   if (!P.mx_w || (P.pitch & 3) || (reinterpret_cast<uintptr_t>(P.src) & 15) || P.W < 4) return false;
   const int nk = mx_nk(P.taps.reach, kV);
+#define FDH_MX(n) (P.opaque ? launch_blur_mx<n, kV, true>(s, P, draws, exts) : launch_blur_mx<n, kV, false>(s, P, draws, exts))
   switch (nk) {
-    case 3: launch_blur_mx<3, kV>(s, P, draws, exts); return true;
-    case 4: launch_blur_mx<4, kV>(s, P, draws, exts); return true;
-    case 5: launch_blur_mx<5, kV>(s, P, draws, exts); return true;
-    case 6: launch_blur_mx<6, kV>(s, P, draws, exts); return true;
-    case 7: launch_blur_mx<7, kV>(s, P, draws, exts); return true;
-    case 8: launch_blur_mx<8, kV>(s, P, draws, exts); return true;
-    case 9: launch_blur_mx<9, kV>(s, P, draws, exts); return true;
-    case 10: launch_blur_mx<10, kV>(s, P, draws, exts); return true;
-    case 11: launch_blur_mx<11, kV>(s, P, draws, exts); return true;
+    case 3: FDH_MX(3); return true;
+    case 4: FDH_MX(4); return true;
+    case 5: FDH_MX(5); return true;
+    case 6: FDH_MX(6); return true;
+    case 7: FDH_MX(7); return true;
+    case 8: FDH_MX(8); return true;
+    case 9: FDH_MX(9); return true;
+    case 10: FDH_MX(10); return true;
+    case 11: FDH_MX(11); return true;
     default: return false;
   }
-}
-template <int NKH, int NKV> static void launch_blur_fx(hipStream_t s, const BlurParams& P, const uint4* w_v, const DrawRec* draws, const QuadExt* exts) {
+#undef FDH_MX
+}
+template <int NKH, int NKV, bool kOpaque> static void launch_blur_fx(hipStream_t s, const BlurParams& P, const uint4* w_v, const DrawRec* draws, const QuadExt* exts) {
   constexpr size_t lds = (size_t)fx_slots(NKH, NKV) * kMxSlot * sizeof(uint32_t);
   static const int wg_per_cu = [] {
     int n = 0;
-    if (hipOccupancyMaxActiveBlocksPerMultiprocessor(&n, k_blur_fx<NKH, NKV>, 64 * kFxWaves, lds) != hipSuccess || n <= 0) n = std::min<int>(8 / kFxWaves, (int)(160 * 1024 / lds));
+    if (hipOccupancyMaxActiveBlocksPerMultiprocessor(&n, k_blur_fx<NKH, NKV, kOpaque>, 64 * kFxWaves, lds) != hipSuccess || n <= 0) n = std::min<int>(8 / kFxWaves, (int)(160 * 1024 / lds));
     return n;
   }();
   const int n_strips = (P.x1 - (P.x0 & ~31) + 31) >> 5, n_sg = (n_strips + kFxWaves - 1) / kFxWaves, blocks = (P.y1 - (P.y0 & ~31) + 31) >> 5;
@@ -754,7 +772,7 @@
   int t = 2;
   while (t < 64 && (long long)n_sg * ((blocks + t - 1) / t) > slots) t++;
   const int total = n_sg * ((blocks + t - 1) / t), per = (total + 7) / 8;
-  FDH_LAUNCH((k_blur_fx<NKH, NKV>), dim3(8 * per), dim3(64 * kFxWaves), lds, s, P, w_v, draws, exts, t);
+  FDH_LAUNCH((k_blur_fx<NKH, NKV, kOpaque>), dim3(8 * per), dim3(64 * kFxWaves), lds, s, P, w_v, draws, exts, t);
 }
 bool blur_fused_supported(int reach, int W, int pitch) {
   const int nkh = mx_nk(reach, false), nkv = mx_nk(reach, true);
@@ -764,7 +782,7 @@
   if (P.x1 <= P.x0 || P.y1 <= P.y0) return true;
   if (!P.mx_w || !w_v || !blur_fused_supported(P.taps.reach, P.W, P.pitch) || (reinterpret_cast<uintptr_t>(P.src) & 15)) return false;
   const int nkh = mx_nk(P.taps.reach, false), nkv = mx_nk(P.taps.reach, true);
-#define FDH_FX(a, b) if (nkh == a && nkv == b) { launch_blur_fx<a, b>(s, P, w_v, draws, exts); return true; }
+#define FDH_FX(a, b) if (nkh == a && nkv == b) { P.opaque ? launch_blur_fx<a, b, true>(s, P, w_v, draws, exts) : launch_blur_fx<a, b, false>(s, P, w_v, draws, exts); return true; }
   FDH_FX(3, 3) FDH_FX(4, 3) FDH_FX(4, 4) FDH_FX(5, 4) FDH_FX(5, 5) FDH_FX(6, 5) FDH_FX(6, 6)
 #undef FDH_FX
   return false;
diff --git a/figdraw_amd/csrc/k_composite.hip b/figdraw_amd/csrc/k_composite.hip
--- a/figdraw_amd/csrc/k_composite.hip
+++ b/figdraw_amd/csrc/k_composite.hip
@@ -182,7 +182,7 @@
                                                 const int lane, const int shader_id);
 
 template <int kPaths, bool kFull, bool kDirect = false>
-__global__ __launch_bounds__(64, (kPaths & 16) ? kSlowAtlasWaves : (kPaths & 1) ? kSlowWaves : kPaths == 4 ? kUniformWaves : (kPaths & 2) ? kAtlasWaves : (kPaths & 8) ? kRotWaves : kFastWaves) void k_composite_tiles(
+__global__ __launch_bounds__(64, (kPaths & 16) ? kSlowAtlasWaves : (kPaths & 1) ? kSlowWaves : (kPaths & ~32) == 4 ? kUniformWaves : (kPaths & 2) ? kAtlasWaves : (kPaths & 8) ? kRotWaves : kFastWaves) void k_composite_tiles(
     const int* __restrict__ a_order, int* __restrict__ a_order_next, const uint32_t* __restrict__ a_counts, const uint2* __restrict__ a_lists,
     int a_bin_x0, int a_bin_y0, int a_bin_nx, int a_bin_ny, int a_bins_x, int a_stride, int a_row_lo, int a_row_hi,
     const DrawRec* __restrict__ draws, const QuadExt* __restrict__ exts, const CompositeParams P_in) {
@@ -198,7 +198,7 @@
   const int blk = P.order_next ? (int)blockIdx.x - 8 : (int)blockIdx.x;
   const int q = blk >> 3, xcd = blk & 7;
   if (blk < 0) {
-    order_bins_wave(P.counts, P.order_next, P.bin_nx, P.bin_nx * P.bin_ny, &mask_stack[0][0][0], threadIdx.x, (int)blockIdx.x, kPaths == 4 ? P.deep_min : 0, kPaths == 4 ? P.deep_out : nullptr);
+    order_bins_wave(P.counts, P.order_next, P.bin_nx, P.bin_nx * P.bin_ny, &mask_stack[0][0][0], threadIdx.x, (int)blockIdx.x, (kPaths & ~32) == 4 ? P.deep_min : 0, (kPaths & ~32) == 4 ? P.deep_out : nullptr);
     return;
   }
   int bin_local = xcd + 8 * (q / kStripsPerBin);
@@ -346,6 +346,7 @@
     FDH_LAUNCH((k_composite_deep<FDH_TU>), dim3(8 + P.deep_k8 * 16 + 8 * bins8 * kWgsPerBin), dim3(256), b.lds, s, draws, exts, P);
   } else if (b.paths == 2) launch_tiles_build<2>(s, b, grid, draws, exts, P);
   else if (b.paths == 0) launch_tiles_build<0>(s, b, grid, draws, exts, P);
+  else if (b.paths == (4 | 32)) launch_tiles_build<4 | 32>(s, b, grid, draws, exts, P);
   else launch_tiles_build<4>(s, b, grid, draws, exts, P);
 }
 void launch_composite_damage_uniform(hipStream_t s, const CompositeBuild& b, int grid, const DrawRec* draws, const QuadExt* exts, const CompositeParams& P,
@@ -372,6 +373,7 @@
   const int bins8 = (P.bin_nx * P.bin_ny + 7) / 8;
   if (b.paths == 4 && P.load_fb == 0 && P.order && P.order_next) b.deep_k8 = std::min(P.deep_k8 & ~7, 8 * bins8);
   b.deep = b.deep_k8 > 0;
+  if (b.paths == 4 && P.opaque && !b.deep && !P.direct) b.paths = 4 | 32;
   b.lds = b.deep ? sizeof(uint32_t) * kDeepLdsDwords
                  : (P.has_masks ? sizeof(uint32_t) * kMaskDepth * 64 : sizeof(uint32_t) * 256) +
                        (P.has_atlas || P.has_slow ? sizeof(uint32_t) * kWinRows * kWinStride : 0);
@@ -380,6 +382,7 @@
 void launch_composite_damage(hipStream_t s, const DrawRec* draws, const QuadExt* exts, CompositeParams P, const int* list, const uint32_t* count,
                              int grid) {
   if (grid <= 0 || P.bin_nx <= 0 || P.bin_ny <= 0) return;
+  P.opaque = 0;
   const CompositeBuild b = composite_build(P);
   P.n_wg = grid;
   if (b.paths == 19) launch_damage<19>(s, b, grid, draws, exts, P, list, count);
diff --git a/figdraw_amd/csrc/k_composite_strip.inc b/figdraw_amd/csrc/k_composite_strip.inc
--- a/figdraw_amd/csrc/k_composite_strip.inc
+++ b/figdraw_amd/csrc/k_composite_strip.inc
@@ -2,6 +2,9 @@
   constexpr int kStripsPerBin = kWgsPerBin * kWavesPerWg;
   constexpr int mslot = 0;
   constexpr bool kBlender = kRole == 1, kShader = kRole == 2;
+  constexpr bool kOpaque = (kPaths & 32) != 0;
+  static_assert(!kOpaque || (kPaths == (4 | 32) && kRole == 0), "the opaque form exists for the no-clip build only");
+  using FT = std::conditional_t<kOpaque, F4o, F4>;
   uint32_t (*mask_stack)[kMaskDepth][64] = reinterpret_cast<uint32_t (*)[kMaskDepth][64]>(composite_lds);
   const DeepRing ring(composite_lds);
   uint32_t rank = 0, unit = 0;
@@ -32,17 +35,17 @@
   const bool row_ok = py < P.H;
   const bool vec_ok = row_ok && px0 + 3 < P.W && (P.pitch & 3) == 0;
   const size_t pix = (size_t)py * P.pitch + px0;
-  F4 F0, F1, F2, F3;
-  F0 = F1 = F2 = F3 = unpack255(P.clear_rgba8);
+  FT F0, F1, F2, F3;
+  F0 = F1 = F2 = F3 = unpack_texel<FT>(P.clear_rgba8);
   if (!kFull && P.load_fb) {
     if (vec_ok) {
       const uint4 q = *reinterpret_cast<const uint4*>(P.fb + pix);
-      F0 = unpack255(q.x); F1 = unpack255(q.y); F2 = unpack255(q.z); F3 = unpack255(q.w);
+      F0 = unpack_texel<FT>(q.x); F1 = unpack_texel<FT>(q.y); F2 = unpack_texel<FT>(q.z); F3 = unpack_texel<FT>(q.w);
     } else if (row_ok) {
-      if (px0 + 0 < P.W) F0 = unpack255(P.fb[pix + 0]);
-      if (px0 + 1 < P.W) F1 = unpack255(P.fb[pix + 1]);
-      if (px0 + 2 < P.W) F2 = unpack255(P.fb[pix + 2]);
-      if (px0 + 3 < P.W) F3 = unpack255(P.fb[pix + 3]);
+      if (px0 + 0 < P.W) F0 = unpack_texel<FT>(P.fb[pix + 0]);
+      if (px0 + 1 < P.W) F1 = unpack_texel<FT>(P.fb[pix + 1]);
+      if (px0 + 2 < P.W) F2 = unpack_texel<FT>(P.fb[pix + 2]);
+      if (px0 + 3 < P.W) F3 = unpack_texel<FT>(P.fb[pix + 3]);
     }
   }
   float mk0 = 1.0f, mk1 = 1.0f, mk2 = 1.0f, mk3 = 1.0f;
@@ -183,7 +186,7 @@
       if ((kPaths & 3) == 0 && ellip) dist4e(r, lxa, lxb, pyy, shx, shy, da, db); else dist4(r, lxa, lxb, pyy, shx, shy, da, db);
     };
     auto edge_blend = [&](const DrawRec& r, const uint32_t mode, const bool ellip, const bool inq, const float m_p2, const float m_p3, const float m_f0, const float m_f1,
-                          const u32x4 m_col, const f2 lxa, const f2 lxb, const float pyy, const f2 da, const f2 db, F4& A0, F4& A1, F4& A2, F4& A3, const uint32_t rk) __attribute__((always_inline)) {
+                          const u32x4 m_col, const f2 lxa, const f2 lxb, const float pyy, const f2 da, const f2 db, FT& A0, FT& A1, FT& A2, FT& A3, const uint32_t rk) __attribute__((always_inline)) {
       f2 ala, alb;
       if (mode == 3u) {
         ala = {cover_aa(da.x, r.aa), cover_aa(da.y, r.aa)}; alb = {cover_aa(db.x, r.aa), cover_aa(db.y, r.aa)};
@@ -306,7 +309,7 @@
             colL.z = tri_lerp(tl.z, c0u.z, br.z, tr.z, s0, t) * inv255;
             colL.w = tri_lerp(tl.w, c0u.w, br.w, tr.w, s0, t) * inv255;
           }
-          auto texel_px = [&](const int k, F4& F, const float mk, const float rm) __attribute__((always_inline)) {
+          auto texel_px = [&](const int k, FT& F, const float mk, const float rm) __attribute__((always_inline)) {
             const F4 a = unpack255(run.v[k]);
             F4 col = colL;
             if (!lane_col) {
@@ -404,7 +407,7 @@
           colL.w = tri_lerp(tl.w, c0u.w, br.w, tr.w, sK[0], t) * inv255;
         }
         const bool msdf3 = msdf && !is_mtsdf;
-        auto pixel = [&](const int k, F4& F, const float mk, const float rm) __attribute__((always_inline)) {
+        auto pixel = [&](const int k, FT& F, const float mk, const float rm) __attribute__((always_inline)) {
           const F4 a = unpack255(q00[k]), b = unpack255(q01[k]), c = unpack255(q10[k]), d = unpack255(q11[k]);
           const float ax = axK[k];
           F4 col = colL;
@@ -878,7 +881,7 @@
         for (int k = 0; k < 4; k++) {
           const F4 fc = eval_fill_rec(r, colv[k], fill_mode, u[k], vv[k]);
           const float mkk = k == 0 ? mk0 : k == 1 ? mk1 : k == 2 ? mk2 : mk3, rmk = k == 0 ? rm0 : k == 1 ? rm1 : k == 2 ? rm2 : rm3;
-          F4& F = k == 0 ? F0 : k == 1 ? F1 : k == 2 ? F2 : F3;
+          FT& F = k == 0 ? F0 : k == 1 ? F1 : k == 2 ? F2 : F3;
           blend(F, fc.x, fc.y, fc.z, cov[k] ? fc.w * alpha[k] * mkk * rmk : 0.0f);
         }
         return;
@@ -907,7 +910,7 @@
               blend(F0, s.r, s.g, s.b, a);
             }
           }
-          { const F4 t = F0; F0 = F1; F1 = F2; F2 = F3; F3 = t; }
+          { const FT t = F0; F0 = F1; F1 = F2; F2 = F3; F3 = t; }
           { const float t = mk0; mk0 = mk1; mk1 = mk2; mk2 = mk3; mk3 = t; }
           { const float t = rm0; rm0 = rm1; rm1 = rm2; rm2 = rm3; rm3 = t; }
         }
```

Result: faster. 193,600 Mpixels/s (median of 6 runs) (+5.2%).
